# davidesantangelo/krep

Measured on AMD Instinct MI355X. Metric: GB/s scanned (literal scan, match offsets produced), haystack resident in HBM, higher is better.
Workload: dtype u8; 1 GPU; literal8: 8-byte case-sensitive literal 'Sherlock', ~1e-4 matches/byte, offsets tracked; 32 GiB per GPU (BASELINE.json configs[1]); pattern=Sherlock, bytes_per_gpu=34359738368, matches=3436005, parallelism=contiguous shards x1, start-offset ownership, 1 RCCL all-reduce of counts

## Files before the change

include/krep_gpu_debug.h:

```cpp
#ifndef KREP_GPU_DEBUG_H
#define KREP_GPU_DEBUG_H
#include "krep_gpu.h"
#ifdef __cplusplus
extern "C" {
#endif

uint64_t krep_gpu_debug_replay_host(int krep_ref_algo, const void *text, size_t n, const void *pattern, uint32_t m,
                                    int whole_word, size_t cur, int open_line);
void krep_gpu_debug_force_rounds(int rounds);
void krep_gpu_debug_force_stage_cap(int records);
void krep_gpu_debug_force_single_grid(int blocks);
uint64_t krep_gpu_debug_single_failovers(void);
uint64_t krep_gpu_debug_single_launches(void);
uint64_t krep_gpu_debug_tiny_launches(void);
uint64_t krep_gpu_debug_tiny_dense_launches(void);
void krep_gpu_debug_inject_failure(int kind);
void krep_gpu_debug_chain_fixups(uint64_t *rescans, uint64_t *replays);
void krep_gpu_debug_fold_carry(const krep_gpu_seq_carry_t *in, const krep_gpu_seq_carry_t *piece, krep_gpu_seq_carry_t *out);
uint64_t krep_gpu_debug_anchored_launches(void);
uint64_t krep_gpu_debug_literal_dma_launches(void);
uint64_t krep_gpu_debug_literal_dma_one_pass_launches(void);
uint64_t krep_gpu_debug_literal_dma_one_pass_failovers(void);
void krep_gpu_debug_force_literal_dma_grid(int blocks);
int krep_gpu_debug_literal_dma_state(const krep_gpu_plan_t *plan, int *looked, int *barred, double *pass_rate);
uint64_t krep_gpu_debug_runs_launches(void);
int krep_gpu_debug_split_state(const krep_gpu_plan_t *plan);
int krep_gpu_debug_anchor_info(const krep_gpu_plan_t *plan, int *state, uint32_t *moved, double *rate_end_grams, double *rate_anchors);
int krep_gpu_debug_anchor_measured(const krep_gpu_plan_t *plan, double *measured, int *resamples);

#ifdef __cplusplus
}
#endif
#endif
```

krep_amd/csrc/kg_ac.hip:

```cpp
#include <hip/hip_runtime.h>

#include <algorithm>
#include <atomic>
#include <cstdlib>
#include <cstring>
#include <unordered_map>
#include <vector>

#include "../../include/krep_gpu.h"
#include "kg_ac_common.h"
#include "kg_ac_tables.h"
#include "kg_internal.h"

namespace kg {

#ifndef KG_AC_LINES_ROLL_CELLS
#define KG_AC_LINES_ROLL_CELLS 4
#endif
template <bool CI, bool LINES, bool SHORT, int STRIDE, int ANCH = 0, bool WW = false>
__global__ __launch_bounds__(kAcBlock) void ac_scan_kernel(const AcArgs a)
{
    static_assert(!WW || (STRIDE == 2 && !SHORT), "the -w filter of the depth masks: pair filter, no short patterns");
    static_assert(!ANCH || (STRIDE == 2 && !LINES && !SHORT), "anchored scan: pair filter, records / counts only");
    extern __shared__ __attribute__((aligned(16))) u32 s_mem[];
// ... 959 lines not shown
    AcArgs &a = r.a;
    const size_t own_lo = c.own_lo, own_hi = r.own_hi, text_len = c.text_len;
    const bool own_by_end = c.own != AcOwn::Start;
    r.lines_on_list = c.own == AcOwn::LinesOnList;
    r.fsc = g_force_stage_cap.load(std::memory_order_relaxed);
    a.text = c.d_text; a.text_len = text_len; a.global_base = c.global_base;
    a.own_lo = own_lo; a.own_hi = own_hi;
    a.end_lo = own_lo;
    a.end_hi = (c.lines || own_by_end) ? own_hi : std::min<u64>(text_len, (u64)own_hi + t->lmax - 1);
    if (own_by_end)
    {
        a.own_lo = 0, a.own_hi = text_len;
    }
    a.anchor = ((own_by_end && !c.lines && own_lo && !getenv("KREP_GPU_AC_R05_ANCHOR")) ? own_lo - 1 : own_lo) & ~(u64)15;
    a.num_tiles = (a.end_hi - a.anchor + kAcUnitBytes - 1) / kAcUnitBytes;
    a.flags = (t->ci ? F_CI : 0) | (c.ww ? F_WW : 0) | (c.lines ? F_LINES : 0);
    a.flags |= getenv("KREP_GPU_AC_NOVERIFY") ? 1u << 31 : 0u;
    a.flags |= getenv("KREP_GPU_AC_NOSTAGE3") ? 1u << 28 : 0u;
    a.flags |= getenv("KREP_GPU_AC_NODEFER") ? 1u << 27 : 0u;
    a.flags |= getenv("KREP_GPU_AC_NOPROBE") ? 1u << 30 : 0u;
    a.lmax = t->lmax; a.has1 = t->has1; a.has2 = t->has2; a.has3 = t->has3; a.has4 = t->has4;
    a.stride = 1;
    a.filter = c.lines ? t->d_filterx19 : t->d_filterx20;
    a.filter_words = (1u << (c.lines ? kXBitsLines : kXBitsBig)) / 32;
    if (t->d_filters20)
    {
        a.filter = c.lines ? t->d_filters19 : t->d_filters20;
        a.stride = 2;
    }
    if (t->anch_state == 0 && text_len >= (1u << 20) && own_hi - own_lo >= (1u << 19))
    {
        HIPCHK(hipSetDevice(t->device));
        if (ac_anchor_prepare(t, c.d_text, text_len, own_lo, own_hi, c.st) == 2)
            (void)hipGetLastError();
    }
    if (t->anch_state == 2 && !c.lines && a.stride == 2 && !getenv("KREP_GPU_AC_NO_ANCHOR"))
    {
        a.filter = t->d_filtera20;
        a.anch = t->d_anch; a.anch_mask = t->anch_mask; a.anch_mul = t->anch_mul; a.anch_five = t->anch_five;
    }
    if (t->d_xtab && !getenv("KREP_GPU_AC_NO_EXACT"))
    {
        a.xlen = t->d_xlen; a.xtab = t->d_xtab; a.xmask = t->xmask; a.xmul = t->xmul;
    }
    a.s1 = t->d_s1; a.s2 = t->d_s2; a.s3 = t->d_s3;
    if (t->short_dup)
        a.flags |= F_AC_SHORT_DUP;
    a.edges = t->d_edges; a.emask = t->emask; a.copies = t->d_copies;
    a.gram4 = t->d_gram4; a.g4x = t->d_g4x; a.g4mask = t->g4mask;
    a.g4x_mode = t->g4x_mode; a.g4x_mask = t->g4x_mask; a.g4x_mul = t->g4x_mul;
    a.ctr = c.d_ctr;
    r.want = (c.d_pos && c.cap && !c.lines) ? std::min<u64>(c.cap, (u64)c.max_count) : 0;
    if (r.want)
        a.flags |= F_POS;
    a.positions = (u64 *)c.d_pos; a.pos_cap = r.want;
    return 0;
}
static int ac_result(const AcScan &c, const AcRun &r, bool staged, krep_gpu_scan_out_t *out)
{
    const Counters &h = *c.h_ctr;
    if (c.time_it)
    {
        float ms = 0;
        HIPCHK(hipEventElapsedTime(&ms, c.ev0, c.ev1));
        out->kernel_ms = ms;
    }
    const u64 total = h.total;
    out->total_matches = total;
    out->line_count = staged ? h.lines : 0;
    if (r.lines_on_list)
        out->line_count = (r.want && !h.overflow_units && total <= r.want) ? h.lines : ~0ull;
    const u64 summary = (staged && (r.want || c.lines)) ? h.summary : (total ? (kLnHead | kLnTail) : 0);
    out->has_newline = (summary & kLnNl) != 0;
    out->head_line_hit = (summary & kLnHead) != 0;
    out->tail_line_hit = (summary & kLnTail) != 0;
    out->count = std::min<u64>(c.lines ? h.lines : total, (u64)c.max_count);
    if (r.want && c.track)
    {
        out->stored = std::min<u64>(out->count, r.want);
        out->overflow = out->count > c.cap;
    }
    return 0;
}
static int ac_byte_set(const AcScan &c, AcRun &r, krep_gpu_scan_out_t *out)
{
    AcTables *t = c.t;
    if (!(t->set_n && r.want && !c.ww && c.own == AcOwn::Start && t->set_ok && c.text_len >= (size_t)16 * kSegBytes && !r.fsc &&
          !getenv("KREP_GPU_NO_FUSED1") && !getenv("KREP_GPU_AC_NO_TINY")))
        return kAcNext;
    LitArgs la{};
    la.text = c.d_text; la.text_len = c.text_len; la.global_base = c.global_base;
    la.own_lo = c.own_lo; la.own_hi = r.own_hi;
    la.anchor = c.own_lo & ~(u64)15;
    la.rounds = kRoundsBig;
    const u64 tile_bytes = (u64)kRoundsBig * kSegBytes * kWavesPerBlk;
    la.num_tiles = (r.own_hi - la.anchor + tile_bytes - 1) / tile_bytes;
    la.ww_exempt_left = ~0ull;
    la.m = 1;
    la.flags = (t->ci ? F_CI : 0) | F_POS;
    la.ctr = c.d_ctr; la.positions = (uint64_t *)c.d_pos; la.pos_cap = r.want;
    la.set_n = t->set_n;
    for (u32 k = 0; k < t->set_n; ++k)
    {
        la.set_p[k] = 0x01010101u * t->set_b[k];
        la.set_l[k] = (t->ci && t->set_b[k] >= 'a' && t->set_b[k] <= 'z') ? 0x20202020u : 0u;
    }
    la.p0 = la.set_p[0]; la.l0 = la.set_l[0]; la.k0 = 0xffu;
    HIPCHK(hipSetDevice(t->device));
    if (c.time_it) HIPCHK(hipEventRecord(c.ev0, c.st));
    const int rc = single_fused_run(la, la.num_tiles * kWavesPerBlk, r.own_hi - la.anchor, *c.post, c.d_ctr, c.h_ctr, (u32)c.num_cu, &t->set_shape,
                                    c.time_it ? c.ev1 : nullptr, c.st, false);
    if (rc == 2)
        return 2;
    if (rc != kFusedGaveUp)
        return ac_result(c, r, false, out);
    t->set_ok = false;
    return kAcNext;
}
static u32 tiny_dense_upt(double e)
{
    if (e <= 0.0)
        return 4u;
    const double u = (double)ac_tiny_dense_ring() / (2.5 * e);
    return u >= 4.0 ? 4u : (u32)u;
}
static void tiny_reopen(AcTables *t, u64 total, u64 n_units)
{
    if (!t->tiny_fused_ok && total < n_units * 20)
        t->tiny_fused_ok = true;
    if (!t->tiny_dense_ok && total < n_units * 20)
        t->tiny_dense_ok = true;
    if (!t->tiny.five && t->tiny_dense_ok && !t->tiny_dense_upt && total >= n_units * 48)
        t->tiny_dense_upt = tiny_dense_upt((double)total / (double)n_units);
}
static int ac_tiny_one_pass(const AcScan &c, const AcRun &r, krep_gpu_scan_out_t *out)
{
    AcTables *t = c.t;
    Counters *h_ctr = c.h_ctr;
    const bool one_pass_ok = t->tiny.ok && !t->tiny.five && r.want && !c.ww && c.own != AcOwn::End && c.track && !r.fsc &&
                             c.text_len >= (size_t)64 * kAcUnitBytes && !getenv("KREP_GPU_AC_NO_TINY_FUSED") && !getenv("KREP_GPU_AC_NO_TINY");
    const bool dense_first = getenv("KREP_GPU_AC_TINY_DENSE_FIRST") != nullptr;
    if (dense_first && one_pass_ok && !t->tiny_dense_upt && t->tiny_dense_ok)
        t->tiny_dense_upt = 4;
    for (int attempt = 0; one_pass_ok && attempt < 3; ++attempt)
    {
        const bool dense = t->tiny_dense_upt != 0 && !getenv("KREP_GPU_AC_NO_TINY_DENSE");
        if (!dense && (!t->tiny_fused_ok || t->tiny.llong))
            break;
        AcArgs f = r.a;
        f.upt = dense ? t->tiny_dense_upt : (u32)std::min<u64>(kAcUnitsPerTicketMax, std::max<u64>(1, f.num_tiles / ((u64)c.num_cu * kTinyWaves * 4)));
        const u64 n_tk = (f.num_tiles + f.upt - 1) / f.upt;
        const size_t tk_bytes = 2 * n_tk * sizeof(unsigned long long);
        HIPCHK(grow_scratch(c.post->tk_cap, n_tk, n_tk, {dev_buf(c.post->d_tk, tk_bytes)}));
        f.tk_agg = c.post->d_tk; f.tk_pref = c.post->d_tk + n_tk; f.n_tk = n_tk; f.stage_cap = 0;
        HIPCHK(hipSetDevice(t->device));
        if (c.time_it) HIPCHK(hipEventRecord(c.ev0, c.st));
        HIPCHK(hipMemsetAsync(c.d_ctr, 0, sizeof(Counters), c.st));
        HIPCHK(hipMemsetAsync(c.post->d_tk, 0, tk_bytes, c.st));
        HIPCHK(ac_tiny_launch_fused(f, t->tiny, n_tk, (u32)c.num_cu, c.st, dense));
        if (r.lines_on_list && tail_launch_line_gaps(c.d_text, c.text_len, c.global_base, (const uint64_t *)c.d_pos, &c.d_ctr->total,
                                                     &c.d_ctr->overflow_units, r.want, &c.d_ctr->lines, c.st))
            return 2;
        if (c.time_it) HIPCHK(hipEventRecord(c.ev1, c.st));
        HIPCHK(hipMemcpyAsync(h_ctr, c.d_ctr, sizeof(Counters), hipMemcpyDeviceToHost, c.st));
        HIPCHK(hipStreamSynchronize(c.st));
        const double per_unit = (double)h_ctr->total / (double)f.num_tiles;
        if (getenv("KREP_GPU_DEBUG"))
            fprintf(stderr, "krep-gpu: tiny one-pass (%s, %u units per ticket): %llu matches, %.1f per unit, %llu waves overflowed\n",
                    dense ? "dense" : "items", f.upt, (unsigned long long)h_ctr->total, per_unit, (unsigned long long)h_ctr->overflow_units);
        if (!h_ctr->overflow_units)
        {
            if (ac_result(c, r, false, out))
                return 2;
            if (dense)
            {
                if (per_unit < 24.0 && !dense_first)
                    t->tiny_dense_upt = 0, t->tiny_fused_ok = true;
                else
                    t->tiny_dense_upt = std::max(1u, tiny_dense_upt(per_unit));
            }
            return 0;
        }
        u32 nu = (t->tiny_dense_ok && h_ctr->total) ? tiny_dense_upt(per_unit) : 0u;
        if (dense && nu >= t->tiny_dense_upt)
            nu = t->tiny_dense_upt - 1u;
        if (!dense)
            t->tiny_fused_ok = false;
        t->tiny_dense_upt = nu;
        if (!nu)
        {
            t->tiny_dense_ok = false;
            break;
        }
    }
    return kAcNext;
}
static hipError_t ac_staged_launch(const AcScan &c, const AcRun &r, const AcArgs &a)
{
    const u64 n_tickets = (a.num_tiles + a.upt - 1) / a.upt;
    if (r.tiny)
        return ac_tiny_launch(a, c.t->tiny, n_tickets, (u32)c.num_cu, c.st);
    const u32 lds = ac_lds_bytes(a.filter_words, c.lines), per_cu = lds <= 80 * 1024 ? 2u : 1u;
    return ac_launch(a, (u32)std::min<u64>((n_tickets + kAcWaves - 1) / kAcWaves, (u64)c.num_cu * per_cu), lds, c.st);
}
static int ac_staged(const AcScan &c, AcRun &r)
{
    AcArgs &a = r.a;
    const bool chain = r.want || c.lines;
    const u64 n_units = a.num_tiles;
    a.stage_cap = r.want ? (r.fsc ? (u32)r.fsc : c.t->stage_cap) : 0u;
    if (chain)
    {
        if (post_reserve(*c.post, n_units, (n_units * a.stage_cap + 1) / 2))
            return 2;
        a.unitinfo = c.post->d_unitinfo; a.stage = (u64 *)c.post->d_stage; a.offsets = (const u64 *)c.post->d_offsets;
    }
    HIPCHK(hipSetDevice(c.t->device));
    r.tiny = c.t->tiny.ok && !c.ww && (!c.t->tiny.five || (!r.want && !c.lines && !c.t->ci));
    const u32 waves = r.tiny ? (u32)kTinyWaves : (u32)kAcWaves;
    a.upt = (u32)std::min<u64>(kAcUnitsPerTicketMax, std::max<u64>(1, a.num_tiles / ((u64)c.num_cu * waves * 4)));
    if (const char *e = getenv("KREP_GPU_AC_UPT"))
    {
        const int v = atoi(e);
        if (v >= 1 && v <= (int)kAcUnitsPerTicketMax)
            a.upt = (u32)v;
    }
    if (c.time_it) HIPCHK(hipEventRecord(c.ev0, c.st));
    const bool dbg_sync = getenv("KREP_GPU_SYNC_DEBUG") != nullptr;
    auto dbg = [&](const char *what) -> int {
        if (!dbg_sync)
            return 0;
        const hipError_t e = hipStreamSynchronize(c.st);
        return e == hipSuccess ? 0 : fail("ac_scan: %s faulted: %s (tiny=%d stride=%u units=%llu stage_cap=%u lines=%d list=%d own=[%llu,%llu) end=[%llu,%llu) n=%llu)", what,
                                          hipGetErrorString(e), (int)r.tiny, a.stride, (unsigned long long)n_units, a.stage_cap, (int)c.lines, (int)r.lines_on_list,
                                          (unsigned long long)a.own_lo, (unsigned long long)a.own_hi, (unsigned long long)a.end_lo,
                                          (unsigned long long)a.end_hi, (unsigned long long)c.text_len);
    };
    HIPCHK(hipMemsetAsync(c.d_ctr, 0, sizeof(Counters), c.st));
    HIPCHK(ac_staged_launch(c, r, a));
    if (dbg("scan kernel")) return 2;
    if (chain && post_order(*c.post, n_units, a.stage_cap, 0, a.anchor + c.global_base, kAcUnitBytes, c.lines, (uint64_t *)c.d_pos, r.want, c.d_ctr,
                            c.num_cu, c.st))
        return 2;
    if (dbg("post-pass")) return 2;
    if (r.lines_on_list && r.want && tail_launch_line_gaps(c.d_text, c.text_len, c.global_base, (const uint64_t *)c.d_pos, &c.d_ctr->total,
                                                           &c.d_ctr->overflow_units, r.want, &c.d_ctr->lines, c.st))
        return 2;
    if (dbg("line-gap kernel")) return 2;
    if (c.time_it) HIPCHK(hipEventRecord(c.ev1, c.st));
    HIPCHK(hipMemcpyAsync(c.h_ctr, c.d_ctr, sizeof(Counters), hipMemcpyDeviceToHost, c.st));
    HIPCHK(hipStreamSynchronize(c.st));
    return 0;
}
static void ac_learn(const AcScan &c, const AcRun &r)
{
    AcTables *t = c.t;
    const AcArgs &a = r.a;
    const Counters &h = *c.h_ctr;
    const size_t own_lo = c.own_lo, own_hi = r.own_hi;
    const u64 n_units = a.num_tiles;
    if (!r.tiny && !c.lines && a.stride == 2 && own_hi > own_lo)
    {
        const double tested = 0.5 * (double)(own_hi - own_lo);
        t->anch_measured = (double)h.candidates / tested;
        const double est = t->anch_state == 2 ? t->anch_rate : t->anch_rate0;
        if (t->anch_state != 0 && t->anch_resamples < kAnchResamples && c.text_len >= (1u << 20) && own_hi - own_lo >= (1u << 19) &&
            t->anch_measured > 0.008 && t->anch_measured > 2.0 * est + 0.002 && !getenv("KREP_GPU_AC_ANCHOR") && !getenv("KREP_GPU_AC_NO_RESAMPLE"))
        {
            if (getenv("KREP_GPU_DEBUG"))
                fprintf(stderr, "krep-gpu: anchors: measured %.3f %% candidates per tested position against %.3f %% estimated (%s): the next scan decides again\n",
                        100.0 * t->anch_measured, 100.0 * est, t->anch_state == 2 ? "anchored" : "end grams");
            t->anch_state = 0;
            ++t->anch_resamples;
        }
    }
    if (!r.want || r.fsc)
        return;
    if (r.tiny && h.overflow_units * 2 > n_units && h.total > n_units * 256)
        t->stage_cap = 0;
    else if (t->stage_cap && h.overflow_units * 64 > n_units)
        t->stage_cap = 64;
    else if (!t->stage_cap && h.total < n_units * 32)
        t->stage_cap = 64;
    if (r.tiny)
        tiny_reopen(t, h.total, n_units);
    if (t->set_n && !t->set_ok && own_hi > a.anchor && single_fused_reopens(h.total, own_hi - a.anchor))
        t->set_ok = true;
}
static int ac_emit(const AcScan &c, const AcRun &r)
{
    AcTables *t = c.t;
    const u64 n_units = r.a.num_tiles;
    AcArgs e = r.a;
    e.emit_mode = 1;
    HIPCHK(hipMemsetAsync(&c.d_ctr->ticket, 0, sizeof(unsigned long long), c.st));
    if (!r.tiny && !getenv("KREP_GPU_AC_NO_REDO_LIST"))
    {
        const u64 n_over = c.h_ctr->overflow_units;
        const u64 redo_cap = n_over + n_over / 4 + 64;
        if (grow_scratch(t->redo_cap, n_over, redo_cap, {dev_buf(t->d_redo, redo_cap * sizeof(u32))}) != hipSuccess)
            (void)hipGetLastError();
        if (t->d_redo && n_over <= 0xffffffffull)
        {
            HIPCHK(hipMemsetAsync(&c.d_ctr->pad[3], 0, sizeof(unsigned long long), c.st));
            hipLaunchKernelGGL(ac_redo_list_kernel, dim3((u32)((n_units + 255) / 256)), dim3(256), 0, c.st, (const u64 *)e.unitinfo, n_units, e.stage_cap,
                               t->d_redo, (u32)t->redo_cap, &c.d_ctr->pad[3]);
// ... 25 lines not shown
```

krep_amd/csrc/kg_ac_tiny.hip:

```cpp
#include <algorithm>
#include <atomic>
#include <type_traits>
#include <utility>

#include "kg_ac_common.h"
#include "kg_internal.h"
#include "kg_tickets.h"

namespace kg {

bool ac_tiny_keeps(const AcArgs &a);
extern int g_s1_force_grid;
#ifndef KG_TINY_KEEP_WAVES
#define KG_TINY_KEEP_WAVES 2
#endif
#ifndef KG_TINY_FUSED_WAVES
#define KG_TINY_FUSED_WAVES 3
#endif
#ifndef KG_TINY_FIVE_WAVES
#define KG_TINY_FIVE_WAVES 2
#endif
#ifndef KG_TINY_ROLL_CELLS
#define KG_TINY_ROLL_CELLS 6
#endif
#ifndef KG_TINY_LINES_WAVES
#define KG_TINY_LINES_WAVES 3
#endif
#ifndef KG_TINY_COUNT_WAVES
#define KG_TINY_COUNT_WAVES 3
#endif
#define KG_TINY_KEEP_WAVES_ARG ((KEEP && !EMIT) ? KG_TINY_KEEP_WAVES : (FIVE ? KG_TINY_FIVE_WAVES : (FUSED ? KG_TINY_FUSED_WAVES : (LINES ? KG_TINY_LINES_WAVES : KG_TINY_COUNT_WAVES))))
constexpr int kTinyBlock = kTinyWaves * 64;
constexpr u32 kTinyEntries = kAcUnitBytes / 16;

template <int... J, typename F>
__device__ __forceinline__ void tiny_static_for(std::integer_sequence<int, J...>, F &&f)
{
    (f(std::integral_constant<int, J>{}), ...);
}
__device__ __forceinline__ u32 tiny_scramble16(u32 m)
{
    u32 f = 0;
#pragma unroll
    for (int w = 0; w < 4; ++w)
        f |= ((((m >> (4 * w)) & 0xfu) * 0x00204081u) & 0x01010101u) << w;
    return f;
}

template <bool CI, bool LINES, bool KEEP, bool EMIT, bool LONG, bool FUSED = false, bool FIVE = false, bool DENSE = false>
__global__ __launch_bounds__(kTinyBlock, KG_TINY_KEEP_WAVES_ARG) void ac_tiny_kernel(const AcArgs a, const AcTiny td)
{
    static_assert(!DENSE || (FUSED && !FIVE), "DENSE is a flavour of the one-pass writer");
    extern __shared__ __attribute__((aligned(16))) u32 s_tiny[];
    const u32 lane = lane_id(), wave = threadIdx.x >> 6;
    static_assert(!FUSED || (!LINES && !KEEP && !EMIT), "the one-pass record writer is its own mode");
    static_assert(!FIVE || (!LINES && !KEEP && !EMIT && !LONG), "a fifth class: counting and one-pass records only");
    if constexpr (FUSED)
    {
        bool resolver = false;
        if (__builtin_amdgcn_readfirstlane(wave) == 0u)
            resolver = wave_fetch_add(&a.ctr->pad[0], 1ull, lane) == 0ull;
        if (resolver)
        {
            tk_resolve(a.tk_agg, a.tk_pref, a.n_tk, a.ctr, lane);
            return;
        }
    }
    constexpr u32 kPark = kAcUnitsPerTicketMax * 64 + kAcUnitsPerTicketMax * 2;
    constexpr u32 kPerWave = FUSED ? kTinyRing * 3u : kTinyEntries * 2 + kPark;
    u32 *base = s_tiny + wave * kPerWave;
    u32 *park_slots = base + kTinyEntries * 2;
    u64 *park_info = reinterpret_cast<u64 *>(base + kTinyEntries * 2 + kAcUnitsPerTicketMax * 64);
    uint2 *cw = reinterpret_cast<uint2 *>(base);

    const bool want_pos = (a.flags & F_POS) != 0;
    const bool chain = !FUSED && (want_pos || LINES);
    constexpr bool emit_final = EMIT;
    uint2 *ring_m = reinterpret_cast<uint2 *>(base);
    u32 *ring_id = base + 2u * kTinyRing;
    bool pend = false, overflowed = false;
    u64 pend_t = 0;
    u32 pend_at = 0, pend_items = 0, wp = 0;
    u32 f_at = 0, f_room = 0, f_items = 0;
    u32 lane_cnt = 0;
    constexpr u32 kDenseRing = kTinyRing * 6u;
    unsigned short *ring16 = reinterpret_cast<unsigned short *>(base);
    u32 u_c0 = 0, u_c1 = 0, u_c2 = 0, u_before = 0, pend_c0 = 0, pend_c1 = 0, pend_c2 = 0;
    auto dwrap = [](const u32 x) -> u32 { return x >= kDenseRing ? x - kDenseRing : x; };
    auto flush_dense = [&](const u32 l4) __attribute__((always_inline)) {
        const u64 first = tk_wait_prefix(a.tk_pref, pend_t, a.ctr, lane);
        const u64 tbase = a.anchor + pend_t * (u64)a.upt * kAcUnitBytes + a.global_base + 1u;
        const u32 b1 = pend_c0, b2 = pend_c0 + pend_c1, b3 = pend_c0 + pend_c1 + pend_c2;
        const u32 pad = (u32)(first & 7ull);
        for (u32 g = lane; g < pend_items + pad; g += 64u)
        {
            if (g < pad)
                continue;
            const u32 i = g - pad;
            const u32 ent = ring16[dwrap(pend_at + i)];
            const u32 unit = (i >= b1 ? 1u : 0u) + (i >= b2 ? 1u : 0u) + (i >= b3 ? 1u : 0u);
            const u64 idx = first + i;
            if (idx < a.pos_cap)
            {
                const u32 code = ent & 3u, len = code == 3u ? l4 : code + 1u;
                const u64 en = tbase + (u64)unit * kAcUnitBytes + (ent >> 2), st = en - len;
                typedef u32 u32x4 __attribute__((ext_vector_type(4)));
                const u32x4 rec = {(u32)st, (u32)(st >> 32), (u32)en, (u32)(en >> 32)};
                __builtin_nontemporal_store(rec, reinterpret_cast<u32x4 *>(a.positions + 2 * idx));
            }
        }
        pend = false;
    };
    auto walk_lane_cell = [&](const u32 cx, const u32 cy, const u32 cz, const u32 l4, const u32 l5, auto put) __attribute__((always_inline)) {
        const u32 hs = (cx | (cx >> 4) | cy | (cy >> 4) | cz) & 0x0f0f0f0fu;
        u32 h = 0;
#pragma unroll
        for (int b = 0; b < 4; ++b)
        {
            const u32 x = (hs >> (8 * b)) & 0xfu;
            h |= ((x | (x << 3) | (x << 6) | (x << 9)) & 0x1111u) << b;
        }
        while (h)
        {
            const u32 e = (u32)__builtin_ctz(h);
            h &= h - 1u;
            const u32 bit = 8u * (e & 3u) + (e >> 2);
            if (FIVE && ((cz >> bit) & 1u)) put(e, l5);
            if ((cy >> (bit + 4u)) & 1u) put(e, l4);
            if ((cy >> bit) & 1u) put(e, 3u);
            if ((cx >> (bit + 4u)) & 1u) put(e, 2u);
            if ((cx >> bit) & 1u) put(e, 1u);
        }
    };
    auto flush = [&](const u32 l4, const u32 l5) __attribute__((always_inline)) {
        const u64 first = tk_wait_prefix(a.tk_pref, pend_t, a.ctr, lane);
        const u64 tbase = a.anchor + pend_t * (u64)a.upt * kAcUnitBytes + a.global_base;
        u64 run = first;
        for (u32 b0 = 0; b0 < pend_items; b0 += 64u)
        {
            const bool live = b0 + lane < pend_items;
            const u32 slot = (pend_at + b0 + lane) & (kTinyRing - 1u);
            const uint2 m = live ? ring_m[slot] : make_uint2(0u, 0u);
            const u32 w3 = live ? ring_id[slot] : 0u;
            const u32 cz = FIVE ? (w3 & 0x0f0f0f0fu) : 0u;
            const u32 id = FIVE ? (((w3 >> 4) & 0xfu) | ((w3 >> 8) & 0xf0u) | ((w3 >> 12) & 0xf00u) | ((w3 >> 16) & 0xf000u)) : w3;
            const u32 c = (u32)(__popc(m.x) + __popc(m.y) + __popc(cz));
            u32 excl = 0, tot = 0;
            auto plane = [&](const int b) __attribute__((always_inline)) {
                const u64 bm = __ballot((c >> b) & 1u);
                excl += mbcnt64(bm) << b;
                tot += (u32)__popcll(bm) << b;
            };
            plane(0);
            plane(1);
            if (__ballot(c > 3u))
            {
                plane(2);
                plane(3);
                if (__ballot(c > 15u))
                {
                    plane(4);
                    plane(5);
                    plane(6);
                }
            }
            u64 idx = run + excl;
            run += tot;
            if (c)
            {
                const u64 end0 = tbase + (u64)id * 16u + 1u;
                walk_lane_cell(m.x, m.y, cz, l4, l5, [&](const u32 e, const u32 len) {
                    if (idx < a.pos_cap)
                    {
                        const u64 en = end0 + e, st = en - len;
                        typedef u32 u32x4 __attribute__((ext_vector_type(4)));
                        const u32x4 rec = {(u32)st, (u32)(st >> 32), (u32)en, (u32)(en >> 32)};
                        __builtin_nontemporal_store(rec, reinterpret_cast<u32x4 *>(a.positions + 2 * idx));
                    }
                    ++idx;
                });
            }
        }
        pend = false;
    };
    u64 acc_total = 0;
    u64 ovf_units = 0;
    u32 ovf_max = 0;
    constexpr bool LINL = LINES && !KEEP;
    static_assert(!EMIT || (KEEP && !LINES), "emit mode writes records");
    static_assert(!(KEEP && LINES), "-c keeps nothing: its lines are counted in the cell");
    u32 k7f;
    asm volatile("v_mov_b32 %0, 0x7f7f7f7f" : "=v"(k7f));
    const u32 lmax = __builtin_amdgcn_readfirstlane(td.lmax), llong = (LONG || FIVE) ? __builtin_amdgcn_readfirstlane(td.llong) : 0u;
    const u32 len4 = (LONG && llong) ? llong : 4u;
    const u32 n5 = FIVE ? __builtin_amdgcn_readfirstlane(td.n5) : 0u;
    const u32 n1 = __builtin_amdgcn_readfirstlane(td.n[0]), n2 = __builtin_amdgcn_readfirstlane(td.n[1]),
              n3 = __builtin_amdgcn_readfirstlane(td.n[2]), n4 = __builtin_amdgcn_readfirstlane(td.n[3]);

    for (;;)
    {
        const u64 tk = wave_fetch_add(&a.ctr->ticket, 1ull, lane);
        const u64 upt = EMIT ? 64ull : (u64)a.upt;
        const u64 u_begin = tk * upt;
        if (u_begin >= a.num_tiles)
            break;
        const u64 u_end = (u_begin + upt < a.num_tiles) ? u_begin + upt : a.num_tiles;
        u64 em_mask = 0;
        if (EMIT)
            em_mask = __ballot(u_begin + lane < u_end && (u32)(a.unitinfo[u_begin + lane] & kUiCountMask) > a.stage_cap);
        uint4 d[kCells];
        constexpr int kRoll = ((FUSED && !DENSE && !FIVE) || (LINES && (CI || LONG)) || (CI && LONG && !KEEP && !FUSED && !LINES)) ? KG_TINY_ROLL_CELLS : kCells;
        bool have = false;
        u32 carry = 0, carry2 = 0;
        if (FUSED)
        {
            f_at = wp;
            f_room = (DENSE ? kDenseRing : kTinyRing) - pend_items;
            f_items = 0;
            lane_cnt = 0;
            u_c0 = u_c1 = u_c2 = u_before = 0;
        }
        for (u64 unit = u_begin; unit < u_end; ++unit)
        {
            const u64 useg = a.anchor + unit * (u64)kAcUnitBytes;
            if (emit_final && !((em_mask >> (u32)(unit - u_begin)) & 1ull))
                continue;
            const bool do_final = emit_final && want_pos, do_stage = !emit_final && want_pos;
            u32 *slot = reinterpret_cast<u32 *>(a.stage) + unit * (u64)a.stage_cap;
            const bool parked = KEEP && !LINES && do_stage && a.stage_cap <= 64u && a.upt <= kAcUnitsPerTicketMax;
            const u64 fbase = do_final ? a.offsets[unit] : 0ull;
            u32 mycnt = 0;
            u32 l_cnt = 0, s_new = 0;
            bool s_open = false, s_seen = false, s_head = false;
            auto line_cell = [&](const u32 H, const u32 N) __attribute__((always_inline)) {
                const u64 B_any = __ballot(H != 0u), B_nl = __ballot(N != 0u);
                if (!B_any)
                {
                    if (B_nl)
                    {
                        if (!s_seen)
                        {
                            s_head = s_open;
                            s_seen = true;
                        }
                        s_open = false;
                    }
                    return;
                }
                const u32 Hs = H | N;
                l_cnt += (u32)__popc(H & ~(Hs - ((N << 1) & 0xffffu)));
                const u64 B_head = __ballot((H & (Hs ^ (Hs - 1u))) != 0u);
                const u64 G = __ballot(H > N), P = ~(B_nl | B_any);
                const unsigned __int128 sum = (unsigned __int128)(G | P) + G + (s_open ? 1u : 0u);
                const u64 O = (u64)sum ^ P;
                s_new += (u32)__popcll(B_head & ~O);
                if (!s_seen && B_nl)
                {
                    s_head = (((O | B_head) >> __builtin_ctzll(B_nl)) & 1ull) != 0ull;
                    s_seen = true;
                }
                s_open = (u64)(sum >> 64) != 0ull;
            };

#pragma unroll 1
            for (int r = 0; r < kAcRounds; ++r)
            {
                const u64 seg = useg + (u64)r * kSegBytes;
                const bool fast_now = seg + kSegBytes <= a.text_len;
                const bool interior = seg >= a.own_lo + (lmax - 1u) && seg >= a.end_lo && seg + kSegBytes <= a.own_hi && seg + kSegBytes <= a.end_hi;
                const uint4 *src = reinterpret_cast<const uint4 *>(a.text + seg) + lane;
                auto cell = [&](auto interC, const int j, const u32 (&D)[4], const u32 P, const u32 P2) __attribute__((always_inline)) {
                    constexpr bool inter = decltype(interC)::value, kp = KEEP;
                    u32 c1 = n1, c2 = n2, c3 = n3, c4 = n4, lmx = lmax, ll = llong;
                    asm volatile("" : "+s"(c1), "+s"(c2), "+s"(c3), "+s"(c4), "+s"(lmx));
                    u32 c5 = n5;
                    if (LONG || FIVE)
                        asm volatile("" : "+s"(ll));
                    if (FIVE)
                        asm volatile("" : "+s"(c5));
                    u32 NL = 0;
                    if (LINES)
                    {
#pragma unroll
                        for (int w = 0; w < 4; ++w)
                            NL |= movemask4(eq_bytes(D[w], 0x0a0a0a0au)) << (4 * w);
                    }
                    u32 X[4][4];
#pragma unroll
// ... 722 lines not shown
```

krep_amd/csrc/kg_config.hip:

```cpp
#include <hip/hip_runtime.h>

#include <algorithm>
#include <atomic>
#include <chrono>
#include <cstdarg>
#include <cstdio>
#include <cstdlib>
#include <cstring>
#include <mutex>
#include <string>
#include <vector>

#include "../../include/krep_gpu.h"
#include "kg_common.h"
#include "kg_internal.h"
#include "kg_plan.h"
#include "kg_replay.h"

using namespace kg;

static thread_local std::string g_err;
namespace kg {
int fail(const char *fmt, ...)
{
// ... 77 lines not shown
}
extern "C" void krep_gpu_set_reference_simd(int l) { g_simd.store(l, std::memory_order_relaxed); }
extern "C" int krep_gpu_get_reference_simd(void) { return kg::current_config().reference_simd; }
extern "C" void krep_gpu_set_only_matching(int on) { g_only_matching.store(on != 0, std::memory_order_relaxed); }
extern "C" void krep_gpu_set_result_order(int by_start) { g_result_order.store(by_start != 0, std::memory_order_relaxed); }
extern "C" void krep_gpu_set_force_no_simd(int on) { g_no_simd.store(on != 0, std::memory_order_relaxed); }
extern "C" void krep_gpu_set_algo_override(int a) { g_algo_override.store(a, std::memory_order_relaxed); }
extern "C" void krep_gpu_set_device(int d) { g_device.store(d, std::memory_order_relaxed); }
extern "C" void krep_gpu_set_stream_chunk(size_t bytes) { g_stream_chunk.store(bytes, std::memory_order_relaxed); }
extern "C" void krep_gpu_set_num_gpus(int n) { g_num_gpus.store(n, std::memory_order_relaxed); }
extern "C" void krep_gpu_set_min_text_bytes(size_t b) { g_min_bytes.store(b, std::memory_order_relaxed); }

__global__ void kg_probe_kernel(unsigned *out) { *out = 0x950u; }
namespace {
struct Avail
{
    std::mutex mu;
    std::vector<int> state;
    std::vector<std::string> reason;
};
Avail &avail()
{
    static Avail *a = new Avail();
    return *a;
}
thread_local std::string tl_unavail;
bool probe_device(int device, std::string &why)
{
    int prev = -1;
    (void)hipGetDevice(&prev);
    auto done = [&](bool ok) {
        if (prev >= 0)
            (void)hipSetDevice(prev);
        (void)hipGetLastError();
        return ok;
    };
    hipDeviceProp_t prop;
    if (hipGetDeviceProperties(&prop, device) != hipSuccess)
    {
        why = "hipGetDeviceProperties failed";
        return done(false);
    }
    if (strncmp(prop.gcnArchName, "gfx950", 6) != 0)
    {
        why = std::string("device is ") + prop.gcnArchName + ", this library holds gfx950 code only";
        return done(false);
    }
    unsigned *d = nullptr, h = 0;
    if (hipSetDevice(device) != hipSuccess || hipMalloc(&d, sizeof(unsigned)) != hipSuccess)
    {
        why = "cannot allocate on the device";
        return done(false);
    }
    hipLaunchKernelGGL(kg_probe_kernel, dim3(1), dim3(1), 0, nullptr, d);
    const bool ok = hipGetLastError() == hipSuccess && hipMemcpy(&h, d, sizeof h, hipMemcpyDeviceToHost) == hipSuccess && h == 0x950u;
    (void)hipFree(d);
    if (!ok)
        why = "the gfx950 code object of this library does not run on the device";
    return done(ok);
}
}
namespace kg {
const char *device_unusable(int device)
{
    if (const char *e = getenv("KREP_GPU_DISABLE"))
        if (*e && *e != '0')
            return "disabled by KREP_GPU_DISABLE";
    if (const char *e = getenv("KREP_GPU_ASSUME_AVAILABLE"))
        if (*e && *e != '0')
            return nullptr;
    int ndev = 0;
    const auto t_first = std::chrono::steady_clock::now();
    if (hipGetDeviceCount(&ndev) != hipSuccess || ndev <= 0)
    {
        (void)hipGetLastError();
        return "no HIP device available";
    }
    if (device < 0 || device >= ndev)
    {
        tl_unavail = "device " + std::to_string(device) + " out of range (have " + std::to_string(ndev) + ")";
        return tl_unavail.c_str();
    }
    Avail &a = avail();
    std::lock_guard<std::mutex> lk(a.mu);
    if ((size_t)ndev > a.state.size())
    {
        a.state.resize((size_t)ndev, 0);
        a.reason.resize((size_t)ndev);
    }
    if (a.state[device] == 0)
    {
        a.state[device] = probe_device(device, a.reason[device]) ? 1 : 2;
        if (a.state[device] == 1)
            cost_note_device_init(std::chrono::duration<double, std::milli>(std::chrono::steady_clock::now() - t_first).count());
    }
    if (a.state[device] == 1)
        return nullptr;
    tl_unavail = a.reason[device];
    return tl_unavail.c_str();
}
static std::atomic<int> g_inject{-1};
bool inject(int kind)
{
    int v = g_inject.load(std::memory_order_relaxed);
    if (v < 0)
    {
        const char *e = getenv("KREP_GPU_INJECT_FAILURE");
        v = e && *e ? atoi(e) : 0;
        g_inject.store(v, std::memory_order_relaxed);
    }
    return v == kind;
}
}
extern "C" void krep_gpu_debug_inject_failure(int kind) { kg::g_inject.store(kind < 0 ? 0 : kind, std::memory_order_relaxed); }
extern "C" int krep_gpu_available(void) { return kg::device_unusable(kg::current_config().device) == nullptr ? 1 : 0; }
extern "C" const char *krep_gpu_unavailable_reason(void)
{
    const char *r = kg::device_unusable(kg::current_config().device);
    return r ? r : "";
}

namespace kg {
std::atomic<int> g_force_rounds{0};
std::atomic<int> g_force_stage_cap{0};
}
extern "C" void krep_gpu_debug_force_stage_cap(int c) { g_force_stage_cap.store(c); }
extern "C" void krep_gpu_debug_force_rounds(int r) { g_force_rounds.store(r); }
namespace kg {
extern int g_s1_force_grid;
std::atomic<uint64_t> g_fused1_failovers{0};
}
extern "C" void krep_gpu_debug_force_single_grid(int blocks) { kg::g_s1_force_grid = blocks < 0 ? 0 : blocks; }
extern "C" uint64_t krep_gpu_debug_single_failovers(void) { return g_fused1_failovers.load(); }
namespace kg {
std::atomic<uint64_t> g_fused1_launches{0};
}
extern "C" uint64_t krep_gpu_debug_single_launches(void) { return kg::g_fused1_launches.load(); }
namespace kg {
std::atomic<uint64_t> g_tiny_launches{0};
}
extern "C" uint64_t krep_gpu_debug_tiny_launches(void) { return kg::g_tiny_launches.load(); }
namespace kg {
std::atomic<uint64_t> g_tiny_dense_launches{0};
}
extern "C" uint64_t krep_gpu_debug_tiny_dense_launches(void) { return kg::g_tiny_dense_launches.load(); }
namespace kg {
std::atomic<uint64_t> g_ac_anchored_launches{0};
}
extern "C" uint64_t krep_gpu_debug_anchored_launches(void) { return kg::g_ac_anchored_launches.load(); }
extern "C" uint64_t krep_gpu_debug_literal_dma_launches(void) { return kg::g_lit_dma_launches.load(); }
extern "C" uint64_t krep_gpu_debug_literal_dma_one_pass_launches(void) { return kg::g_lit_dma1p_launches.load(); }
extern "C" uint64_t krep_gpu_debug_literal_dma_one_pass_failovers(void) { return kg::g_lit_dma1p_failovers.load(); }
extern "C" void krep_gpu_debug_force_literal_dma_grid(int blocks) { kg::g_lit_dma1p_force_grid = blocks < 0 ? 0 : blocks; }
extern "C" uint64_t krep_gpu_debug_runs_launches(void) { return kg::g_runs_launches.load(); }
```

krep_amd/csrc/kg_internal.h:

```cpp
#pragma once
#include <hip/hip_runtime.h>

#include <atomic>
#include <cstring>
#include <initializer_list>
#include <mutex>
#include <vector>

#include "../../include/krep_gpu.h"
#include "../../include/krep_gpu_debug.h"
#include "kg_common.h"

namespace kg {

int fail(const char *fmt, ...);
const char *device_unusable(int device);
bool inject(int kind);
#define HIPCHK(x)                                                                                 \
    do                                                                                            \
    {                                                                                             \
        hipError_t e_ = (x);                                                                      \
        if (e_ != hipSuccess)                                                                     \
            return kg::fail("%s failed: %s (%s:%d)", #x, hipGetErrorString(e_), __FILE__, __LINE__); \
    } while (0)

struct DevBuf
{
    void **p;
    size_t bytes;
};
template <class T> DevBuf dev_buf(T *&p, size_t bytes) { return {reinterpret_cast<void **>(&p), bytes}; }
inline hipError_t grow_scratch(uint64_t &cap, uint64_t need, uint64_t new_cap, std::initializer_list<DevBuf> bufs)
{
    if (need <= cap)
        return hipSuccess;
    for (const DevBuf &b : bufs)
    {
        if (*b.p) (void)hipFree(*b.p);
        *b.p = nullptr;
    }
    cap = 0;
    for (const DevBuf &b : bufs)
        if (b.bytes)
            if (const hipError_t e = hipMalloc(b.p, b.bytes); e != hipSuccess)
                return e;
    cap = new_cap;
    return hipSuccess;
}

template <auto Kernel> hipError_t grant_dynamic_lds(int bytes)
{
    static std::atomic<bool> granted[64];
    int dev = 0;
    (void)hipGetDevice(&dev);
    const bool known = dev >= 0 && dev < 64;
    if (known && granted[dev].load(std::memory_order_acquire))
        return hipSuccess;
    const hipError_t e = hipFuncSetAttribute(reinterpret_cast<const void *>(Kernel), hipFuncAttributeMaxDynamicSharedMemorySize, bytes);
    if (e == hipSuccess && known)
        granted[dev].store(true, std::memory_order_release);
    return e;
}

hipError_t launch_literal(const LitArgs &a, uint32_t num_cu, hipStream_t st);
int runs_count_greedy(const uint8_t *d_text, uint64_t text_len, uint64_t lo, uint64_t hi, uint32_t m, uint8_t byte, bool ci, int num_cu,
                      unsigned long long *d_slots, unsigned long long *h_slots, hipStream_t st, uint64_t *total, uint64_t *end_p1);
bool literal_dma_eligible(const LitArgs &a);
hipError_t launch_literal_dma(const LitArgs &a, uint32_t num_cu, hipStream_t st);
hipError_t launch_dma_byte_look(const uint8_t *text, uint64_t lo, uint32_t n_cells, uint32_t prefilter, bool ci, unsigned long long *out, hipStream_t st);
extern std::atomic<uint64_t> g_runs_launches;
extern std::atomic<uint64_t> g_lit_dma_launches;
hipError_t launch_literal_dma_one_pass(const LitArgs &a, unsigned long long *d_agg, unsigned long long *d_pref, uint64_t n_tickets,
                                       uint32_t num_cu, hipStream_t st);
uint32_t lit_dma_one_pass_list();
extern std::atomic<uint64_t> g_lit_dma1p_launches;
extern std::atomic<uint64_t> g_lit_dma1p_failovers;
extern int g_lit_dma1p_force_grid;

struct PostScratch;
constexpr int kFusedShapeMax = 5;
double single_fused_max_density(int shape);
int single_fused_shape_for(double density, double margin, int start);
bool single_fused_reopens(uint64_t total, uint64_t span);
constexpr int kFusedGaveUp = 1;
int single_fused_run(const LitArgs &a, uint64_t n_units, uint64_t span, PostScratch &post, Counters *d_ctr, Counters *h_ctr,
                     uint32_t num_cu, int *shape, hipEvent_t ev_end, hipStream_t st, bool count_launch);

struct PostScratch
{
    unsigned long long *d_unitinfo = nullptr;
    unsigned long long *d_offsets = nullptr;
    unsigned long long *d_blk = nullptr;
    uint64_t units_cap = 0;
    unsigned long long *d_stage = nullptr;
    uint64_t stage_cap_words = 0;
    uint64_t *d_occ = nullptr;
    uint64_t occ_cap = 0;
    uint8_t *d_keep = nullptr;
    unsigned long long *d_gblk = nullptr;
    unsigned long long *d_surv = nullptr;
    uint64_t keep_cap = 0;
    unsigned long long *d_tk = nullptr;
    uint64_t tk_cap = 0;
};
void post_free(PostScratch &s);
int post_reserve(PostScratch &s, uint64_t n_units, uint64_t stage_words);
int post_order(PostScratch &s, uint64_t n_units, uint32_t stage_cap, uint32_t fixed_len, uint64_t origin, uint64_t unit_bytes,
               bool want_lines, uint64_t *d_pos, uint64_t pos_cap, Counters *d_ctr, int num_cu, hipStream_t st);
int post_offsets_pass(PostScratch &s, uint64_t n_units, bool want_lines, Counters *d_ctr, hipStream_t st);
int post_gather_pass(PostScratch &s, uint64_t n_units, uint32_t stage_cap, uint32_t fixed_len, uint64_t origin,
                     uint64_t unit_bytes, uint64_t *d_pos, uint64_t pos_cap, int num_cu, hipStream_t st);
constexpr uint32_t kWalkGreedy = 0;
constexpr uint32_t kWalkShortO = 1;
constexpr uint32_t kWalkShortOLines = 2;
struct WalkSpec
{
    uint32_t mode, m;
    bool ww, lines, ci;
    uint8_t b1, b2;
};
int post_walk(PostScratch &s, const uint8_t *d_text, uint64_t text_len, uint64_t global_base, const WalkSpec &ws,
              uint64_t n_occ, uint64_t *d_pos, uint64_t want, Counters *d_ctr, Counters *h_ctr, hipStream_t st,
              uint64_t *total, uint64_t *nlines, uint64_t *resume);

constexpr uint32_t kNlWalkSse42 = 0, kNlWalkKmp = 1;
int post_nlwalk(PostScratch &s, const uint8_t *d_text, uint64_t text_len, uint32_t mode, uint32_t m, uint32_t k0, bool ww, bool om,
                uint64_t maxc, uint64_t n_occ, const uint64_t *d_lineno, Counters *d_ctr, Counters *h_ctr, hipStream_t st,
                uint64_t *count, uint64_t global_base, uint64_t global_len, uint64_t line_off, uint64_t cp_in, uint64_t seen_in,
                uint64_t *cp_out, uint64_t *seen_out);

struct ReplayIn;
int tail_last_hit(const unsigned long long *d_unitinfo, uint64_t limit_units, unsigned long long *d_slot,
                  unsigned long long *h_slot, hipStream_t st, uint64_t *unit_plus1);
int tail_find_next_newline(const uint8_t *d_text, uint64_t from, uint64_t n, unsigned long long *d_slot,
                           unsigned long long *h_slot, hipStream_t st, uint64_t *pos);
int tail_find_prev_newline(const uint8_t *d_text, uint64_t before, unsigned long long *d_slot, unsigned long long *h_slot,
                           hipStream_t st, uint64_t *pos_plus1);
int tail_count_changes(const uint64_t *d_v, uint64_t n, unsigned long long *d_slot, unsigned long long *h_slot, hipStream_t st,
                       uint64_t *changes);
int tail_count_line_gaps(const uint8_t *d_text, uint64_t text_len, uint64_t global_base, const uint64_t *d_rec, uint64_t n, unsigned long long *d_slot,
                         unsigned long long *h_slot, hipStream_t st, uint64_t *lines);
int tail_launch_line_gaps(const uint8_t *d_text, uint64_t text_len, uint64_t global_base, const uint64_t *d_rec, const unsigned long long *d_n,
                          const unsigned long long *d_skip_if, uint64_t cap, unsigned long long *d_out, hipStream_t st);
int tail_count_newlines(const uint8_t *d_text, uint64_t lo, uint64_t hi, unsigned long long *d_slot, unsigned long long *h_slot,
                        hipStream_t st, uint64_t *count);
int tail_run_replay(const ReplayIn &r, unsigned long long *d_slot, unsigned long long *h_slot, hipStream_t st, uint64_t *lines);

int order_records(match_position_t *d_positions, uint64_t n, size_t max_offset, hipStream_t st, bool by_end);
struct AcTables;
AcTables *ac_build(const search_params_t &sp, int device);
void ac_free(AcTables *t);
enum class AcOwn { Start, LinesOnList, End };
struct AcScan
{
    AcTables *t = nullptr;
    Counters *d_ctr = nullptr, *h_ctr = nullptr;
    PostScratch *post = nullptr;
    int num_cu = 0;
    hipEvent_t ev0 = nullptr, ev1 = nullptr;
    hipStream_t st = nullptr;
    const uint8_t *d_text = nullptr;
    size_t text_len = 0, own_lo = 0, own_hi = 0, global_base = 0;
    match_position_t *d_pos = nullptr;
    uint64_t cap = 0, max_count = SIZE_MAX;
    bool track = false, ww = false, lines = false;
    AcOwn own = AcOwn::Start;
    int time_it = 0;
};
int ac_scan(const AcScan &c, krep_gpu_scan_out_t *out);

extern std::atomic<int> g_force_rounds, g_force_stage_cap;
extern std::atomic<uint64_t> g_tiny_launches;
extern std::atomic<uint64_t> g_tiny_dense_launches;
extern std::atomic<uint64_t> g_ac_anchored_launches;
extern std::atomic<uint64_t> g_fused1_launches;
extern std::atomic<uint64_t> g_fused1_failovers;
inline uint8_t lo8(uint8_t c) { return (c >= 'A' && c <= 'Z') ? (uint8_t)(c + 32) : c; }
inline bool pattern_has_border(const uint8_t *p, size_t m)
{
    for (size_t k = 1; k < m; ++k)
        if (memcmp(p, p + k, m - k) == 0)
            return true;
    return false;
}

krep_gpu_config_t current_config();
int mirror_top(const search_params_t *p, const krep_gpu_config_t &c);
int mirror_effective(int top, const search_params_t *p, size_t text_len);
const char *unsupported_reason(const search_params_t *p, const krep_gpu_config_t &c);
constexpr int kSplitWhole = 0, kSplitPieces = 1, kSplitChain = 2;
int split_mode(const search_params_t *p, const krep_gpu_config_t &c, size_t text_len);
bool shardable(const search_params_t *p, const krep_gpu_config_t &c, size_t text_len);
krep_gpu_seq_carry_t fold_carry(const krep_gpu_seq_carry_t &in, const krep_gpu_seq_carry_t &piece);
bool result_reserve(match_result_t *r, uint64_t extra);
inline bool by_start_end(const match_position_t &a, const match_position_t &b)
{
    return a.start_offset != b.start_offset ? a.start_offset < b.start_offset : a.end_offset < b.end_offset;
}
bool have_error();

void format_release();
extern std::mutex g_fmt_mu;
int fmt_reserve(size_t bytes, void **out);
uint64_t scan_sums_words(uint64_t n);
void scan_exclusive(const unsigned long long *in, uint64_t n, unsigned long long *out, unsigned long long *sums, bool take_max,
                    hipStream_t st);
constexpr uint32_t kLineBlock = 4096;
inline uint64_t line_blocks(uint64_t text_len) { return (text_len + kLineBlock - 1) / kLineBlock + 1; }
int newlines_before_blocks(const uint8_t *d_text, uint64_t text_len, unsigned long long *counts, unsigned long long *before,
                           unsigned long long *sums, hipStream_t st);

int allreduce_across_devices(const std::vector<int> &devs, std::vector<std::vector<unsigned long long>> &vecs);
int comm_warmup(const std::vector<int> &devs);
int comm_clique_ranks(const std::vector<int> &devs);

void cost_note_device_init(double ms);
void cost_note_host_path(size_t bytes, double seconds);

int host_scan(const search_params_t *params, const krep_gpu_config_t &cfg, const char *text, size_t text_len, int num_gpus,
              match_result_t *result, uint64_t *ret);

}
```

krep_amd/csrc/kg_literal_dma.hip:

```cpp
#include <hip/hip_runtime.h>
#include <algorithm>
#include <atomic>
#include <cstdlib>
#include "kg_common.h"
#include "kg_device.h"
#include "kg_internal.h"
#include "kg_tickets.h"

namespace kg {

namespace {

constexpr u32 kDmaPark = 80;
constexpr u32 kDmaRing = 2u * kSegBytes;
constexpr u32 kDmaTail = 256u;
constexpr u32 kDmaWaveLds = kDmaRing + kDmaTail;
constexpr u32 kOpHits = 768;
constexpr u32 kOpTk = 32;
static_assert(kOpHits * 4u + kOpTk * 12u <= kDmaPark * 44u, "the one-pass mode's static LDS stays within the staging mode's (two workgroups per CU)");
static_assert(kOpTk <= 64u, "one lane per parked ticket picks its prefix up");
}
uint32_t lit_dma_one_pass_list() { return kOpHits; }

template <int KIND, bool MASKED, bool CI, bool ONEP>
__global__ __launch_bounds__(kBlock, 2) void lit_scan_dma(const LitArgs a, u64 *__restrict__ agg, const u64 *__restrict__ pref, const u64 n_tickets)
{
    extern __shared__ __attribute__((aligned(16))) uint8_t d_smem[];
    __shared__ u64 s_info_all[kWavesPerBlk][ONEP ? 1u : kDmaPark];
    __shared__ __attribute__((aligned(16))) unsigned short s_slots_all[kWavesPerBlk][ONEP ? 8u : kDmaPark * 16u];
    __shared__ u32 s_unit_all[kWavesPerBlk][ONEP ? 1u : kDmaPark];
    __shared__ u32 s_hits_all[kWavesPerBlk][ONEP ? kOpHits : 1u];
    __shared__ u32 s_tk_all[kWavesPerBlk][ONEP ? 3u * kOpTk : 1u];
    const u32 lane = lane_id();
    const u32 wave = __builtin_amdgcn_readfirstlane(threadIdx.x >> 6);
    if (ONEP && wave == 0)
    {
        u64 r = 1;
        if (lane == 0)
            r = __hip_atomic_fetch_add(&a.ctr->pad[0], 1ull, __ATOMIC_RELAXED, __HIP_MEMORY_SCOPE_AGENT);
        if (rfl64(r) == 0ull)
        {
            tk_resolve(agg, const_cast<u64 *>(pref), n_tickets, a.ctr, lane);
            return;
        }
    }
    u32 *s_hits = s_hits_all[wave];
    u32 *s_tk = s_tk_all[wave];
    uint8_t *ring = d_smem + wave * kDmaWaveLds;
    uint8_t *tailb = ring + kDmaRing;
    u64 *s_info = s_info_all[wave];
    unsigned short *s_slots = s_slots_all[wave];
    u32 *s_unit = s_unit_all[wave];
    const u32 ring_lds = (u32)(size_t)(__attribute__((address_space(3))) uint8_t *)ring;

    const bool want_pos = (a.flags & F_POS) != 0;
    const bool ww = (a.flags & F_WW) != 0;
    const u64 hi_match = (a.own_hi < a.text_len - a.m + 1) ? a.own_hi : (a.text_len - a.m + 1);
    constexpr u64 kUnitBytes = (u64)kRoundsBig * kSegBytes;
    const u64 n_units = a.num_tiles * kWavesPerBlk;

    const bool park = want_pos && a.stage_cap >= 16u && a.stage_cap <= 128u && (a.stage_cap & 7u) == 0u && n_units < (1ull << 32);
    const u32 park_max = park ? kDmaPark * 16u / a.stage_cap : 0u;
    u32 n_park = 0;
    auto flush_parked = [&]() __attribute__((always_inline)) {
        for (u32 i = lane; i < n_park; i += 64u)
        {
            const u64 u = s_unit[i];
            a.unitinfo[u] = s_info[i];
            if (s_info[i] & kUiCountMask)
            {
                uint4 *dst = reinterpret_cast<uint4 *>(reinterpret_cast<unsigned short *>(a.stage) + u * (u64)a.stage_cap);
                const uint4 *src = reinterpret_cast<const uint4 *>(&s_slots[i * a.stage_cap]);
                const u32 c = (u32)(s_info[i] & kUiCountMask), nv = ((c < a.stage_cap ? c : a.stage_cap) + 7u) >> 3;
                for (u32 q = 0; q < nv; ++q)
                    dst[q] = src[q];
            }
        }
        n_park = 0;
    };

    const u32 tk_units = a.upt ? a.upt : 1u;
    u64 static_next = (u64)blockIdx.x * kWavesPerBlk + wave;
    auto next_ticket = [&]() -> u64 {
        if (a.upt)
        {
            return wave_fetch_add(&a.ctr->ticket, 1ull, lane) * (u64)a.upt;
        }
        const u64 u = static_next;
        static_next += (u64)gridDim.x * kWavesPerBlk;
        return u;
    };
    auto issue_round = [&](u64 seg, u32 buf) -> bool {
        if (seg + kSegBytes > a.text_len)
            return false;
        const uint8_t *src = a.text + seg + lane * 16u;
        uint8_t *dst = ring + buf * kSegBytes;
#pragma unroll
        for (int j = 0; j < kCells; ++j)
            __builtin_amdgcn_global_load_lds((const __attribute__((address_space(1))) void *)(src + j * kCellBytes),
                                             (__attribute__((address_space(3))) void *)(dst + j * kCellBytes), 16, 0, 2 );
        return true;
    };
    auto issue_tail = [&](u64 at) -> bool {
        if (at + kDmaTail > a.text_len)
            return false;
        __builtin_amdgcn_global_load_lds((const __attribute__((address_space(1))) void *)(a.text + at + lane * 4u),
                                         (__attribute__((address_space(3))) void *)tailb, 4, 0, 0);
        return true;
    };

    u32 hp = 0;
    u32 used = 0;
    u32 n_tkp = 0;
    bool overflowed = false;
    auto hwrap = [](const u32 x) -> u32 { return x >= kOpHits ? x - kOpHits : x; };
    auto flush_records = [&](const u32 n_out) __attribute__((always_inline)) {
        u64 pfx = 0;
        if (lane < n_out)
            pfx = tk_wait_prefix_lane(pref, (u64)s_tk[3u * lane], a.ctr);
        for (u32 i = 0; i < n_out; ++i)
        {
            const u32 t = __builtin_amdgcn_readfirstlane(s_tk[3u * i]), cnt = __builtin_amdgcn_readfirstlane(s_tk[3u * i + 1u]),
                      at = __builtin_amdgcn_readfirstlane(s_tk[3u * i + 2u]);
            const u64 first = ((u64)(u32)__builtin_amdgcn_readlane((u32)(pfx >> 32), i) << 32) | (u32)__builtin_amdgcn_readlane((u32)pfx, i);
            const u64 tbase = a.global_base + a.anchor + (u64)t * ((u64)tk_units * kUnitBytes);
            const u32 pad = (u32)(first & 7ull);
            for (u32 q = lane; q < cnt + pad; q += 64u)
            {
                if (q < pad)
                    continue;
                const u32 e = q - pad;
                const u64 idx = first + e;
                if (idx < a.pos_cap)
                {
                    const u64 st = tbase + s_hits[hwrap(at + e)], en = st + a.m;
                    typedef u32 u32x4 __attribute__((ext_vector_type(4)));
                    const u32x4 rec = {(u32)st, (u32)(st >> 32), (u32)en, (u32)(en >> 32)};
                    __builtin_nontemporal_store(rec, reinterpret_cast<u32x4 *>(a.positions + 2 * idx));
                }
            }
            used -= cnt;
        }
        if (n_out < n_tkp)
        {
            const u32 t = s_tk[3u * n_out], cnt = s_tk[3u * n_out + 1u], at = s_tk[3u * n_out + 2u];
            if (lane == 0)
            {
                s_tk[0] = t;
                s_tk[1] = cnt;
                s_tk[2] = at;
            }
        }
        n_tkp -= n_out;
    };

    u64 acc_total = 0;
    u32 pf_cells = 0;
    u32 wcnt = 0;
    auto stage_hit = [&](u64 unit, u32 idx, u32 rel) __attribute__((always_inline)) {
        if (ONEP)
        {
            if (idx < kOpHits - used)
                s_hits[hwrap(hp + idx)] = rel;
        }
        else if (idx < a.stage_cap)
        {
            unsigned short *slot = park ? &s_slots[n_park * a.stage_cap] : reinterpret_cast<unsigned short *>(a.stage) + unit * (u64)a.stage_cap;
            slot[idx] = (unsigned short)rel;
        }
    };
    auto publish = [&](u64 unit) __attribute__((always_inline)) {
        if (ONEP)
            return;
        acc_total += wcnt;
        if (want_pos)
        {
            if (lane == 0)
            {
                const u64 info = (u64)wcnt | (wcnt ? (kLnHead | kLnTail) : 0ull);
                if (park)
                {
                    s_info[n_park] = info;
                    s_unit[n_park] = (u32)unit;
                }
                else
                    a.unitinfo[unit] = info;
                if (wcnt > a.stage_cap)
                {
                    atomicAdd(&a.ctr->overflow_units, 1ull);
                    atomicMax(&a.ctr->max_unit_count, (u64)wcnt);
                }
            }
            if (park && ++n_park == park_max)
                flush_parked();
        }
        wcnt = 0;
    };
    auto end_ticket = [&](u32 t) __attribute__((always_inline)) {
        if (lane == 0)
            __hip_atomic_store(&agg[t], (u64)wcnt | kTkReady, __ATOMIC_RELAXED, __HIP_MEMORY_SCOPE_AGENT);
        u32 fresh = 0;
        if (wcnt > kOpHits - used)
            overflowed = true;
        else if (wcnt)
        {
            if (lane == 0)
            {
                s_tk[3u * n_tkp] = t;
                s_tk[3u * n_tkp + 1u] = wcnt;
                s_tk[3u * n_tkp + 2u] = hp;
            }
            ++n_tkp;
            hp = hwrap(hp + wcnt);
            used += wcnt;
            fresh = 1;
        }
        wcnt = 0;
        if ((n_tkp == kOpTk || used > kOpHits / 2u) && n_tkp > fresh)
            flush_records(n_tkp - fresh);
    };
    auto exact = [&](u32 A0, u32 A4) -> bool {
        const u32 e0 = CI ? (A0 | a.l0) : A0;
        bool h = (KIND == 4 && MASKED) ? (((e0 ^ a.p0) & a.k0) == 0u) : (e0 == a.p0);
        if (KIND >= 8)
        {
            const u32 e4 = CI ? (A4 | a.l1) : A4;
            h = h && ((KIND == 8 && MASKED) ? (((e4 ^ a.p1) & a.k1) == 0u) : (e4 == a.p1));
        }
        return h;
    };
    auto owned = [&](u64 p) -> bool { return p >= a.own_lo && p < hi_match && !(p >= a.excl_lo && p < a.excl_hi); };
    auto word_ok = [&](u64 p) -> bool {
        if (p > 0 && p != a.ww_exempt_left && is_wordc(a.text[p - 1]))
            return false;
        if (p + a.m < a.text_len && is_wordc(a.text[p + a.m]))
            return false;
        return true;
    };
    auto boundary = [&](u64 seg_prev, u64 unit, u32 r_prev, u32 c0, u32 c1, u32 n0, u32 n1) __attribute__((always_inline)) {
        {
            const u32 f = 0x01010101u * ((CI ? (a.p0 | 0x20u) : a.p0) & 0xffu);
            const u32 y0 = (CI ? (c0 | 0x20202020u) : c0) ^ f, y1 = (CI ? (c1 | 0x20202020u) : c1) ^ f;
            if (((((y0 - 0x01010101u) & ~y0) | ((y1 - 0x01010101u) & ~y1)) & 0x80808080u) == 0u)
                return;
        }
        const u32 q = lane & 7u, sh = q & 3u;
        const bool up = (q >> 2) != 0u;
        const u32 lo = up ? c1 : c0, mid = up ? n0 : c1, hi = up ? n1 : n0;
        const u32 A0 = __builtin_amdgcn_alignbyte(mid, lo, sh), A4 = __builtin_amdgcn_alignbyte(hi, mid, sh);
        const u64 p = seg_prev + (kSegBytes - 8u) + q;
        bool h = lane < 8u && q + a.m > 8u && exact(A0, A4) && owned(p);
        if (ww && __ballot(h))
            h = h && word_ok(p);
        const u64 bm = __ballot(h);
        if (bm)
        {
            if (h && want_pos)
                stage_hit(unit, wcnt + mbcnt64(bm), r_prev * kSegBytes + (kSegBytes - 8u) + q);
            wcnt += (u32)__popcll(bm);
        }
    };

    u64 u0 = next_ticket();
    bool dma_cur = u0 < n_units && issue_round(a.anchor + u0 * kUnitBytes, 0u);
    while (u0 < n_units)
    {
        const u32 nun = (u32)((n_units - u0 < (u64)tk_units) ? (n_units - u0) : (u64)tk_units), nr = nun * (u32)kRoundsBig;
        const u64 tbase = a.anchor + u0 * kUnitBytes;
        u64 u_next = ~0ull;
        bool tail_ok = false;
        u32 c0 = 0, c1 = 0;
        bool deferred = false;
#pragma unroll 1
        for (u32 g = 0; g < nr; ++g)
        {
            const u64 seg = tbase + (u64)g * kSegBytes, unit = u0 + (g >> 2);
            const u32 r = g & 3u;
            bool dma_nx = false, tail_now = false;
            asm volatile("s_waitcnt lgkmcnt(0)" ::: "memory");
            if (g + 1u < nr)
                dma_nx = issue_round(seg + kSegBytes, (g + 1u) & 1u);
            else
            {
                u_next = next_ticket();
                if (u_next < n_units)
                    dma_nx = issue_round(a.anchor + u_next * kUnitBytes, (g + 1u) & 1u);
            }
            if (g + 2u == nr)
                tail_ok = tail_now = issue_tail(tbase + (u64)nr * kSegBytes);
            if (dma_cur)
            {
                if (dma_nx && tail_now)
                    asm volatile("s_waitcnt vmcnt(9)" ::: "memory");
                else if (dma_nx)
                    asm volatile("s_waitcnt vmcnt(8)" ::: "memory");
                else if (tail_now)
                    asm volatile("s_waitcnt vmcnt(1)" ::: "memory");
                else
                    asm volatile("s_waitcnt vmcnt(0)" ::: "memory");
            }
            const bool interior = seg >= a.own_lo && seg + kSegBytes <= hi_match && (seg + kSegBytes <= a.excl_lo || seg >= a.excl_hi);
            uint4 vv[kCells];
            uint2 nn[kCells];
            if (dma_cur)
            {
                typedef u32 v4 __attribute__((ext_vector_type(4)));
                typedef u32 v2 __attribute__((ext_vector_type(2)));
                const u32 addr = ring_lds + (g & 1u) * kSegBytes + lane * 16u;
                v4 x[kCells];
                v2 y[kCells];
#pragma unroll
                for (int j = 0; j < kCells; ++j)
                {
                    asm volatile("ds_read_b128 %0, %1 offset:%2" : "=v"(x[j]) : "v"(addr), "n"(j * (int)kCellBytes));
                    asm volatile("ds_read_b64 %0, %1 offset:%2" : "=v"(y[j]) : "v"(addr), "n"(j * (int)kCellBytes + 16));
                }
                asm volatile("s_waitcnt lgkmcnt(0)"
                             : "+v"(x[0]), "+v"(x[1]), "+v"(x[2]), "+v"(x[3]), "+v"(x[4]), "+v"(x[5]), "+v"(x[6]), "+v"(x[7]), "+v"(y[0]), "+v"(y[1]),
                               "+v"(y[2]), "+v"(y[3]), "+v"(y[4]), "+v"(y[5]), "+v"(y[6]), "+v"(y[7])
                             :
                             : "memory");
#pragma unroll
                for (int j = 0; j < kCells; ++j)
                {
                    vv[j] = make_uint4(x[j].x, x[j].y, x[j].z, x[j].w);
                    nn[j] = make_uint2(y[j].x, y[j].y);
                }
            }
            else
            {
#pragma unroll
                for (int j = 0; j < kCells; ++j)
                {
                    const W6 w = load_window_guarded(a.text, a.text_len, seg + (u64)j * kCellBytes + (u64)lane * 16u);
                    vv[j] = make_uint4(w.v[0], w.v[1], w.v[2], w.v[3]);
                    nn[j] = make_uint2(w.v[4], w.v[5]);
                }
            }
            if (deferred)
            {
                boundary(seg - kSegBytes, u0 + ((g - 1u) >> 2), ONEP ? g - 1u : (g - 1u) & 3u, c0, c1, __builtin_amdgcn_readfirstlane(vv[0].x),
                         __builtin_amdgcn_readfirstlane(vv[0].y));
                deferred = false;
                if (r == 0u)
                    publish(unit - 1u);
            }
            __builtin_amdgcn_sched_barrier(0);
#pragma unroll
            for (int j = 0; j < kCells; ++j)
            {
                const u64 lbase = seg + (u64)j * kCellBytes + (u64)lane * 16u;
                const u32 D[6] = {vv[j].x, vv[j].y, vv[j].z, vv[j].w, nn[j].x, nn[j].y};
                auto A = [&](int k) -> u32 {
// ... 1 lines not shown
                };
                u32 Dq[6];
#pragma unroll
                for (int w = 0; w < 6; ++w)
                    Dq[w] = CI ? (D[w] | 0x20202020u) : D[w];
                auto Aq = [&](int k) -> u32 {
                    return ((k & 3) == 0) ? Dq[k >> 2] : __builtin_amdgcn_alignbyte(Dq[(k >> 2) + 1], Dq[k >> 2], (u32)(k & 3));
                };
                const u32 p0q = CI ? (a.p0 | 0x20202020u) : a.p0;
                if (a.prefilter)
                {
                    u32 z = 0;
#pragma unroll
                    for (int w = 0; w < 4; ++w)
                    {
                        const u32 y = Dq[w] ^ a.prefilter;
                        z |= (y - 0x01010101u) & ~y;
                    }
                    if (!__ballot((z & 0x80808080u) != 0u))
                        continue;
                    ++pf_cells;
                }
                bool c[16];
                u64 any = 0;
#pragma unroll
                for (int k = 0; k < 16; ++k)
                {
                    const u32 x = Aq(k);
                    c[k] = (KIND == 4 && MASKED) ? (((x ^ p0q) & a.k0) == 0u) : (x == p0q);
                    any |= __ballot(c[k]);
                }
                if (!any)
                    continue;
                u32 m16 = 0;
#pragma unroll
                for (int k = 0; k < 16; ++k)
                    if (__ballot(c[k]))
                        m16 |= (c[k] && exact(A(k), A(k + 4))) ? (1u << k) : 0u;
                if (dma_cur && j == kCells - 1 && lane == 63u)
                    m16 &= (1u << (17u - a.m)) - 1u;
                if (!interior)
                {
                    auto clip = [&](u64 lo, u64 hi) -> u32 {
                        const u32 klo = lo > lbase ? (u32)((lo - lbase) < 16 ? (lo - lbase) : 16) : 0u;
                        const u32 khi = hi > lbase ? (u32)((hi - lbase) < 16 ? (hi - lbase) : 16) : 0u;
                        return khi > klo ? (((1u << khi) - 1u) & ~((1u << klo) - 1u)) : 0u;
                    };
                    m16 &= clip(a.own_lo, hi_match) & ~clip(a.excl_lo, a.excl_hi);
                }
                if (ww && __ballot(m16 != 0u))
                {
                    const u32 below = __shfl_up(D[3], 1);
                    auto pick = [&](u32 i) -> u32 {
                        const u32 q = i >> 2;
                        const u32 w = q == 0u ? below : q == 1u ? D[0] : q == 2u ? D[1] : q == 3u ? D[2] : q == 4u ? D[3] : q == 5u ? D[4] : D[5];
                        return (w >> (8u * (i & 3u))) & 0xffu;
                    };
                    const bool edge = dma_cur && j == kCells - 1 && lane == 63u;
                    u32 rest = m16;
                    while (rest)
                    {
                        const u32 k = __builtin_ctz(rest);
                        rest &= rest - 1u;
                        const u64 p = lbase + k;
                        bool bad;
                        if (edge || (lane == 0u && k == 0u))
                            bad = !word_ok(p);
                        else
                            bad = (p != a.ww_exempt_left && is_wordc(pick(k + 3u))) || is_wordc(pick(k + a.m + 4u));
                        if (bad)
                            m16 &= ~(1u << k);
                    }
                }
                if (!__ballot(m16 != 0u))
                    continue;
                const u32 cnt = __popc(m16);
                u32 idx = wcnt, tot = 0;
                auto plane = [&](int b) {
                    const u64 bm = __ballot((cnt >> b) & 1u);
                    idx += mbcnt64(bm) << b;
                    tot += (u32)__popcll(bm) << b;
                };
                plane(0);
                plane(1);
                if (__ballot(cnt > 3u))
                {
                    plane(2);
                    plane(3);
                    plane(4);
                }
                wcnt += tot;
                if (want_pos)
                {
                    const u32 rel0 = ((ONEP ? g : r) * (u32)kCells + (u32)j) * kCellBytes + lane * 16u;
                    u32 rest = m16;
                    while (rest)
                    {
                        const u32 k = __builtin_ctz(rest);
                        rest &= rest - 1u;
                        stage_hit(unit, idx++, rel0 + k);
                    }
                }
            }
            if (dma_cur)
            {
                c0 = __builtin_amdgcn_readlane(vv[kCells - 1].z, 63);
                c1 = __builtin_amdgcn_readlane(vv[kCells - 1].w, 63);
                deferred = true;
            }
            if (g + 1u == nr)
            {
                if (deferred)
                {
                    u32 n0 = 0, n1 = 0;
                    if (tail_ok)
                    {
                        typedef u32 v2 __attribute__((ext_vector_type(2)));
                        v2 t;
                        const u32 taddr = ring_lds + kDmaRing;
                        asm volatile("ds_read_b64 %0, %1\n\ts_waitcnt lgkmcnt(0)" : "=v"(t) : "v"(taddr) : "memory");
                        n0 = __builtin_amdgcn_readfirstlane(t.x);
                        n1 = __builtin_amdgcn_readfirstlane(t.y);
                    }
                    else
                    {
                        const W6 w = load_window_guarded(a.text, a.text_len, seg + kSegBytes);
                        n0 = __builtin_amdgcn_readfirstlane(w.v[0]);
                        n1 = __builtin_amdgcn_readfirstlane(w.v[1]);
                    }
                    boundary(seg, unit, ONEP ? g : r, c0, c1, n0, n1);
                    deferred = false;
                }
                if (ONEP)
                    end_ticket((u32)u0 / tk_units);
                else
                    publish(unit);
            }
            else if (!deferred && r == 3u)
                publish(unit);
            dma_cur = dma_nx;
        }
        u0 = u_next;
    }
    if (!ONEP && park && n_park)
        flush_parked();
    if (ONEP && n_tkp)
        flush_records(n_tkp);
    if (ONEP && overflowed && lane == 0)
        atomicAdd(&a.ctr->overflow_units, 1ull);
    if (lane == 0 && acc_total)
        atomicAdd(&a.ctr->total, acc_total);
    if (lane == 0 && pf_cells)
        atomicAdd(&a.ctr->candidates, (u64)pf_cells);
}

__global__ __launch_bounds__(256) void dma_byte_look(const uint8_t *text, u64 lo, u32 n_cells, u32 b4, u32 fold, unsigned long long *out)
{
    const u32 lane = lane_id();
    const u32 wave = blockIdx.x * 4u + (threadIdx.x >> 6), n_waves = gridDim.x * 4u;
    u32 cnt = 0;
    for (u32 c = wave; c < n_cells; c += n_waves)
    {
        const uint4 v = *reinterpret_cast<const uint4 *>(text + lo + (u64)c * kCellBytes + lane * 16u);
        const u32 d[4] = {v.x, v.y, v.z, v.w};
        u32 z = 0;
#pragma unroll
        for (int w = 0; w < 4; ++w)
        {
            const u32 y = (d[w] | fold) ^ b4;
            z |= (y - 0x01010101u) & ~y;
        }
        if (__ballot((z & 0x80808080u) != 0u))
            ++cnt;
    }
    if (lane == 0 && cnt)
        atomicAdd(out, (u64)cnt);
}
hipError_t launch_dma_byte_look(const uint8_t *text, uint64_t lo, uint32_t n_cells, uint32_t prefilter, bool ci, unsigned long long *out, hipStream_t st)
{
    hipLaunchKernelGGL(dma_byte_look, dim3(256), dim3(256), 0, st, text, (u64)lo, n_cells, prefilter, ci ? 0x20202020u : 0u, out);
    return hipGetLastError();
}

std::atomic<uint64_t> g_lit_dma_launches{0};
std::atomic<uint64_t> g_lit_dma1p_launches{0};
std::atomic<uint64_t> g_lit_dma1p_failovers{0};
int g_lit_dma1p_force_grid = 0;

template <int KIND, bool MASKED, bool CI, bool ONEP>
static hipError_t dma_launch4(const LitArgs &a, u64 *agg, const u64 *pref, u64 n_tickets, u32 num_cu, hipStream_t st)
{
    constexpr u32 lds = kWavesPerBlk * kDmaWaveLds;
    if (const hipError_t e = grant_dynamic_lds<&lit_scan_dma<KIND, MASKED, CI, ONEP>>((int)lds); e != hipSuccess)
        return e;
    static const u32 bpc = [] { const char *e = getenv("KREP_GPU_LIT_DMA_BLOCKS_PER_CU"); return e && atoi(e) > 0 ? (u32)atoi(e) : 2u; }();
    u32 grid = (u32)std::min<u64>(a.num_tiles, (u64)num_cu * bpc);
    if (ONEP && g_lit_dma1p_force_grid > 0)
        grid = std::min<u32>(grid, (u32)g_lit_dma1p_force_grid);
    hipLaunchKernelGGL((lit_scan_dma<KIND, MASKED, CI, ONEP>), dim3(grid ? grid : 1), dim3(kBlock), lds, st, a, agg, pref, n_tickets);
    g_lit_dma_launches.fetch_add(1, std::memory_order_relaxed);
    if (ONEP)
        g_lit_dma1p_launches.fetch_add(1, std::memory_order_relaxed);
    return hipGetLastError();
}
template <int KIND, bool MASKED, bool ONEP>
static hipError_t dma_launch2(const LitArgs &a, u64 *agg, const u64 *pref, u64 n_tickets, u32 num_cu, hipStream_t st)
{
    return (a.flags & F_CI) ? dma_launch4<KIND, MASKED, true, ONEP>(a, agg, pref, n_tickets, num_cu, st)
                            : dma_launch4<KIND, MASKED, false, ONEP>(a, agg, pref, n_tickets, num_cu, st);
}
template <bool ONEP>
static hipError_t dma_launch1(const LitArgs &a, u64 *agg, const u64 *pref, u64 n_tickets, u32 num_cu, hipStream_t st)
{
    if (a.m < 4)
        return dma_launch2<4, true, ONEP>(a, agg, pref, n_tickets, num_cu, st);
    if (a.m == 4)
        return dma_launch2<4, false, ONEP>(a, agg, pref, n_tickets, num_cu, st);
    if (a.m < 8)
        return dma_launch2<8, true, ONEP>(a, agg, pref, n_tickets, num_cu, st);
    return dma_launch2<8, false, ONEP>(a, agg, pref, n_tickets, num_cu, st);
}

bool literal_dma_eligible(const LitArgs &a)
{
    return !getenv("KREP_GPU_LIT_NO_DMA") && a.prefilter != 0u && a.m >= 2 && a.m <= 8 && a.rounds == (u32)kRoundsBig && !(a.flags & F_LINES) && !a.emit_mode &&
           (a.upt >= 4 || getenv("KREP_GPU_LIT_DMA_ALL")) && a.text_len >= 4u * kSegBytes;
}
hipError_t launch_literal_dma(const LitArgs &a, u32 num_cu, hipStream_t st)
{
    return dma_launch1<false>(a, nullptr, nullptr, 0, num_cu, st);
}
hipError_t launch_literal_dma_one_pass(const LitArgs &a, unsigned long long *d_agg, unsigned long long *d_pref, uint64_t n_tickets, u32 num_cu,
                                       hipStream_t st)
{
    const u64 n_units = a.num_tiles * kWavesPerBlk;
    if (!(a.flags & F_POS) || !a.upt || n_units >= (1ull << 32) || n_tickets != (n_units + a.upt - 1) / a.upt || (u64)a.upt * kRoundsBig * kSegBytes > (1ull << 31))
        return hipErrorInvalidValue;
    return dma_launch1<true>(a, d_agg, d_pref, n_tickets, num_cu, st);
}

}
```

krep_amd/csrc/kg_plan.hip:

```cpp
#include <hip/hip_runtime.h>

#include <algorithm>
#include <atomic>
#include <chrono>
#include <cstdarg>
#include <cstdio>
#include <cstdlib>
#include <cstring>
#include <mutex>
#include <string>
#include <vector>

#include "../../include/krep_gpu.h"
#include "kg_common.h"
#include "kg_internal.h"
#include "kg_plan.h"
#include "kg_replay.h"
#include "kg_ac_tables.h"

using namespace kg;

extern "C" krep_gpu_plan_t *krep_gpu_plan_create_ex(const search_params_t *p, const krep_gpu_config_t *cfg_in)
{
    if (!p)
// ... 33 lines not shown
    else if (p->pattern)
        pl->pats.emplace_back((const uint8_t *)p->pattern, (const uint8_t *)p->pattern + p->pattern_len);
    for (auto &v : pl->pats)
    {
        pl->pat_ptrs.push_back(v.empty() ? "" : (const char *)v.data());
        pl->pat_lens.push_back(v.size());
    }
    pl->sp = *p;
    pl->sp.patterns = pl->pat_ptrs.data();
    pl->sp.pattern_lens = pl->pat_lens.data();
    pl->sp.num_patterns = pl->pats.size();
    if (!pl->pats.empty())
    {
        pl->sp.pattern = pl->pat_ptrs[0];
        pl->sp.pattern_len = pl->pat_lens[0];
    }
    pl->ref_algo = mirror_top(&pl->sp, cfg);
    if (const char *why = kg::unsupported_reason(&pl->sp, cfg))
        pl->unsupported = why;

    hipDeviceProp_t prop;
    if (hipGetDeviceProperties(&prop, device) == hipSuccess)
        pl->num_cu = prop.multiProcessorCount;
    bool ok = hipMalloc(&pl->d_ctr, sizeof(Counters)) == hipSuccess &&
              hipHostMalloc(&pl->h_ctr, sizeof(Counters)) == hipSuccess &&
              hipEventCreate(&pl->ev0) == hipSuccess && hipEventCreate(&pl->ev1) == hipSuccess;
    if (ok && pl->sp.num_patterns == 1 && pl->pats[0].size() >= 1)
    {
        const auto &raw = pl->pats[0];
        pl->m = (uint32_t)raw.size();
        pl->pat_folded = raw;
        if (!pl->cs)
            for (auto &c : pl->pat_folded)
                c = lo8(c);
        pl->has_border = pattern_has_border(pl->pat_folded.data(), pl->pat_folded.size());
        pl->has_newline = memchr(raw.data(), '\n', raw.size()) != nullptr;
        uint8_t w[8] = {0}, k[8] = {0};
        for (uint32_t i = 0; i < 8 && i < pl->m; ++i)
        {
            w[i] = pl->pat_folded[i];
            k[i] = 0xff;
        }
        memcpy(&pl->p0, w, 4);
        memcpy(&pl->p1, w + 4, 4);
        memcpy(&pl->k0, k, 4);
        memcpy(&pl->k1, k + 4, 4);
        if (pl->m == 1)
            pl->p0 = 0x01010101u * w[0];
        {
            uint8_t w2[8] = {0}, kk[8] = {0}, ll[8] = {0};
            for (uint32_t i = 8; i < 16 && i < pl->m; ++i)
            {
                w2[i - 8] = pl->pat_folded[i];
                kk[i - 8] = 0xff;
                ll[i - 8] = (!pl->cs && w2[i - 8] >= 'a' && w2[i - 8] <= 'z') ? 0x20 : 0;
            }
            memcpy(&pl->p2, w2, 4); memcpy(&pl->p3, w2 + 4, 4);
            memcpy(&pl->k2, kk, 4); memcpy(&pl->k3, kk + 4, 4);
            memcpy(&pl->l2, ll, 4); memcpy(&pl->l3, ll + 4, 4);
        }
        if (!pl->cs)
        {
            uint8_t l[8] = {0};
            for (uint32_t i = 0; i < 8 && i < pl->m; ++i)
                l[i] = (w[i] >= 'a' && w[i] <= 'z') ? 0x20 : 0;
            memcpy(&pl->l0, l, 4);
            memcpy(&pl->l1, l + 4, 4);
            if (pl->m == 1)
                pl->l0 = 0x01010101u * l[0];
        }
        ok = hipMalloc(&pl->d_pat, pl->m) == hipSuccess &&
             hipMemcpy(pl->d_pat, pl->pat_folded.data(), pl->m, hipMemcpyHostToDevice) == hipSuccess;
        if (ok && pl->m > 8)
        {
            pl->n_chunks = (pl->m - 8 + 7) / 8;
            std::vector<unsigned long long> ch(2 * pl->n_chunks, 0ull);
            for (uint32_t k = 0; k < pl->n_chunks; ++k)
            {
                const uint8_t *src = pl->pat_folded.data() + std::min<uint32_t>(8 + 8 * k, pl->m - 8);
                memcpy(&ch[k], src, 8);
                uint8_t l[8];
                for (int b = 0; b < 8; ++b)
                    l[b] = (!pl->cs && src[b] >= 'a' && src[b] <= 'z') ? 0x20 : 0;
                memcpy(&ch[pl->n_chunks + k], l, 8);
            }
            ok = hipMalloc(&pl->d_pat_chunks, ch.size() * 8) == hipSuccess &&
                 hipMemcpy(pl->d_pat_chunks, ch.data(), ch.size() * 8, hipMemcpyHostToDevice) == hipSuccess;
        }
    }
    if (ok && pl->ref_algo == KREP_RA_AHO_CORASICK)
    {
        for (auto &v : pl->pats)
            if (!v.empty() && memchr(v.data(), '\n', v.size()))
                pl->ac_has_newline = true;
        pl->ac = ac_build(pl->sp, device);
        ok = pl->ac != nullptr;
    }
    if (!ok)
    {
        if (!kg::have_error())
            kg::fail("plan_create: device allocation failed");
        krep_gpu_plan_destroy(pl);
        return nullptr;
    }
    return pl;
}
extern "C" krep_gpu_plan_t *krep_gpu_plan_create(const search_params_t *p, int only_matching, int device)
{
    krep_gpu_config_t c = kg::current_config();
    c.only_matching = only_matching != 0;
    c.device = device;
    return krep_gpu_plan_create_ex(p, &c);
}

#define DBGFREE(x)                                                                      \
    do                                                                                  \
    {                                                                                   \
        hipError_t e_ = (x);                                                            \
        if (e_ != hipSuccess && getenv("KREP_GPU_DEBUG"))                               \
            fprintf(stderr, "krep-gpu: (debug) %s -> %s\n", #x, hipGetErrorString(e_)); \
    } while (0)
extern "C" void krep_gpu_plan_destroy(krep_gpu_plan_t *pl)
{
    if (!pl)
        return;
    (void)hipSetDevice(pl->device);
    if (pl->d_pat) DBGFREE(hipFree(pl->d_pat));
    if (pl->d_pat_chunks) DBGFREE(hipFree(pl->d_pat_chunks));
    if (pl->d_ctr) DBGFREE(hipFree(pl->d_ctr));
    if (pl->h_ctr) DBGFREE(hipHostFree(pl->h_ctr));
    if (pl->ev0) DBGFREE(hipEventDestroy(pl->ev0));
    if (pl->ev1) DBGFREE(hipEventDestroy(pl->ev1));
    if (pl->ac) ac_free(pl->ac);
    if (pl->ac_long) ac_free(pl->ac_long);
    if (pl->ac_short) ac_free(pl->ac_short);
    if (pl->d_split_rec) DBGFREE(hipFree(pl->d_split_rec));
    if (pl->d_nl_rec) DBGFREE(hipFree(pl->d_nl_rec));
    if (pl->d_nl_ln) DBGFREE(hipFree(pl->d_nl_ln));
    post_free(pl->post);
    post_free(pl->aux);
    delete pl;
}
extern "C" int krep_gpu_plan_ref_algo(const krep_gpu_plan_t *pl) { return pl ? pl->ref_algo : KREP_RA_NONE; }
extern "C" int krep_gpu_debug_split_state(const krep_gpu_plan_t *pl) { return pl ? pl->ac_split : -1; }
extern "C" int krep_gpu_debug_literal_dma_state(const krep_gpu_plan_t *pl, int *looked, int *barred, double *pass_rate)
{
    if (!pl)
        return 2;
    if (looked) *looked = pl->dma_look_done;
    if (barred) *barred = pl->dma_off;
    if (pass_rate) *pass_rate = pl->dma_pass_rate;
    return 0;
}
extern "C" int krep_gpu_debug_anchor_measured(const krep_gpu_plan_t *pl, double *measured, int *resamples)
{
    if (!pl || !pl->ac)
        return 2;
    if (measured) *measured = pl->ac->anch_measured;
    if (resamples) *resamples = pl->ac->anch_resamples;
    return 0;
}
extern "C" int krep_gpu_debug_anchor_info(const krep_gpu_plan_t *pl, int *state, uint32_t *moved, double *rate_end_grams, double *rate_anchors)
{
    if (!pl || !pl->ac)
        return 2;
    if (state) *state = pl->ac->anch_state;
    if (moved) *moved = pl->ac->anch_moved;
    if (rate_end_grams) *rate_end_grams = pl->ac->anch_rate0;
    if (rate_anchors) *rate_anchors = pl->ac->anch_rate;
    return 0;
}
```

krep_amd/csrc/kg_scan.hip:

```cpp
#include <hip/hip_runtime.h>

#include <algorithm>
#include <cstdio>
#include <cstdlib>
#include <cstring>
#include <vector>

#include "../../include/krep_gpu.h"
#include "kg_common.h"
#include "kg_internal.h"
#include "kg_plan.h"
#include "kg_replay.h"

using namespace kg;

struct Verdict { uint64_t ret, store; };
static Verdict verdict_for(int algo, const krep_gpu_plan *pl, uint64_t total, uint64_t lines, bool have_result)
{
    const size_t maxc = pl->max_count;
    const bool store = pl->track && have_result;
    Verdict v{0, 0};
    switch (algo)
    {
    case KREP_RA_MEMCHR:
    case KREP_RA_KMP:
    case KREP_RA_AHO_CORASICK:
    case KREP_RA_SSE42:
        if (maxc == 0)
            return v;
        break;
    case KREP_RA_NEON:
        if (maxc == 0)
            return v;
        break;
    default:
        if (maxc == 0)
        {
            if (pl->lines || pl->track)
                return v;
            v.ret = total > 0 ? 1 : 0;
            return v;
        }
    }
    if (pl->lines)
    {
        v.ret = std::min<uint64_t>(lines, maxc);
        return v;
    }
    v.ret = std::min<uint64_t>(total, maxc);
    if (store)
    {
        v.store = v.ret;
        if (algo == KREP_RA_KMP && maxc != SIZE_MAX && total > maxc)
            v.store = v.ret + 1;
    }
    return v;
}

int kg::stop_clock(krep_gpu_plan *pl, bool record_ev1, hipStream_t st, krep_gpu_scan_out_t *out)
{
    if (record_ev1) HIPCHK(hipEventRecord(pl->ev1, st));
    HIPCHK(hipStreamSynchronize(st));
    float ms = 0;
    HIPCHK(hipEventElapsedTime(&ms, pl->ev0, pl->ev1));
    out->kernel_ms = ms;
    return 0;
}

namespace {
struct LitPass
{
    bool ww = false, lines = false;
    bool first_byte = false;
    size_t own_lo = 0, own_hi = 0;
    uint64_t excl_lo = 0, excl_hi = 0;
    uint64_t ww_exempt = ~0ull;
    enum Sink { COUNT, RECORDS, OCC } sink = COUNT;
    uint64_t *d_out = nullptr;
    uint64_t out_cap = 0;
    PostScratch *post = nullptr;
    hipEvent_t ev_end = nullptr;
};
struct LitResult
{
    uint64_t total = 0, lines = 0;
    unsigned long long summary = 0;
    uint64_t n_units = 0, unit_bytes = 0, anchor = 0;
};
struct LitScan
{
    LitArgs a{};
    uint64_t hi_match = 0;
    uint64_t n_units = 0;
    int fsc = 0;
    bool dma_keep = false;
    uint64_t span() const { return hi_match - a.anchor; }
    uint64_t unit_bytes() const { return (uint64_t)a.rounds * kSegBytes; }
    double density(uint64_t hits) const { return (double)hits / (double)span(); }
};
}

static double fusedk_min_hits_per_unit()
{
    static const double v = [] {
        const char *e = getenv("KREP_GPU_FUSEDK_MIN");
        return e ? atof(e) : 24.0;
    }();
    return v;
}
static double lit_dma_max_pass()
{
    static const double v = [] { const char *e = getenv("KREP_GPU_LIT_DMA_MAX_PASS"); return e ? atof(e) : 0.35; }();
    return v;
}

static LitScan lit_args(const krep_gpu_plan *pl, const Window &w, const LitPass &ps, size_t own_hi, uint64_t hi_match)
{
    LitScan L;
    LitArgs &a = L.a;
    const uint32_t m_scan = ps.first_byte ? 1u : pl->m;
    L.hi_match = hi_match;
    a.text = w.d_text;
    a.text_len = w.text_len;
    a.own_lo = ps.own_lo;
    a.own_hi = own_hi;
    a.anchor = ps.own_lo & ~(uint64_t)15;
    {
        const uint64_t span = hi_match - a.anchor;
        a.rounds = span >= ((uint64_t)pl->num_cu * 16 * kRoundsBig * kSegBytes * kWavesPerBlk) ? kRoundsBig : 1;
        const int fr = g_force_rounds.load(std::memory_order_relaxed);
        if (fr == 1 || fr == kRoundsBig)
            a.rounds = (uint32_t)fr;
        const uint64_t tile_bytes = (uint64_t)a.rounds * kSegBytes * kWavesPerBlk;
        a.num_tiles = (span + tile_bytes - 1) / tile_bytes;
    }
    a.global_base = w.global_base;
    a.ww_exempt_left = ps.ww_exempt;
    a.excl_lo = ps.excl_lo;
    a.excl_hi = ps.excl_hi;
    a.m = m_scan;
    if (ps.first_byte)
    {
        const uint8_t b = pl->pat_folded[0];
        a.p0 = 0x01010101u * b;
        a.k0 = 0xffu;
        a.l0 = (!pl->cs && b >= 'a' && b <= 'z') ? 0x20202020u : 0u;
    }
    else
    {
        a.p0 = pl->p0; a.p1 = pl->p1; a.k0 = pl->k0; a.k1 = pl->k1;
        a.l0 = pl->l0; a.l1 = pl->l1;
        a.p2 = pl->p2; a.p3 = pl->p3; a.k2 = pl->k2; a.k3 = pl->k3; a.l2 = pl->l2; a.l3 = pl->l3;
    }
    a.pat = pl->d_pat;
    a.pat_chunks = pl->d_pat_chunks;
    a.n_chunks = ps.first_byte ? 0 : pl->n_chunks;
    a.ctr = pl->d_ctr;
    a.flags = (pl->cs ? 0 : F_CI) | (ps.ww ? F_WW : 0) | (ps.lines ? F_LINES : 0) | (ps.sink != LitPass::COUNT ? F_POS : 0);
    {
        const uint32_t b0 = (a.p0 & 0xffu) | (pl->cs ? 0u : 0x20u);
        static const char common[] = "etaoinshrdlu";
        bool rare = b0 != ' ' && b0 != '\n';
        for (const char *q = common; *q; ++q)
            rare = rare && b0 != (uint32_t)*q;
        a.prefilter = (rare && !ps.first_byte && !getenv("KREP_GPU_LIT_NO_PREFILTER")) ? 0x01010101u * b0 : 0u;
// ... 57 lines not shown
    if (pl->dma_pass_rate > lit_dma_max_pass() && !L.dma_keep)
    {
        pl->dma_off = true;
        pl->dma_off_text = w.d_text;
        pl->dma_off_len = w.text_len;
        if (getenv("KREP_GPU_DEBUG"))
            fprintf(stderr, "krep-gpu: literal scan: the prefilter passed %.1f %% of the 1-KiB cells -> the register kernel from the next scan on\n", 100.0 * pl->dma_pass_rate);
    }
}

static int lit_first_look(krep_gpu_plan *pl, const LitPass &ps, LitScan &L, hipStream_t st)
{
    LitArgs &a = L.a;
    const uint32_t m_scan = a.m;
    if (!(ps.sink == LitPass::RECORDS && !pl->first_look_done && a.rounds == kRoundsBig && L.fsc == 0 && !ps.first_byte && !ps.lines &&
          ps.excl_lo == ps.excl_hi && L.span() >= (1ull << 30) && !getenv("KREP_GPU_NO_FIRST_LOOK")))
        return 0;
    pl->first_look_done = true;
    const uint64_t span = L.span(), win = 2ull << 20, tile_bytes = (uint64_t)kRoundsBig * kSegBytes * kWavesPerBlk;
    HIPCHK(hipMemsetAsync(pl->d_ctr, 0, sizeof(Counters), st));
    uint64_t looked = 0;
    for (int q = 0; q < 2; ++q)
    {
        LitArgs sm = a;
        sm.flags &= ~(uint32_t)(F_POS | F_LINES);
        sm.stage_cap = 0;
        sm.upt = 0;
        sm.emit_mode = 0;
        sm.own_lo = (a.anchor + span / 4 * (2 * q + 1)) & ~(uint64_t)15;
        sm.own_hi = std::min<uint64_t>(L.hi_match, sm.own_lo + win);
        sm.anchor = sm.own_lo;
        sm.num_tiles = (sm.own_hi - sm.anchor + tile_bytes - 1) / tile_bytes;
        looked += sm.own_hi - sm.own_lo;
        HIPCHK(launch_literal(sm, (uint32_t)pl->num_cu, st));
    }
    HIPCHK(hipMemcpyAsync(pl->h_ctr, pl->d_ctr, sizeof(Counters), hipMemcpyDeviceToHost, st));
    HIPCHK(hipStreamSynchronize(st));
    const double density = looked ? (double)pl->h_ctr->total / (double)looked : 0.0, per_unit = density * 32768.0;
    pl->lit_density = density;
    if (m_scan == 1)
    {
        if (density > single_fused_max_density(kFusedShapeMax))
            pl->fused1_ok = false;
        else
            pl->fused1_shape = single_fused_shape_for(density, 1.05, 0);
    }
    else if (m_scan <= 8 && !pl->fusedk_never && per_unit >= fusedk_min_hits_per_unit() &&
             density <= single_fused_max_density(kFusedShapeMax))
    {
        pl->fusedk_on = true;
        pl->fusedk_shape = single_fused_shape_for(density, 1.05, 0);
    }
    else if (per_unit > 6.0)
        pl->sparse_cap = std::max<uint32_t>(pl->sparse_cap, per_unit > 100.0 ? 256u : per_unit > 40.0 ? 128u : 64u);
    if (getenv("KREP_GPU_DEBUG"))
        fprintf(stderr, "krep-gpu: first look: %.2f hits per 32-KiB unit in %llu sampled bytes -> one-pass %d (shape %d / %d), staging slot %u\n", per_unit,
                (unsigned long long)looked, (int)(m_scan == 1 ? pl->fused1_ok : pl->fusedk_on), pl->fused1_shape, pl->fusedk_shape, pl->sparse_cap);
    if ((a.flags & F_POS) && !L.fsc)
        a.stage_cap = a.rounds == kRoundsBig ? (m_scan == 1 ? 512u : pl->sparse_cap) : a.stage_cap;
    return 0;
}

static int lit_one_pass(krep_gpu_plan *pl, const Window &w, const LitPass &ps, LitScan &L, hipStream_t st, LitResult *res, bool *done)
{
    LitArgs &a = L.a;
    const uint32_t m_scan = a.m;
    *done = false;
    const bool fusedk = m_scan >= 2 && m_scan <= 8 && pl->fusedk_on;
    if (!((m_scan == 1 ? pl->fused1_ok : fusedk) && ps.sink == LitPass::RECORDS && !(ps.ww && m_scan == 1) && !ps.lines && !ps.first_byte &&
          a.rounds == kRoundsBig && L.fsc == 0 && ps.excl_lo == ps.excl_hi && w.text_len >= 2 * (size_t)kSegBytes &&
          !getenv("KREP_GPU_NO_FUSED1")))
        return 0;
    a.positions = ps.d_out;
    a.pos_cap = ps.out_cap;
    int &plan_shape = m_scan == 1 ? pl->fused1_shape : pl->fusedk_shape;
    const int rc = single_fused_run(a, L.n_units, L.span(), *ps.post, pl->d_ctr, pl->h_ctr, (uint32_t)pl->num_cu, &plan_shape, ps.ev_end, st,
                                    true);
    if (rc == 2)
        return 2;
    if (rc != kFusedGaveUp)
    {
        res->total = pl->h_ctr->total;
        res->summary = res->total ? (kLnHead | kLnTail) : 0;
        if (m_scan != 1 && L.density(res->total) * 32768.0 < 0.5 * fusedk_min_hits_per_unit())
            pl->fusedk_on = false;
        *done = true;
        return 0;
    }
    if (m_scan == 1)
        pl->fused1_ok = false;
    else
        pl->fusedk_on = false, pl->fusedk_never = true;
    g_fused1_failovers.fetch_add(1);
    return 0;
}

static void lit_learn_density(krep_gpu_plan *pl, const LitPass &ps, const LitScan &L)
{
    const LitArgs &a = L.a;
    const uint32_t m_scan = a.m;
    if (L.span() >= 8 * L.unit_bytes() && !ps.first_byte)
        pl->lit_density = L.density(pl->h_ctr->total);
    if ((a.flags & F_POS) && m_scan != 1 && a.rounds == kRoundsBig && pl->h_ctr->overflow_units * 64 > L.n_units && !L.fsc)
    {
        uint32_t want = 64;
        if (pl->sparse_cap >= 64)
            for (want = 128; want < 256 && want < pl->h_ctr->max_unit_count; want *= 2) {}
        pl->sparse_cap = std::max(pl->sparse_cap, want);
    }
    if ((a.flags & F_POS) && m_scan >= 2 && m_scan <= 8 && a.rounds == kRoundsBig && !L.fsc && !pl->fusedk_never &&
        ps.sink == LitPass::RECORDS && !ps.lines && L.hi_match > a.anchor)
    {
        const double density = L.density(pl->h_ctr->total);
        if (density * 32768.0 >= fusedk_min_hits_per_unit() && density <= single_fused_max_density(kFusedShapeMax))
        {
            pl->fusedk_on = true;
            pl->fusedk_shape = single_fused_shape_for(density, 1.0, 0);
        }
    }
    if (getenv("KREP_GPU_DEBUG") && (a.flags & F_POS))
        fprintf(stderr, "krep-gpu: literal scan: %llu of %llu units overflowed a %u-entry slot (fullest: %llu); one-pass next: %d (shape %d)\n",
                pl->h_ctr->overflow_units, (unsigned long long)L.n_units, a.stage_cap, pl->h_ctr->max_unit_count, (int)pl->fusedk_on,
                pl->fusedk_shape);
}
static void lit_reopen(krep_gpu_plan *pl, const LitScan &L)
{
    const uint32_t m_scan = L.a.m;
    if (!pl->fused1_ok && m_scan == 1 && single_fused_reopens(pl->h_ctr->total, L.span()))
        pl->fused1_ok = true;
    if (pl->fusedk_never && m_scan >= 2 && m_scan <= 8 && single_fused_reopens(pl->h_ctr->total, L.span()))
        pl->fusedk_never = false;
}

static int lit_dma_one_pass(krep_gpu_plan *pl, const Window &w, const LitPass &ps, LitScan &L, hipStream_t st, LitResult *res, bool *done)
{
    *done = false;
    if (!(ps.sink == LitPass::RECORDS && !ps.lines && !ps.first_byte && ps.excl_lo == ps.excl_hi && L.fsc == 0 && !getenv("KREP_GPU_LIT_DMA_TWO_PASS")))
        return 0;
    LitArgs a = L.a;
    if (!a.upt && getenv("KREP_GPU_LIT_DMA_ALL") && !getenv("KREP_GPU_LIT_UPT"))
        a.upt = 8;
    if (!a.upt || !literal_dma_eligible(a) || L.n_units >= (1ull << 32))
        return 0;
    if (pl->dma1p_off && pl->dma1p_off_text == (const void *)w.d_text && pl->dma1p_off_len == w.text_len)
        return 0;
    const uint64_t ticket_bytes = (uint64_t)a.upt * L.unit_bytes();
    const double gate = std::min(0.25 * (double)lit_dma_one_pass_list(), fusedk_min_hits_per_unit() * (double)a.upt);
    if (pl->lit_density >= 0.0 && pl->lit_density * (double)ticket_bytes >= gate)
        return 0;
    constexpr uint64_t kCtrWords = 16;
    static_assert(sizeof(Counters) <= kCtrWords * sizeof(unsigned long long), "the counters in front of the ticket arrays");
    const uint64_t n_tk = (L.n_units + a.upt - 1) / a.upt, cap_tk = n_tk + kCtrWords / 2;
    PostScratch &post = *ps.post;
    HIPCHK(grow_scratch(post.tk_cap, cap_tk, cap_tk, {dev_buf(post.d_tk, 2 * cap_tk * sizeof(unsigned long long))}));
    Counters *d_ctr = reinterpret_cast<Counters *>(post.d_tk);
    unsigned long long *d_agg = post.d_tk + kCtrWords, *d_pref = d_agg + n_tk;
    a.ctr = d_ctr;
    a.positions = ps.d_out;
    a.pos_cap = ps.out_cap;
    a.stage_cap = 0;
    HIPCHK(hipMemsetAsync(post.d_tk, 0, (kCtrWords + 2 * n_tk) * sizeof(unsigned long long), st));
    HIPCHK(launch_literal_dma_one_pass(a, d_agg, d_pref, n_tk, (uint32_t)pl->num_cu, st));
    if (ps.ev_end) HIPCHK(hipEventRecord(ps.ev_end, st));
    HIPCHK(hipMemcpyAsync(pl->h_ctr, d_ctr, sizeof(Counters), hipMemcpyDeviceToHost, st));
    HIPCHK(hipStreamSynchronize(st));
    LitScan La = L;
    La.a = a;
    lit_dma_rate(pl, w, La);
    if (pl->h_ctr->overflow_units)
    {
        pl->dma1p_off = true;
        pl->dma1p_off_text = w.d_text;
        pl->dma1p_off_len = w.text_len;
        g_lit_dma1p_failovers.fetch_add(1);
        if (getenv("KREP_GPU_DEBUG"))
            fprintf(stderr, "krep-gpu: literal scan: a ticket overflowed the one-pass hit list -> the two-pass road for this text\n");
        return 0;
    }
    if (L.span() >= ticket_bytes)
        pl->lit_density = L.density(pl->h_ctr->total);
    res->total = pl->h_ctr->total;
    res->summary = res->total ? (kLnHead | kLnTail) : 0;
    *done = true;
    return 0;
}

static int lit_two_pass(krep_gpu_plan *pl, const Window &w, const LitPass &ps, LitScan &L, bool chain, hipStream_t st)
{
    LitArgs &a = L.a;
    a.positions = ps.d_out;
    a.pos_cap = ps.sink == LitPass::RECORDS ? ps.out_cap : 0;
    HIPCHK(launch_literal(a, (uint32_t)pl->num_cu, st));
    if (chain && post_order(*ps.post, L.n_units, a.stage_cap, a.m, a.anchor + w.global_base, L.unit_bytes(), ps.lines, ps.d_out, a.pos_cap,
                            pl->d_ctr, pl->num_cu, st))
        return 2;
    if (ps.ev_end) HIPCHK(hipEventRecord(ps.ev_end, st));
    HIPCHK(hipMemcpyAsync(pl->h_ctr, pl->d_ctr, sizeof(Counters), hipMemcpyDeviceToHost, st));
    HIPCHK(hipStreamSynchronize(st));
    lit_dma_rate(pl, w, L);
    lit_learn_density(pl, ps, L);
    if ((a.flags & F_POS) && pl->h_ctr->overflow_units)
    {
        LitArgs e = a;
        e.emit_mode = 1;
        HIPCHK(hipMemsetAsync(&pl->d_ctr->ticket, 0, sizeof(unsigned long long), st));
        HIPCHK(launch_literal(e, (uint32_t)pl->num_cu, st));
        if (ps.ev_end) HIPCHK(hipEventRecord(ps.ev_end, st));
    }
    return 0;
}
static int lit_two_pass_occ(krep_gpu_plan *pl, const Window &w, const LitPass &ps, const LitScan &L, hipStream_t st)
{
    const LitArgs &a = L.a;
    PostScratch &post = *ps.post;
    HIPCHK(launch_literal(a, (uint32_t)pl->num_cu, st));
    if (post_offsets_pass(post, L.n_units, false, pl->d_ctr, st))
        return 2;
    HIPCHK(hipMemcpyAsync(pl->h_ctr, pl->d_ctr, sizeof(Counters), hipMemcpyDeviceToHost, st));
    HIPCHK(hipStreamSynchronize(st));
    const uint64_t n_occ = pl->h_ctr->total;
    HIPCHK(grow_scratch(post.occ_cap, n_occ, n_occ, {dev_buf(post.d_occ, n_occ * 2 * sizeof(uint64_t))}));
    if (n_occ)
    {
        if (post_gather_pass(post, L.n_units, a.stage_cap, a.m, a.anchor + w.global_base, L.unit_bytes(), post.d_occ, n_occ, pl->num_cu, st))
            return 2;
        if (pl->h_ctr->overflow_units)
        {
            LitArgs e = a;
            e.emit_mode = 1;
            e.positions = post.d_occ;
            e.pos_cap = n_occ;
            HIPCHK(hipMemsetAsync(&pl->d_ctr->ticket, 0, sizeof(unsigned long long), st));
            HIPCHK(launch_literal(e, (uint32_t)pl->num_cu, st));
        }
    }
    return 0;
}

static int lit_pass(krep_gpu_plan *pl, const Window &w, const LitPass &ps, hipStream_t st, LitResult *res)
{
    *res = LitResult{};
    const uint32_t m_scan = ps.first_byte ? 1u : pl->m;
    size_t own_hi = std::min(ps.own_hi, w.text_len);
    if (ps.first_byte)
        own_hi = std::min<size_t>(own_hi, w.text_len - pl->m + 1);
    const uint64_t hi_match = std::min<uint64_t>(own_hi, w.text_len - m_scan + 1);
    if (hi_match <= ps.own_lo)
        return 0;
    LitScan L = lit_args(pl, w, ps, own_hi, hi_match);
    if (lit_dma_look(pl, w, ps, L, st))
        return 2;
    res->n_units = L.n_units;
    res->unit_bytes = L.unit_bytes();
    res->anchor = L.a.anchor;
    bool done = false;
    if (lit_first_look(pl, ps, L, st) || lit_one_pass(pl, w, ps, L, st, res, &done))
        return 2;
    if (done)
        return 0;
    if (lit_dma_one_pass(pl, w, ps, L, st, res, &done))
        return 2;
    if (done)
        return 0;
    const bool chain = (L.a.flags & (F_POS | F_LINES)) != 0;
    if (chain)
    {
        PostScratch &post = *ps.post;
        if (post_reserve(post, L.n_units, (L.n_units * L.a.stage_cap + 3) / 4))
            return 2;
        L.a.unitinfo = post.d_unitinfo;
        L.a.stage = (uint64_t *)post.d_stage;
        L.a.offsets = (const uint64_t *)post.d_offsets;
    }
    HIPCHK(hipMemsetAsync(pl->d_ctr, 0, sizeof(Counters), st));
    if (ps.sink != LitPass::OCC ? lit_two_pass(pl, w, ps, L, chain, st) : lit_two_pass_occ(pl, w, ps, L, st))
        return 2;
    res->total = pl->h_ctr->total;
    res->lines = pl->h_ctr->lines;
    lit_reopen(pl, L);
    res->summary = chain ? pl->h_ctr->summary : (res->total ? (kLnHead | kLnTail) : 0);
    return 0;
}

namespace {
struct Family
{
    bool greedy = false;
    bool mshort_o = false;
    bool need_walk = false;
    bool replay = false;
    bool neon_zero = false;
    bool nlwalk = false;
    bool whole_text() const { return need_walk || replay || neon_zero || nlwalk; }
};
Family family_of(int algo, bool only_matching, bool lines, bool ww, bool track, size_t maxc, bool has_border, uint32_t m,
                 bool pat_has_newline = false)
{
    Family f;
    if (lines && pat_has_newline && (algo == KREP_RA_SSE42 || algo == KREP_RA_KMP))
    {
        f.nlwalk = true;
        return f;
    }
    f.greedy = (algo == KREP_RA_SSE42 || algo == KREP_RA_KMP);
    if (only_matching)
    {
        if (algo == KREP_RA_SSE42)
            f.greedy = false;
        else if (algo == KREP_RA_BMH && !lines)
            f.greedy = true;
        else if (algo == KREP_RA_MEMCHR_SHORT)
            f.mshort_o = true;
    }
    f.need_walk = (f.greedy && has_border && m > 1) || f.mshort_o;
    if (f.need_walk && !f.mshort_o && lines && !ww)
        f.need_walk = false;
    f.replay = lines && (algo == KREP_RA_AVX512 || algo == KREP_RA_NEON || (algo == KREP_RA_AVX2 && ww));
    f.neon_zero = algo == KREP_RA_NEON && maxc == 0 && !lines && !track;
// ... 506 lines not shown
    }
    if (j.carry_out)
        j.carry_out->resume = std::max(resume_in, resume_out);
    t->summary = t->total ? (kLnHead | kLnTail) : 0;
    if (pl->lines && !j.whole)
    {
        unsigned long long *d_slot = &pl->d_ctr->pad[0], *h_slot = &pl->h_ctr->pad[0];
        uint64_t first_nl = own_hi, last_p1 = 0;
        if (tail_find_next_newline(w.d_text, w.own_lo, own_hi, d_slot, h_slot, st, &first_nl))
            return 2;
        t->summary = 0;
        if (first_nl < own_hi)
        {
            if (tail_find_prev_newline(w.d_text, own_hi, d_slot, h_slot, st, &last_p1))
                return 2;
            t->summary |= kLnNl;
        }
        if (t->total)
        {
            uint64_t s_first[2], s_last[2];
            HIPCHK(hipMemcpy(s_first, pl->post.d_surv, sizeof s_first, hipMemcpyDeviceToHost));
            HIPCHK(hipMemcpy(s_last, pl->post.d_surv + 2 * (t->total - 1), sizeof s_last, hipMemcpyDeviceToHost));
            const uint64_t f = s_first[0] - w.global_base, l = s_last[0] - w.global_base;
            if (!(t->summary & kLnNl))
                t->summary |= kLnHead | kLnTail;
            else
                t->summary |= (f <= first_nl ? kLnHead : 0) | (l >= last_p1 ? kLnTail : 0);
        }
    }
    return 0;
}

static int lit_finish(const LitJob &j, int time_it, const LitTotals &t, krep_gpu_scan_out_t *out)
{
    krep_gpu_plan *pl = j.pl;
    if (time_it)
    {
        if (stop_clock(pl, !t.ev1_recorded, j.st, out))
            return 2;
    }
    else
        HIPCHK(hipStreamSynchronize(j.st));
    out->total_matches = t.total;
    out->line_count = t.lines;
    out->has_newline = (t.summary & kLnNl) != 0;
    out->head_line_hit = (t.summary & kLnHead) != 0;
    out->tail_line_hit = (t.summary & kLnTail) != 0;
    Verdict v = verdict_for(j.algo, pl, t.total, t.lines, j.d_pos != nullptr);
    out->count = v.ret;
    if (j.d_pos && j.cap && pl->track && !pl->lines)
    {
        const uint64_t maxc = pl->max_count;
        const uint64_t needed = (j.algo == KREP_RA_MEMCHR && maxc != SIZE_MAX && maxc != 0) ? std::min<uint64_t>(t.total, maxc + 1)
                                                                                             : v.store;
        out->overflow = needed > j.cap;
        out->stored = std::min<uint64_t>(needed, std::min<uint64_t>(t.total, j.want));
    }
    return 0;
}

static int scan_literal(krep_gpu_plan *pl, int algo, const Window &w, match_position_t *d_pos, uint64_t cap, hipStream_t st,
                        int time_it, const krep_gpu_seq_carry_t *carry_in, krep_gpu_seq_carry_t *carry_out, krep_gpu_scan_out_t *out)
{
    const uint32_t m = pl->m;
    memset(out, 0, sizeof *out);
    if (carry_out)
        *carry_out = carry_in ? *carry_in : krep_gpu_seq_carry_t{};
    if (m == 0 || w.global_len < m || w.text_len < m || w.own_lo >= w.own_hi)
        return 0;
    const size_t own_hi = std::min(w.own_hi, w.text_len);
    const bool whole = w.global_base == 0 && w.own_lo == 0 && own_hi + m > w.text_len && w.global_len == w.text_len;

    const Family fam = family_of(algo, pl->only_matching, pl->lines, pl->ww, pl->track, pl->max_count, pl->has_border, m,
                                 pl->has_newline);
    LitJob j{pl, algo, w, own_hi, whole, st, carry_in, carry_out, d_pos, cap, 0};
    if (fam.nlwalk)
        return lit_nlwalk(j, time_it, out);
    if (fam.need_walk && !whole && !carry_in && w.global_base + w.own_lo != 0)
        return kg::fail("the greedy / only-matching families couple neighbouring matches: scan the whole text in one window, or "
                        "its pieces in text order through krep_gpu_scan_device_seq() (%s, pattern length %u)",
                        krep_gpu_algorithm_name(algo), m);

    {
        const uint64_t G = w.global_len, base = w.global_base;
        auto to_local = [&](uint64_t g) -> uint64_t { return g >= base && g - base < w.text_len ? g - base : ~0ull; };
        if (algo == KREP_RA_AVX512 && !pl->lines && G >= 64 && (G % 64) < (uint64_t)m - 1)
        {
            const uint64_t ghi = G - G % 64, glo = ghi - 64;
            if (ghi > base && glo < base + w.text_len)
            {
                j.excl_lo = glo > base ? glo - base : 0;
                j.excl_hi = std::min<uint64_t>(ghi - base, w.text_len);
            }
        }
        if (pl->ww && !pl->lines)
        {
            const uint64_t B = algo == KREP_RA_AVX2 ? 32 : algo == KREP_RA_AVX512 ? 64 : algo == KREP_RA_NEON ? 16 : 0;
            if (B && (G % B) >= m)
                j.ww_exempt = to_local(G - G % B);
        }
    }
    if (d_pos && cap && !pl->lines)
    {
        const uint64_t maxc = pl->max_count;
        j.want = maxc;
        if ((algo == KREP_RA_KMP || algo == KREP_RA_MEMCHR) && maxc != SIZE_MAX)
            j.want = maxc + 1;
        j.want = std::min<uint64_t>(j.want, cap);
    }

    HIPCHK(hipSetDevice(pl->device));
    if (time_it) HIPCHK(hipEventRecord(pl->ev0, st));
    LitTotals t;
    int rc;
    if (fam.replay)
        rc = whole ? lit_replay_whole(j, &t) : lit_replay_piece(j, &t);
    else if (fam.need_walk)
        rc = lit_walk(j, fam, &t);
    else if (fam.neon_zero)
        return lit_neon_zero(j, time_it, out);
    else
        rc = lit_plain(j, time_it, &t);
    if (rc)
        return rc;
    return lit_finish(j, time_it, t, out);
}

static int scan_device_impl(krep_gpu_plan_t *pl, const void *d_text, size_t text_len, size_t own_lo, size_t own_hi,
                            size_t global_base, size_t global_len, match_position_t *d_positions, uint64_t position_capacity,
                            void *stream, int time_it, const krep_gpu_seq_carry_t *carry_in, krep_gpu_seq_carry_t *carry_out,
                            krep_gpu_scan_out_t *out)
{
    krep_gpu_scan_out_t tmp;
    if (!out)
        out = &tmp;
    memset(out, 0, sizeof *out);
    if (carry_out)
        *carry_out = carry_in ? *carry_in : krep_gpu_seq_carry_t{};
    if (!pl || (!d_text && text_len))
        return kg::fail("scan_device: bad arguments");
    if (global_len == 0)
        global_len = global_base + text_len;
    if (global_len < global_base + text_len)
        return kg::fail("scan_device: global_len %zu is shorter than global_base + text_len", global_len);
    {
        const hipError_t stale = hipGetLastError();
        if (stale != hipSuccess && getenv("KREP_GPU_DEBUG"))
            fprintf(stderr, "krep-gpu: (debug) cleared stale HIP error: %s\n", hipGetErrorString(stale));
    }
    hipStream_t st = (hipStream_t)stream;
    if (pl->unsupported)
        return kg::fail("%s", pl->unsupported);
    if (kg::inject(3))
        return kg::fail("injected failure: kernel launch");
    Window w{(const uint8_t *)d_text, text_len, own_lo, own_hi, global_base, global_len};
    if (pl->ref_algo == KREP_RA_AHO_CORASICK)
        return scan_ac(pl, w, d_positions, position_capacity, st, time_it, carry_in, carry_out, out);
    if (pl->sp.num_patterns != 1)
        return kg::fail("scan_device: no pattern");
    const int algo = mirror_effective(pl->ref_algo, &pl->sp, global_len);
    return scan_literal(pl, algo, w, d_positions, position_capacity, st, time_it, carry_in, carry_out, out);
}
extern "C" int krep_gpu_scan_device_ex(krep_gpu_plan_t *pl, const void *d_text, size_t text_len, size_t own_lo, size_t own_hi,
                                       size_t global_base, size_t global_len, match_position_t *d_positions,
                                       uint64_t position_capacity, void *stream, int time_it, krep_gpu_scan_out_t *out)
{
    return scan_device_impl(pl, d_text, text_len, own_lo, own_hi, global_base, global_len, d_positions, position_capacity, stream,
                            time_it, nullptr, nullptr, out);
}
extern "C" int krep_gpu_scan_device_seq(krep_gpu_plan_t *pl, const void *d_text, size_t text_len, size_t own_lo, size_t own_hi,
                                        size_t global_base, size_t global_len, match_position_t *d_positions,
                                        uint64_t position_capacity, void *stream, int time_it,
                                        const krep_gpu_seq_carry_t *carry_in, krep_gpu_seq_carry_t *carry_out,
                                        krep_gpu_scan_out_t *out)
{
    krep_gpu_seq_carry_t zero{};
    return scan_device_impl(pl, d_text, text_len, own_lo, own_hi, global_base, global_len, d_positions, position_capacity, stream,
                            time_it, carry_in ? carry_in : &zero, carry_out, out);
}
extern "C" int krep_gpu_replay_tail(krep_gpu_plan_t *pl, const void *d_tail, size_t tail_len, size_t global_len, void *stream,
                                    const krep_gpu_seq_carry_t *carry_true, const krep_gpu_seq_carry_t *piece,
                                    krep_gpu_seq_carry_t *carry_out, uint64_t *lines)
{
    if (!pl || !d_tail || !piece || !lines)
        return kg::fail("krep_gpu_replay_tail: NULL argument");
    if (pl->unsupported)
        return kg::fail("%s", pl->unsupported);
    if (pl->ref_algo == KREP_RA_AHO_CORASICK || pl->sp.num_patterns != 1)
        return kg::fail("krep_gpu_replay_tail: not a single-literal plan");
    const int algo = mirror_effective(pl->ref_algo, &pl->sp, global_len);
    const Family fam = family_of(algo, pl->only_matching, pl->lines, pl->ww, pl->track, pl->max_count, pl->has_border, pl->m, pl->has_newline);
    if (!fam.replay)
        return kg::fail("krep_gpu_replay_tail: %s under these parameters has no end-of-text replay", krep_gpu_algorithm_name(algo));
    if (!piece->local_lines)
        return kg::fail("krep_gpu_replay_tail: the record is not that of the piece that ends the text");
    const uint64_t G = global_len, need = std::min<uint64_t>(G, 512);
    if (tail_len > G || tail_len < need)
        return kg::fail("krep_gpu_replay_tail: the tail must hold the last %llu bytes of the text", (unsigned long long)need);
    const krep_gpu_seq_carry_t zero{};
    const krep_gpu_seq_carry_t co = kg::fold_carry(carry_true ? *carry_true : zero, *piece);
    uint64_t extra = 0;
    hipStream_t st = (hipStream_t)stream;
    if (replay_from_record(pl, algo, co, rebased(d_tail, G - tail_len), G - tail_len ? G - tail_len + 1 : 0, G, st, &extra))
        return 2;
    HIPCHK(hipStreamSynchronize(st));
    if (carry_out)
        *carry_out = co;
    *lines = (piece->local_lines - 1) + extra;
    return 0;
}
extern "C" int krep_gpu_scan_device(krep_gpu_plan_t *pl, const void *d_text, size_t text_len, size_t own_lo, size_t own_hi,
                                    size_t global_base, match_position_t *d_positions, uint64_t position_capacity,
                                    void *stream, int time_it, krep_gpu_scan_out_t *out)
{
    return krep_gpu_scan_device_ex(pl, d_text, text_len, own_lo, own_hi, global_base, 0, d_positions, position_capacity, stream,
                                   time_it, out);
}

extern "C" uint64_t krep_gpu_combine_line_counts(const krep_gpu_scan_out_t *s, int n)
{
    uint64_t total = 0;
    bool open = false;
    for (int i = 0; i < n; ++i)
    {
        total += s[i].line_count;
        if (open && s[i].head_line_hit)
            total -= 1;
        open = s[i].has_newline ? (s[i].tail_line_hit != 0) : (open || s[i].head_line_hit != 0);
    }
    return total;
}
```

krep_amd/csrc/kg_single.hip:

```cpp
#include <hip/hip_runtime.h>
#include <algorithm>
#include <atomic>
#include <cstdlib>
#include "kg_common.h"
#include "kg_device.h"
#include "kg_internal.h"
#include "kg_tickets.h"

namespace kg {

#ifndef KG_S1_UPT
#define KG_S1_UPT 4
#endif
constexpr u32 kUptStd = KG_S1_UPT;
static_assert(kUptStd >= 1 && kUptStd <= 4, "flush() derives a record's unit from three boundaries");
constexpr u32 kRingStd = 1024u * kUptStd;
constexpr u32 kRingDense = 8192u;
constexpr u32 kRingDensest = 16384u;
constexpr u64 kReady = kTkReady;
constexpr u64 kUnitBytes1 = (u64)kRoundsBig * kSegBytes;

__device__ __noinline__ uint4 s_load16_guarded(const uint8_t *text, u64 text_len, u64 off)
{
    u32 w[4] = {0, 0, 0, 0};
    for (u32 b = 0; b < 16; ++b)
        if (off + b < text_len)
            w[b >> 2] |= (u32)text[off + b] << (8 * (b & 3u));
    return make_uint4(w[0], w[1], w[2], w[3]);
}


template <bool CI, u32 kUpt, u32 kRing, int WPE, bool SET, bool MULTI = false, bool BDRAW = false, bool WW = false>
__global__ __launch_bounds__(kBlock, WPE) void single_fused(const LitArgs a, u64 *__restrict__ agg, u64 *__restrict__ pref,
                                                            const u64 n_tickets)
{
    static_assert(!MULTI || !SET, "a byte set is a single-byte scan");
    static_assert(kUpt >= 1 && kUpt <= 4, "ticket shape");
    auto rwrap = [](const u32 x) -> u32 {
        if constexpr ((kRing & (kRing - 1u)) == 0u)
            return x & (kRing - 1u);
        else
            return x >= kRing ? x - kRing : x;
    };
    const u32 lane = lane_id();
    const u32 wave = __builtin_amdgcn_readfirstlane(threadIdx.x >> 6);
    const u64 n_units = a.num_tiles * kWavesPerBlk;

    bool resolver = false;
    if (wave == 0)
    {
        u64 r = 1;
        if (lane == 0)
            r = __hip_atomic_fetch_add(&a.ctr->pad[0], 1ull, __ATOMIC_RELAXED, __HIP_MEMORY_SCOPE_AGENT);
        resolver = rfl64(r) == 0ull;
    }
    extern __shared__ __attribute__((aligned(16))) unsigned short s_ring[];
    u64 *s_draw = reinterpret_cast<u64 *>(s_ring + (size_t)kWavesPerBlk * kRing);
    bool bmode = false;
    if constexpr (BDRAW)
    {
        if (threadIdx.x == 0)
            s_draw[1] = resolver ? 1ull : 0ull;
        __syncthreads();
        bmode = s_draw[1] == 0ull;
    }
    if (resolver)
    {
        tk_resolve(agg, pref, n_tickets, a.ctr, lane);
        return;
    }
    unsigned short *ring = s_ring + (size_t)wave * kRing;
    const u64 hi_match = a.own_hi < a.text_len - a.m + 1 ? a.own_hi : a.text_len - a.m + 1;

    bool pend = false;
    u64 pend_t = 0;
    u32 pend_at = 0, pend_cnt = 0, pend_c0 = 0, pend_c1 = 0, pend_c2 = 0;
    u32 wp = 0;
    bool overflowed = false;

    auto flush = [&]() __attribute__((always_inline)) {
#ifdef KG_S1_NOWAIT
        const u64 first = pend_t * 1400ull;
#else
        const u64 first = tk_wait_prefix(pref, pend_t, a.ctr, lane);
#endif
        const u64 tbase = a.anchor + pend_t * (u64)kUpt * kUnitBytes1 + a.global_base;
        const u32 b1 = pend_c0, b2 = pend_c0 + pend_c1, b3 = pend_c0 + pend_c1 + pend_c2;
        const u32 pad = (u32)(first & 7ull);
        for (u32 g = lane; g < pend_cnt + pad; g += 64u)
        {
            if (g < pad)
                continue;
            const u32 i = g - pad;
            const u32 off = ring[rwrap(pend_at + i)];
            const u32 unit = (i >= b1 ? 1u : 0u) + (i >= b2 ? 1u : 0u) + (i >= b3 ? 1u : 0u);
            const u64 idx = first + i;
#ifdef KG_S1_NOSTORE
            if (idx == ~0ull)
#else
            if (idx < a.pos_cap)
#endif
            {
                const u64 st = tbase + (u64)unit * kUnitBytes1 + off, en = st + (MULTI ? (u64)a.m : 1ull);
                typedef u32 u32x4 __attribute__((ext_vector_type(4)));
                const u32x4 rec = {(u32)st, (u32)(st >> 32), (u32)en, (u32)(en >> 32)};
#ifdef KG_S1_PLAIN_STORES
                *reinterpret_cast<u32x4 *>(a.positions + 2 * idx) = rec;
#else
                __builtin_nontemporal_store(rec, reinterpret_cast<u32x4 *>(a.positions + 2 * idx));
#endif
            }
        }
        pend = false;
    };

    constexpr u32 kRoundsPerTicket = kUpt * kRoundsBig;
    constexpr u64 kTicketBytes = (u64)kUpt * kUnitBytes1;
    const u64 scan_end = a.anchor + n_units * kUnitBytes1 < a.text_len ? a.anchor + n_units * kUnitBytes1 : a.text_len;
    const u64 fb = (a.text_len - kSegBytes) & ~15ull;
    auto issue = [&](uint4 (&X)[kCells], u64 seg) __attribute__((always_inline)) {
        const uint4 *src = reinterpret_cast<const uint4 *>(a.text + seg) + lane;
#pragma unroll
        for (int j = 0; j < kCells; ++j)
        {
            typedef u32 u32x4 __attribute__((ext_vector_type(4)));
            const u32x4 v = __builtin_nontemporal_load(reinterpret_cast<const u32x4 *>(src + j * kWave));
            X[j] = make_uint4(v.x, v.y, v.z, v.w);
        }
    };
    u32 cnt = 0;
    u32 at = 0, room = 0;
    auto process = [&](uint4 (&X)[kCells], u64 seg, bool have, u32 rr) __attribute__((always_inline)) {
        if (!have)
        {
            if (seg + kSegBytes <= a.text_len)
                issue(X, seg);
            else
            {
#pragma unroll
                for (int j = 0; j < kCells; ++j)
                    X[j] = s_load16_guarded(a.text, a.text_len, seg + (u64)j * kCellBytes + (u64)lane * 16u);
            }
        }
        const bool interior = seg >= a.own_lo && seg + kSegBytes <= hi_match;
        u32 aft0 = 0, aft1 = 0;
        if (MULTI)
        {
            const u64 q = seg + kSegBytes;
            if (q + 8 <= a.text_len)
            {
                const uint2 t2 = *reinterpret_cast<const uint2 *>(a.text + q);
                aft0 = __builtin_amdgcn_readfirstlane(t2.x);
                aft1 = __builtin_amdgcn_readfirstlane(t2.y);
            }
            else
            {
                u32 w2[2] = {0, 0};
                for (u32 b = 0; b < 8; ++b)
                    if (q + b < a.text_len)
                        w2[b >> 2] |= (u32)a.text[q + b] << (8 * (b & 3u));
                aft0 = __builtin_amdgcn_readfirstlane(w2[0]);
                aft1 = __builtin_amdgcn_readfirstlane(w2[1]);
            }
        }
#pragma unroll
        for (int j = 0; j < kCells; ++j)
        {
            const u32 D[4] = {X[j].x, X[j].y, X[j].z, X[j].w};
            u32 m16 = 0;
            if (MULTI)
            {
                const u32 n0 = __shfl_down(D[0], 1), n1 = __shfl_down(D[1], 1);
                const u32 e0 = j + 1 < kCells ? __builtin_amdgcn_readfirstlane(X[j + 1 < kCells ? j + 1 : j].x) : aft0;
                const u32 e1 = j + 1 < kCells ? __builtin_amdgcn_readfirstlane(X[j + 1 < kCells ? j + 1 : j].y) : aft1;
                const u32 W[6] = {D[0], D[1], D[2], D[3], lane == 63u ? e0 : n0, lane == 63u ? e1 : n1};
                auto A = [&](int k) -> u32 {
                    return ((k & 3) == 0) ? W[k >> 2] : __builtin_amdgcn_alignbyte(W[(k >> 2) + 1], W[k >> 2], (u32)(k & 3));
                };
#pragma unroll
                for (int k = 0; k < 16; ++k)
                    m16 |= ((((CI ? (A(k) | a.l0) : A(k)) ^ a.p0) & a.k0) == 0u) ? (1u << k) : 0u;
                if (a.m > 4u && __ballot(m16 != 0u))
                {
#pragma unroll
                    for (int k = 0; k < 16; ++k)
                        if ((((CI ? (A(k + 4) | a.l1) : A(k + 4)) ^ a.p1) & a.k1) != 0u)
                            m16 &= ~(1u << k);
                }
                if (WW && __ballot(m16 != 0u))
                {
                    const u32 below = __shfl_up(D[3], 1);
                    const u64 lb = seg + (u64)j * kCellBytes + (u64)lane * 16u;
                    auto pick = [&](u32 i) -> u32 {
                        const u32 q = i >> 2;
                        const u32 w = q == 0u ? below : q == 1u ? W[0] : q == 2u ? W[1] : q == 3u ? W[2] : q == 4u ? W[3] : q == 5u ? W[4] : W[5];
                        return (w >> (8u * (i & 3u))) & 0xffu;
                    };
                    u32 rest = m16;
                    while (rest)
                    {
                        const u32 k = __builtin_ctz(rest);
                        rest &= rest - 1u;
                        const u64 p = lb + k;
                        bool left = is_wordc(pick(k + 3u));
                        if (lane == 0u && k == 0u)
                            left = p > 0 && is_wordc(a.text[p - 1]);
                        if (p == a.ww_exempt_left)
                            left = false;
                        if (left || is_wordc(pick(k + a.m + 4u)))
                            m16 &= ~(1u << k);
                    }
                }
            }
            else if (SET)
            {
#pragma unroll
                for (int w = 0; w < 4; ++w)
                {
                    u32 f = eq_bytes(CI ? (D[w] | a.set_l[0]) : D[w], a.set_p[0]);
                    if (a.set_n > 1u) f |= eq_bytes(CI ? (D[w] | a.set_l[1]) : D[w], a.set_p[1]);
                    if (a.set_n > 2u) f |= eq_bytes(CI ? (D[w] | a.set_l[2]) : D[w], a.set_p[2]);
                    if (a.set_n > 3u) f |= eq_bytes(CI ? (D[w] | a.set_l[3]) : D[w], a.set_p[3]);
                    m16 |= movemask4(f) << (4 * w);
                }
            }
            else
            {
#pragma unroll
                for (int w = 0; w < 4; ++w)
                    m16 |= movemask4(eq_bytes(CI ? (D[w] | a.l0) : D[w], a.p0)) << (4 * w);
            }
            if (!interior)
            {
                const u64 lbase = seg + (u64)j * kCellBytes + (u64)lane * 16u;
                const u32 klo = a.own_lo > lbase ? (u32)((a.own_lo - lbase) < 16 ? (a.own_lo - lbase) : 16) : 0u;
                const u32 khi = hi_match > lbase ? (u32)((hi_match - lbase) < 16 ? (hi_match - lbase) : 16) : 0u;
                m16 &= khi > klo ? (((1u << khi) - 1u) & ~((1u << klo) - 1u)) : 0u;
// ... 69 lines not shown
                break;
            process(A, seg, haveA, rr);
            haveA = false;
            if ((rr & (kRoundsBig - 1u)) == kRoundsBig - 1u)
            {
                const u32 cu = cnt - before, uu = rr / kRoundsBig;
                before = cnt;
                units_done = uu + 1u;
                c0 = uu == 0u ? cu : c0;
                c1 = uu == 1u ? cu : c1;
                c2 = uu == 2u ? cu : c2;
            }
        }
        {
            const u32 cu = cnt - before;
            c0 = units_done == 0u ? cu : c0;
            c1 = units_done == 1u ? cu : c1;
            c2 = units_done == 2u ? cu : c2;
        }
        if (cnt > room)
            overflowed = true;
        if (lane == 0 && mine)
            __hip_atomic_store(&agg[t], (u64)cnt | kReady, __ATOMIC_RELAXED, __HIP_MEMORY_SCOPE_AGENT);
        const u64 tn = draw();
        haveA = tn < n_tickets && a.anchor + tn * kTicketBytes + kSegBytes <= a.text_len;
        issue(A, haveA ? a.anchor + tn * kTicketBytes : fb);
        if (pend)
            flush();
        if (cnt && cnt <= room)
        {
            pend = true;
            pend_t = t;
            pend_at = at;
            pend_cnt = cnt;
            pend_c0 = c0;
            pend_c1 = c1;
            pend_c2 = c2;
            wp = rwrap(at + cnt);
        }
        else
            pend_cnt = 0;
        t = tn;
    }
    if (pend)
        flush();
    if (overflowed && lane == 0)
        atomicAdd(&a.ctr->overflow_units, 1ull);
}

int g_s1_force_grid = 0;
template <bool CI, u32 UPT, u32 RING, int WPE, bool SET, bool MULTI, bool BDRAW = false, bool WW = false>
static hipError_t launch_fused(const LitArgs &a, u64 *agg, u64 *pref, u64 n_tickets, u32 num_cu, hipStream_t st)
{
    constexpr size_t kLds = (size_t)kWavesPerBlk * RING * sizeof(unsigned short) + (BDRAW ? 16u : 0u);
    static std::atomic<u32> s_bpc[64];
    int dev = 0;
    (void)hipGetDevice(&dev);
    const u32 slot = (u32)dev < 64u ? (u32)dev : 63u;
    u32 bpc = s_bpc[slot].load(std::memory_order_acquire);
    if (!bpc)
    {
        if (kLds > 64 * 1024)
        {
            const hipError_t e = hipFuncSetAttribute(reinterpret_cast<const void *>(&single_fused<CI, UPT, RING, WPE, SET, MULTI, BDRAW, WW>),
                                                     hipFuncAttributeMaxDynamicSharedMemorySize, (int)kLds);
            if (e != hipSuccess)
                return e;
        }
        int n = 0;
        if (hipOccupancyMaxActiveBlocksPerMultiprocessor(&n, single_fused<CI, UPT, RING, WPE, SET, MULTI, BDRAW, WW>, kBlock, kLds) != hipSuccess || n < 1)
        {
            (void)hipGetLastError();
            n = 1;
        }
        bpc = (u32)std::min(n, 4);
        s_bpc[slot].store(bpc, std::memory_order_release);
    }
    const u64 want = (n_tickets + kWavesPerBlk - 1) / kWavesPerBlk + 1;
    u32 grid = (u32)std::max<u64>(1, std::min<u64>(want, (u64)num_cu * bpc));
    if (g_s1_force_grid > 0)
        grid = std::min<u32>(grid, (u32)g_s1_force_grid);
    hipLaunchKernelGGL((single_fused<CI, UPT, RING, WPE, SET, MULTI, BDRAW, WW>), dim3(grid), dim3(kBlock), kLds, st, a, agg, pref, n_tickets);
    return hipGetLastError();
}

constexpr u32 kRingMid = 6144u;
static u32 shape_upt(int shape) { return shape == 0 ? kUptStd : (shape <= 2 ? 2u : 1u); }
static u32 shape_ring(int shape) { return shape == 0 ? kRingStd : (shape == 5 ? kRingDensest : ((shape & 1) ? kRingMid : kRingDense)); }
static uint64_t single_fused_tickets(uint64_t n_units, int shape) { return (n_units + shape_upt(shape) - 1) / shape_upt(shape); }
static uint64_t single_fused_scratch_words(uint64_t n_tickets) { return 2 * n_tickets; }
double single_fused_max_density(int shape)
{
    return 0.4 * (double)shape_ring(shape) / ((double)shape_upt(shape) * (double)kUnitBytes1);
}

template <bool CI, bool SET, bool MULTI = false, bool WW = false>
static hipError_t launch_shape(const LitArgs &a, u64 *agg, u64 *pref, u64 n_tickets, u32 num_cu, int shape, hipStream_t st)
{
    static_assert(kFusedShapeMax == 5, "six shapes");
    if (shape == 0) return launch_fused<CI, kUptStd, kRingStd, 4, SET, MULTI, false, WW>(a, agg, pref, n_tickets, num_cu, st);
    if (shape == 1) return launch_fused<CI, 2u, kRingMid, 3, SET, MULTI, false, WW>(a, agg, pref, n_tickets, num_cu, st);
    if (shape == 2) return launch_fused<CI, 2u, kRingDense, 2, SET, MULTI, false, WW>(a, agg, pref, n_tickets, num_cu, st);
#ifndef KG_S1_NO_BDRAW
    constexpr bool kB = true;
#else
    constexpr bool kB = false;
#endif
    if (shape == 3) return launch_fused<CI, 1u, kRingMid, 3, SET, MULTI, kB, WW>(a, agg, pref, n_tickets, num_cu, st);
    if (shape == 4) return launch_fused<CI, 1u, kRingDense, 2, SET, MULTI, kB, WW>(a, agg, pref, n_tickets, num_cu, st);
    return launch_fused<CI, 1u, kRingDensest, 1, SET, MULTI, false, WW>(a, agg, pref, n_tickets, num_cu, st);
}

hipError_t launch_single_fused(const LitArgs &a, unsigned long long *d_agg, unsigned long long *d_pref, uint64_t n_tickets,
                               uint32_t num_cu, int shape, hipStream_t st)
{
    const bool ci = (a.flags & F_CI) != 0, set = a.set_n != 0u;
    if (!set && a.m > 1u)
    {
        if (a.m > 8u)
            return hipErrorInvalidValue;
        if (a.flags & F_WW)
            return ci ? launch_shape<true, false, true, true>(a, d_agg, d_pref, n_tickets, num_cu, shape, st)
                      : launch_shape<false, false, true, true>(a, d_agg, d_pref, n_tickets, num_cu, shape, st);
        return ci ? launch_shape<true, false, true>(a, d_agg, d_pref, n_tickets, num_cu, shape, st)
                  : launch_shape<false, false, true>(a, d_agg, d_pref, n_tickets, num_cu, shape, st);
    }
    if (set)
        return ci ? launch_shape<true, true>(a, d_agg, d_pref, n_tickets, num_cu, shape, st)
                  : launch_shape<false, true>(a, d_agg, d_pref, n_tickets, num_cu, shape, st);
    return ci ? launch_shape<true, false>(a, d_agg, d_pref, n_tickets, num_cu, shape, st)
              : launch_shape<false, false>(a, d_agg, d_pref, n_tickets, num_cu, shape, st);
}

int single_fused_shape_for(double density, double margin, int start)
{
    int shape = start;
    while (shape < kFusedShapeMax && margin * density > single_fused_max_density(shape))
        ++shape;
    return shape;
}
bool single_fused_reopens(uint64_t total, uint64_t span)
{
    return span && (double)total / (double)span < 0.5 * single_fused_max_density(kFusedShapeMax);
}
int single_fused_run(const LitArgs &a, uint64_t n_units, uint64_t span, PostScratch &post, Counters *d_ctr, Counters *h_ctr,
                     uint32_t num_cu, int *shape_io, hipEvent_t ev_end, hipStream_t st, bool count_launch)
{
    for (;;)
    {
        const int shape = *shape_io;
        const uint64_t n_tk = single_fused_tickets(n_units, shape);
        const size_t tk_bytes = single_fused_scratch_words(n_tk) * sizeof(unsigned long long);
        HIPCHK(grow_scratch(post.tk_cap, n_tk, n_tk, {dev_buf(post.d_tk, tk_bytes)}));
        HIPCHK(hipMemsetAsync(d_ctr, 0, sizeof(Counters), st));
        HIPCHK(hipMemsetAsync(post.d_tk, 0, tk_bytes, st));
        HIPCHK(launch_single_fused(a, post.d_tk, post.d_tk + n_tk, n_tk, num_cu, shape, st));
        if (count_launch)
            g_fused1_launches.fetch_add(1);
        if (ev_end) HIPCHK(hipEventRecord(ev_end, st));
        HIPCHK(hipMemcpyAsync(h_ctr, d_ctr, sizeof(Counters), hipMemcpyDeviceToHost, st));
        HIPCHK(hipStreamSynchronize(st));
        const double density = (double)h_ctr->total / (double)span;
        if (!h_ctr->overflow_units)
        {
            if (shape > 0 && density < 0.5 * single_fused_max_density(shape - 1))
                *shape_io = shape - 1;
            return 0;
        }
        const int next = shape < kFusedShapeMax ? single_fused_shape_for(density, 1.0, shape + 1) : shape;
        if (next == shape || density > single_fused_max_density(next) || h_ctr->total == 0)
            return kFusedGaveUp;
        *shape_io = next;
    }
}

}
```

krep_amd/csrc/kg_tickets.h:

```cpp
#pragma once
#include <hip/hip_runtime.h>
#include "kg_common.h"
#include "kg_device.h"

namespace kg {

constexpr unsigned long long kTkReady = 1ull << 63;
constexpr uint32_t kTkSpinLimit = 1u << 24;
constexpr uint32_t kTkResolveChunk = 8;

__device__ __forceinline__ void tk_resolve(unsigned long long *__restrict__ agg, unsigned long long *__restrict__ pref,
                                           const unsigned long long n_tickets, Counters *ctr, const uint32_t lane)
{
    u64 running = 0, base = 0;
    u32 spins = 0;
    while (base < n_tickets)
    {
        const u64 mine = base + (u64)lane * kTkResolveChunk;
        u64 v[kTkResolveChunk];
        u32 lead = 0, nvalid = 0;
        bool run = true;
#pragma unroll
        for (u32 k = 0; k < kTkResolveChunk; ++k)
        {
            const bool valid = mine + k < n_tickets;
            v[k] = valid ? __hip_atomic_load(&agg[mine + k], __ATOMIC_RELAXED, __HIP_MEMORY_SCOPE_AGENT) : 0ull;
            nvalid += valid ? 1u : 0u;
            run = run && valid && (v[k] & kTkReady);
            lead += run ? 1u : 0u;
        }
        const u64 open = __ballot(lead != nvalid);
        const u32 f = open ? (u32)__builtin_ctzll(open) : 64u;
        const u32 take = lane < f ? nvalid : (lane == f ? lead : 0u);
        u64 s = 0;
#pragma unroll
        for (u32 k = 0; k < kTkResolveChunk; ++k)
            s += k < take ? (v[k] & ~kTkReady) : 0ull;
        u64 incl = s;
        u32 tincl = take;
#pragma unroll
        for (int o = 1; o < 64; o <<= 1)
        {
            const u64 up = __shfl_up(incl, o);
            const u32 tup = __shfl_up(tincl, o);
            if (lane >= (u32)o)
            {
                incl += up;
                tincl += tup;
            }
        }
        u64 e = running + incl - s;
#pragma unroll
        for (u32 k = 0; k < kTkResolveChunk; ++k)
        {
            if (k < take)
                __hip_atomic_store(&pref[mine + k], e | kTkReady, __ATOMIC_RELAXED, __HIP_MEMORY_SCOPE_AGENT);
            e += k < take ? (v[k] & ~kTkReady) : 0ull;
        }
        const u32 published = __shfl(tincl, 63);
        running += __shfl(incl, 63);
        base += published;
        if (published)
            spins = 0;
        else
        {
            if (++spins > kTkSpinLimit)
            {
                if (lane == 0)
                    atomicAdd(&ctr->overflow_units, 1ull);
                for (u64 t = base + lane; t < n_tickets; t += 64)
                    __hip_atomic_store(&pref[t], kTkReady, __ATOMIC_RELAXED, __HIP_MEMORY_SCOPE_AGENT);
                return;
            }
            __builtin_amdgcn_s_sleep(8);
        }
    }
    if (lane == 0)
        ctr->total = running;
}

__device__ __forceinline__ unsigned long long tk_wait_prefix(const unsigned long long *__restrict__ pref, const unsigned long long t,
                                                              Counters *ctr, const uint32_t lane)
{
    u64 p = 0;
    if (lane == 0)
    {
        for (uint32_t spins = 0;; ++spins)
        {
            p = __hip_atomic_load(&pref[t], __ATOMIC_RELAXED, __HIP_MEMORY_SCOPE_AGENT);
            if (p & kTkReady)
                break;
            if (spins > 2u * kTkSpinLimit)
            {
                atomicAdd(&ctr->overflow_units, 1ull);
                p = kTkReady;
                break;
            }
            __builtin_amdgcn_s_sleep(4);
        }
    }
    return rfl64(p) & ~kTkReady;
}

__device__ __forceinline__ unsigned long long tk_wait_prefix_lane(const unsigned long long *__restrict__ pref, const unsigned long long t,
                                                                   Counters *ctr)
{
    u64 p = 0;
    for (uint32_t spins = 0;; ++spins)
    {
        p = __hip_atomic_load(&pref[t], __ATOMIC_RELAXED, __HIP_MEMORY_SCOPE_AGENT);
        if (p & kTkReady)
            break;
        if (spins > 2u * kTkSpinLimit)
        {
            atomicAdd(&ctr->overflow_units, 1ull);
            p = kTkReady;
            break;
        }
        __builtin_amdgcn_s_sleep(4);
    }
    return p & ~kTkReady;
}

}
```

krep_amd/engine.py:

```python
from __future__ import annotations

import ctypes as C
import os

import numpy as np

from . import abi

HERE = os.path.dirname(os.path.abspath(__file__))
LIB_PATH = os.path.join(HERE, "lib", "libkrep_gpu.so")


class KrepGpuError(RuntimeError):
    pass


class Engine:

    def __init__(self, path: str = LIB_PATH):
        path = os.environ.get("KREP_GPU_LIB", path)
        if not os.path.exists(path):
            raise KrepGpuError(f"{path} is missing: build it with `python -m krep_amd.build` "
                               "(hipcc --offload-arch=gfx950); there is no CPU fallback")
        if not os.environ.get("KREP_GPU_NO_TORCH"):
            try:
                import torch
            except Exception:
                pass
        L = self.lib = C.CDLL(path)
        sf = [C.POINTER(abi.SearchParams), C.c_void_p, C.c_size_t, C.POINTER(abi.MatchResult)]
        for n in ("krep_gpu_literal_search", "krep_gpu_aho_corasick_search"):
            getattr(L, n).restype = C.c_uint64
            getattr(L, n).argtypes = sf
        L.krep_gpu_select_search_algorithm.restype = C.c_void_p
        L.krep_gpu_select_search_algorithm.argtypes = [C.POINTER(abi.SearchParams)]
        L.search_buffer.restype = C.c_int
        L.search_buffer.argtypes = [C.POINTER(abi.SearchParams), C.c_void_p, C.c_size_t, C.c_int, C.c_int,
                                    C.POINTER(abi.MatchResult), C.POINTER(C.c_uint64)]
        L.search_buffer_ex.restype = C.c_int
        L.search_buffer_ex.argtypes = [C.POINTER(abi.SearchParams), C.c_void_p, C.c_size_t, C.POINTER(abi.Config), C.c_int,
                                       C.POINTER(abi.MatchResult), C.POINTER(C.c_uint64)]
        L.krep_gpu_can_accelerate.restype = C.c_int
        L.krep_gpu_can_accelerate.argtypes = [C.POINTER(abi.SearchParams)]
        L.krep_gpu_config_default.restype = None
        L.krep_gpu_config_default.argtypes = [C.POINTER(abi.Config)]
        L.krep_gpu_set_thread_config.restype = None
        L.krep_gpu_set_thread_config.argtypes = [C.POINTER(abi.Config)]
        L.krep_gpu_set_stream_chunk.restype = None
        L.krep_gpu_set_stream_chunk.argtypes = [C.c_size_t]
        L.krep_gpu_release_device_resources.restype = None
        L.krep_gpu_plan_create_ex.restype = C.c_void_p
        L.krep_gpu_plan_create_ex.argtypes = [C.POINTER(abi.SearchParams), C.POINTER(abi.Config)]
        L.krep_gpu_scan_device_ex.restype = C.c_int
        L.krep_gpu_scan_device_ex.argtypes = [C.c_void_p, C.c_void_p, C.c_size_t, C.c_size_t, C.c_size_t, C.c_size_t, C.c_size_t,
                                              C.c_void_p, C.c_uint64, C.c_void_p, C.c_int, C.POINTER(abi.ScanOut)]
        L.krep_gpu_scan_device_seq.restype = C.c_int
        L.krep_gpu_scan_device_seq.argtypes = [C.c_void_p, C.c_void_p, C.c_size_t, C.c_size_t, C.c_size_t, C.c_size_t, C.c_size_t,
                                               C.c_void_p, C.c_uint64, C.c_void_p, C.c_int, C.POINTER(abi.SeqCarry),
                                               C.POINTER(abi.SeqCarry), C.POINTER(abi.ScanOut)]
        L.krep_gpu_split_mode.restype = C.c_int
        L.krep_gpu_split_mode.argtypes = [C.POINTER(abi.SearchParams), C.c_size_t]
        L.krep_gpu_match_result_init.restype = C.POINTER(abi.MatchResult)
        L.krep_gpu_match_result_init.argtypes = [C.c_uint64]
        L.krep_gpu_match_result_free.restype = None
        L.krep_gpu_match_result_free.argtypes = [C.POINTER(abi.MatchResult)]
        L.krep_gpu_plan_create.restype = C.c_void_p
        L.krep_gpu_plan_create.argtypes = [C.POINTER(abi.SearchParams), C.c_int, C.c_int]
        L.krep_gpu_plan_destroy.restype = None
        L.krep_gpu_plan_destroy.argtypes = [C.c_void_p]
        L.krep_gpu_plan_ref_algo.restype = C.c_int
        L.krep_gpu_plan_ref_algo.argtypes = [C.c_void_p]
        L.krep_gpu_scan_device.restype = C.c_int
        L.krep_gpu_scan_device.argtypes = [C.c_void_p, C.c_void_p, C.c_size_t, C.c_size_t, C.c_size_t, C.c_size_t,
                                           C.c_void_p, C.c_uint64, C.c_void_p, C.c_int, C.POINTER(abi.ScanOut)]
        L.krep_gpu_generate.restype = C.c_int
        L.krep_gpu_generate.argtypes = [C.c_void_p, C.c_size_t, C.c_size_t, C.c_int, C.c_uint64, C.c_void_p,
                                        C.c_size_t, C.c_uint64, C.c_void_p]
        L.krep_gpu_generate_host.restype = None
        L.krep_gpu_generate_host.argtypes = [C.c_void_p, C.c_size_t, C.c_size_t, C.c_int, C.c_uint64, C.c_void_p,
                                             C.c_size_t, C.c_uint64]
        L.krep_gpu_combine_line_counts.restype = C.c_uint64
        L.krep_gpu_combine_line_counts.argtypes = [C.POINTER(abi.ScanOut), C.c_int]
        L.krep_gpu_mirror_select.restype = C.c_int
        L.krep_gpu_mirror_select.argtypes = [C.POINTER(abi.SearchParams), C.c_size_t]
        L.krep_gpu_algorithm_name.restype = C.c_char_p
        L.krep_gpu_algorithm_name.argtypes = [C.c_int]
        L.krep_gpu_order_by_start.restype = C.c_int
        L.krep_gpu_order_by_start.argtypes = [C.c_void_p, C.c_uint64, C.c_size_t, C.c_void_p]
        L.krep_gpu_line_numbers.restype = C.c_int
        L.krep_gpu_line_numbers.argtypes = [C.c_void_p, C.c_size_t, C.c_void_p, C.c_uint64, C.c_void_p, C.c_void_p]
        if hasattr(L, "krep_gpu_format_lines"):
            L.krep_gpu_matching_lines.restype = C.c_int
            L.krep_gpu_matching_lines.argtypes = [C.c_void_p, C.c_size_t, C.c_void_p, C.c_uint64, C.c_uint64, C.c_void_p, C.c_void_p,
                                                  C.c_uint64, C.POINTER(abi.LinesOut), C.c_void_p]
            L.krep_gpu_format_lines.restype = C.c_int
            L.krep_gpu_format_lines.argtypes = [C.c_void_p, C.c_size_t, C.c_void_p, C.c_uint64, C.c_uint64, C.c_char_p, C.c_size_t,
                                                C.c_void_p, C.c_size_t, C.POINTER(abi.LinesOut), C.c_void_p]
        if hasattr(L, "krep_gpu_format_lines_ex"):
            L.krep_gpu_format_lines_ex.restype = C.c_int
            L.krep_gpu_format_lines_ex.argtypes = [C.c_void_p, C.c_size_t, C.c_void_p, C.c_uint64, C.c_uint64, C.POINTER(abi.LineFormat),
                                                   C.c_void_p, C.c_size_t, C.POINTER(abi.LinesOut), C.c_void_p]
        if hasattr(L, "krep_gpu_format_lines_window"):
            L.krep_gpu_format_lines_window.restype = C.c_int
            L.krep_gpu_format_lines_window.argtypes = [C.c_void_p, C.c_size_t, C.POINTER(abi.LinesWindow), C.c_void_p, C.c_uint64,
                                                       C.c_uint64, C.POINTER(abi.LineFormat), C.c_void_p, C.c_size_t,
                                                       C.POINTER(abi.LinesWindowOut), C.c_void_p]
        if hasattr(L, "krep_gpu_format_matches"):
            L.krep_gpu_format_matches.restype = C.c_int
            L.krep_gpu_format_matches.argtypes = [C.c_void_p, C.c_size_t, C.c_void_p, C.c_uint64, C.c_uint64, C.POINTER(abi.MatchFormat),
                                                  C.c_void_p, C.c_size_t, C.POINTER(abi.MatchesOut), C.c_void_p]
        if hasattr(L, "krep_gpu_format_matches_window"):
            L.krep_gpu_format_matches_window.restype = C.c_int
            L.krep_gpu_format_matches_window.argtypes = [C.c_void_p, C.c_size_t, C.POINTER(abi.MatchesWindow), C.c_void_p, C.c_uint64,
                                                         C.c_uint64, C.POINTER(abi.MatchFormat), C.c_void_p, C.c_size_t,
                                                         C.POINTER(abi.MatchesWindowOut), C.c_void_p]
        for n in ("krep_gpu_set_reference_simd", "krep_gpu_set_only_matching", "krep_gpu_set_force_no_simd",
                  "krep_gpu_set_algo_override", "krep_gpu_debug_force_rounds", "krep_gpu_debug_force_stage_cap",
                  "krep_gpu_set_result_order", "krep_gpu_set_device", "krep_gpu_set_num_gpus", "krep_gpu_debug_inject_failure"):
            getattr(L, n).restype = None
            getattr(L, n).argtypes = [C.c_int]
        L.krep_gpu_get_reference_simd.restype = C.c_int
        L.krep_gpu_comm_unique_id.restype = C.c_int
        L.krep_gpu_comm_unique_id.argtypes = [C.c_void_p]
        L.krep_gpu_comm_init_rank.restype = C.c_int
        L.krep_gpu_comm_init_rank.argtypes = [C.c_void_p, C.c_int, C.c_int, C.c_int]
        L.krep_gpu_comm_allreduce_u64.restype = C.c_int
        L.krep_gpu_comm_allreduce_u64.argtypes = [C.POINTER(C.c_uint64), C.c_int]
        L.krep_gpu_comm_allreduce_device_u64.restype = C.c_int
        L.krep_gpu_comm_allreduce_device_u64.argtypes = [C.c_void_p, C.c_int, C.c_void_p]
        L.krep_gpu_comm_destroy.restype = None
        L.krep_gpu_rccl_calls.restype = C.c_uint64
        L.krep_gpu_rccl_version.restype = C.c_int
        L.krep_gpu_debug_force_single_grid.restype = None
        L.krep_gpu_debug_force_single_grid.argtypes = [C.c_int]
        L.krep_gpu_debug_single_failovers.restype = C.c_uint64
        L.krep_gpu_debug_single_launches.restype = C.c_uint64
        L.krep_gpu_debug_tiny_launches.restype = C.c_uint64
        L.krep_gpu_debug_chain_fixups.restype = None
        L.krep_gpu_debug_chain_fixups.argtypes = [C.POINTER(C.c_uint64), C.POINTER(C.c_uint64)]
        L.krep_gpu_debug_tiny_dense_launches.restype = C.c_uint64
        if hasattr(L, "krep_gpu_debug_anchor_info"):
            L.krep_gpu_debug_anchored_launches.restype = C.c_uint64
            L.krep_gpu_debug_literal_dma_launches.restype = C.c_uint64
            L.krep_gpu_debug_runs_launches.restype = C.c_uint64
            L.krep_gpu_debug_anchor_info.restype = C.c_int
            L.krep_gpu_debug_anchor_info.argtypes = [C.c_void_p, C.POINTER(C.c_int), C.POINTER(C.c_uint32), C.POINTER(C.c_double),
                                                     C.POINTER(C.c_double)]
        if hasattr(L, "krep_gpu_debug_literal_dma_one_pass_launches"):
            L.krep_gpu_debug_literal_dma_one_pass_launches.restype = C.c_uint64
            L.krep_gpu_debug_literal_dma_one_pass_failovers.restype = C.c_uint64
            L.krep_gpu_debug_force_literal_dma_grid.restype = None
            L.krep_gpu_debug_force_literal_dma_grid.argtypes = [C.c_int]
        if hasattr(L, "krep_gpu_alloc_placed"):
            L.krep_gpu_alloc_placed.restype = C.c_int
            L.krep_gpu_alloc_placed.argtypes = [C.c_int, C.c_size_t, C.c_size_t, C.c_int, C.POINTER(C.c_void_p), C.POINTER(C.c_void_p),
                                                C.POINTER(abi.Placement)]
            L.krep_gpu_free_placed.restype = C.c_int
            L.krep_gpu_free_placed.argtypes = [C.c_int, C.c_void_p]
        if hasattr(L, "krep_gpu_debug_literal_dma_state"):
            L.krep_gpu_debug_literal_dma_state.restype = C.c_int
            L.krep_gpu_debug_literal_dma_state.argtypes = [C.c_void_p, C.POINTER(C.c_int), C.POINTER(C.c_int), C.POINTER(C.c_double)]
        if hasattr(L, "krep_gpu_debug_anchor_measured"):
            L.krep_gpu_debug_anchor_measured.restype = C.c_int
            L.krep_gpu_debug_anchor_measured.argtypes = [C.c_void_p, C.POINTER(C.c_double), C.POINTER(C.c_int)]
        L.krep_gpu_last_shard_info.restype = None
        L.krep_gpu_last_shard_info.argtypes = [C.POINTER(abi.ShardInfo)]
        L.krep_gpu_available.restype = C.c_int
        L.krep_gpu_unavailable_reason.restype = C.c_char_p
        L.krep_gpu_last_status.restype = C.c_int
        L.krep_gpu_set_cpu_fallback.restype = None
        L.krep_gpu_set_cpu_fallback.argtypes = [C.c_void_p]
        L.krep_gpu_worthwhile.restype = C.c_int
        L.krep_gpu_worthwhile.argtypes = [C.POINTER(abi.SearchParams), C.c_size_t]
        L.krep_gpu_worthwhile_ex.restype = C.c_int
        L.krep_gpu_worthwhile_ex.argtypes = [C.POINTER(abi.SearchParams), C.c_size_t, C.c_int]
        L.krep_gpu_cost_estimate.restype = C.c_int
        L.krep_gpu_cost_estimate.argtypes = [C.POINTER(abi.SearchParams), C.c_size_t, C.c_int, C.POINTER(abi.Cost)]
        L.krep_gpu_get_cost_rates.restype = None
        L.krep_gpu_get_cost_rates.argtypes = [C.POINTER(abi.CostRates)]
        L.krep_gpu_set_cost_rates.restype = None
        L.krep_gpu_set_cost_rates.argtypes = [C.POINTER(abi.CostRates)]
        L.krep_gpu_set_min_text_bytes.restype = None
        L.krep_gpu_set_min_text_bytes.argtypes = [C.c_size_t]
        L.krep_gpu_device_count.restype = C.c_int
        L.krep_gpu_last_error.restype = C.c_char_p
        L.krep_gpu_clear_error.restype = None
        L.krep_gpu_version.restype = C.c_char_p

    def set_reference_simd(self, level: int):
        self.lib.krep_gpu_set_reference_simd(level)

    def set_only_matching(self, on: bool):
        self.lib.krep_gpu_set_only_matching(int(on))

    def set_force_no_simd(self, on: bool):
        self.lib.krep_gpu_set_force_no_simd(int(on))

    def set_algo_override(self, a: int):
        self.lib.krep_gpu_set_algo_override(a)

    def force_rounds(self, r: int):
        self.lib.krep_gpu_debug_force_rounds(r)

    def force_single_grid(self, blocks: int):
        self.lib.krep_gpu_debug_force_single_grid(blocks)

    def single_failovers(self) -> int:
        return int(self.lib.krep_gpu_debug_single_failovers())

    def single_launches(self) -> int:
        return int(self.lib.krep_gpu_debug_single_launches())

    def chain_fixups(self):
        a, b = C.c_uint64(0), C.c_uint64(0)
        self.lib.krep_gpu_debug_chain_fixups(C.byref(a), C.byref(b))
        return int(a.value), int(b.value)

    def tiny_dense_launches(self) -> int:
        return int(self.lib.krep_gpu_debug_tiny_dense_launches())

    def runs_launches(self) -> int:
        return int(self.lib.krep_gpu_debug_runs_launches())

    def literal_dma_launches(self) -> int:
        return int(self.lib.krep_gpu_debug_literal_dma_launches())

    def literal_dma_one_pass_launches(self) -> int:
        return int(self.lib.krep_gpu_debug_literal_dma_one_pass_launches())

    def literal_dma_one_pass_failovers(self) -> int:
        return int(self.lib.krep_gpu_debug_literal_dma_one_pass_failovers())

    def force_literal_dma_grid(self, blocks: int):
        self.lib.krep_gpu_debug_force_literal_dma_grid(blocks)

    def alloc_placed(self, text_bytes: int, record_bytes: int, tries: int = 3, device: int = 0):
        t, r, info = C.c_void_p(0), C.c_void_p(0), abi.Placement()
        if self.lib.krep_gpu_alloc_placed(device, text_bytes, record_bytes, tries, C.byref(t), C.byref(r), C.byref(info)):
            raise KrepGpuError("krep_gpu_alloc_placed failed: " + self.last_error())
        return int(t.value), int(r.value or 0), info

    def free_placed(self, d_text: int, device: int = 0):
        if self.lib.krep_gpu_free_placed(device, C.c_void_p(d_text)):
            raise KrepGpuError("krep_gpu_free_placed failed: " + self.last_error())

    def anchored_launches(self) -> int:
        return int(self.lib.krep_gpu_debug_anchored_launches())

    def tiny_launches(self) -> int:
        return int(self.lib.krep_gpu_debug_tiny_launches())

    def force_stage_cap(self, c: int):
        self.lib.krep_gpu_debug_force_stage_cap(c)

    def default_config(self) -> abi.Config:
        c = abi.Config()
        self.lib.krep_gpu_config_default(C.byref(c))
        return c

    def set_thread_config(self, cfg: "abi.Config | None"):
        self.lib.krep_gpu_set_thread_config(C.byref(cfg) if cfg is not None else None)

    def set_stream_chunk(self, nbytes: int):
        self.lib.krep_gpu_set_stream_chunk(nbytes)

    def can_accelerate(self, params: abi.Params) -> bool:
        return bool(self.lib.krep_gpu_can_accelerate(params.ref))

    def select(self, params: abi.Params):
        return self.lib.krep_gpu_select_search_algorithm(params.ref)

    def available(self) -> bool:
        return bool(self.lib.krep_gpu_available())

    def unavailable_reason(self) -> str:
        return (self.lib.krep_gpu_unavailable_reason() or b"").decode()

    def last_status(self) -> int:
        return int(self.lib.krep_gpu_last_status())

    def set_cpu_fallback(self, selector_address):
        self.lib.krep_gpu_set_cpu_fallback(C.c_void_p(selector_address) if selector_address else None)

    def worthwhile(self, params: abi.Params, text_len: int) -> bool:
        return bool(self.lib.krep_gpu_worthwhile(params.ref, text_len))

    def worthwhile_ex(self, params: abi.Params, text_len: int, cpu_threads: int) -> bool:
        return bool(self.lib.krep_gpu_worthwhile_ex(params.ref, text_len, cpu_threads))

    def cost_estimate(self, params: abi.Params, text_len: int, cpu_threads: int = 0) -> "abi.Cost":
        c = abi.Cost()
        if self.lib.krep_gpu_cost_estimate(params.ref, text_len, cpu_threads, C.byref(c)):
            raise KrepGpuError("krep_gpu_cost_estimate failed")
        return c

    def cost_rates(self) -> "abi.CostRates":
        r = abi.CostRates()
        self.lib.krep_gpu_get_cost_rates(C.byref(r))
        return r

    def set_cost_rates(self, rates: "abi.CostRates | None"):
        self.lib.krep_gpu_set_cost_rates(C.byref(rates) if rates is not None else None)

    def inject_failure(self, kind: int):
        self.lib.krep_gpu_debug_inject_failure(kind)

    def set_num_gpus(self, n: int):
        self.lib.krep_gpu_set_num_gpus(n)

    def comm_unique_id(self) -> bytes:
        buf = C.create_string_buffer(128)
        if self.lib.krep_gpu_comm_unique_id(buf):
            raise KrepGpuError("krep_gpu_comm_unique_id failed: " + self.last_error())
        return buf.raw

    def comm_init_rank(self, id128: bytes, nranks: int, rank: int, device: int):
        assert len(id128) == 128
        buf = C.create_string_buffer(id128, 128)
        if self.lib.krep_gpu_comm_init_rank(buf, nranks, rank, device):
            raise KrepGpuError("krep_gpu_comm_init_rank failed: " + self.last_error())

    def comm_allreduce(self, values):
        arr = (C.c_uint64 * len(values))(*[int(v) for v in values])
        if self.lib.krep_gpu_comm_allreduce_u64(arr, len(values)):
            raise KrepGpuError("krep_gpu_comm_allreduce_u64 failed: " + self.last_error())
        return [int(v) for v in arr]

    def comm_destroy(self):
        self.lib.krep_gpu_comm_destroy()

    def rccl_calls(self) -> int:
        return int(self.lib.krep_gpu_rccl_calls())

    def rccl_version(self) -> int:
        return int(self.lib.krep_gpu_rccl_version())

    def last_shard_info(self) -> "abi.ShardInfo":
        info = abi.ShardInfo()
        self.lib.krep_gpu_last_shard_info(C.byref(info))
        return info

    def split_mode(self, params: abi.Params, text_len: int) -> int:
        return int(self.lib.krep_gpu_split_mode(params.ref, text_len))

    def release_device_resources(self):
        self.lib.krep_gpu_release_device_resources()

    def mirror_select(self, params: abi.Params, text_len: int) -> int:
        return int(self.lib.krep_gpu_mirror_select(params.ref, text_len))

    def last_error(self) -> str:
        return (self.lib.krep_gpu_last_error() or b"").decode()

    def device_count(self) -> int:
        return int(self.lib.krep_gpu_device_count())

    def set_result_order(self, by_start: bool):
        self.lib.krep_gpu_set_result_order(int(by_start))

    def order_by_start(self, d_positions: int, n: int, text_len: int, stream: int = 0):
        if self.lib.krep_gpu_order_by_start(C.c_void_p(d_positions), n, text_len, C.c_void_p(stream)):
            raise KrepGpuError("krep_gpu_order_by_start failed: " + self.last_error())

    def line_numbers(self, d_text: int, text_len: int, d_positions: int, n: int, d_lines: int, stream: int = 0):
        if self.lib.krep_gpu_line_numbers(C.c_void_p(d_text), text_len, C.c_void_p(d_positions), n, C.c_void_p(d_lines),
                                          C.c_void_p(stream)):
            raise KrepGpuError("krep_gpu_line_numbers failed: " + self.last_error())

    def matching_lines(self, d_text: int, text_len: int, d_positions: int, n: int, max_lines: int = abi.SIZE_MAX, d_lines: int = 0,
                       d_first_record: int = 0, line_capacity: int = 0, stream: int = 0) -> "abi.LinesOut":
        out = abi.LinesOut()
        if self.lib.krep_gpu_matching_lines(C.c_void_p(d_text), text_len, C.c_void_p(d_positions), n, max_lines,
                                            C.c_void_p(d_lines) if d_lines else None,
                                            C.c_void_p(d_first_record) if d_first_record else None, line_capacity, C.byref(out),
                                            C.c_void_p(stream) if stream else None):
            raise KrepGpuError("krep_gpu_matching_lines failed: " + self.last_error())
        return out

    def format_lines(self, d_text: int, text_len: int, d_positions: int, n: int, max_lines: int = abi.SIZE_MAX, prefix: bytes = b"",
                     d_out: int = 0, out_capacity: int = 0, stream: int = 0) -> "abi.LinesOut":
        out = abi.LinesOut()
        if self.lib.krep_gpu_format_lines(C.c_void_p(d_text), text_len, C.c_void_p(d_positions), n, max_lines, prefix, len(prefix),
                                          C.c_void_p(d_out) if d_out else None, out_capacity, C.byref(out),
                                          C.c_void_p(stream) if stream else None):
            raise KrepGpuError("krep_gpu_format_lines failed: " + self.last_error())
        return out

# ... 284 lines not shown
                    if whole is not None:
                        assert whole.lines.lines == 1 and not whole.incomplete_line_start1
                        if lines_left != abi.SIZE_MAX:
                            lines_left -= 1
        return b"".join(parts)

    def grep_only_matching(self, d_text: int, n: int, filename=None, max_count=None, color=False, stream: int = 0) -> bytes:
        import torch
        eng = self.eng
        if not self.only_matching:
            raise KrepGpuError("grep_only_matching: the plan was not created with only_matching=True (the match set of -o differs)")
        limit = int(self.params.s.max_count)
        if max_count is not None:
            limit = min(limit, int(max_count))
        if limit == 0 or n == 0:
            return b""
        found = self.scan(d_text, n, stream=stream)
        cap = int(max(found.count, found.total_matches))
        if cap == 0:
            return b""
        pos = torch.empty(2 * (cap + 1), dtype=torch.int64, device="cuda")
        out = self.scan(d_text, n, d_positions=pos.data_ptr(), capacity=cap + 1, stream=stream)
        if out.overflow:
            raise KrepGpuError("grep_only_matching: the record list outgrew the count of the scan before it")
        m = min(int(out.stored), limit)
        if m == 0:
            return b""
        if self.params.s.num_patterns > 1:
            eng.order_by_start(pos.data_ptr(), m, n, stream)
        name = b"" if filename is None else (filename if isinstance(filename, bytes) else str(filename).encode())
        fmt = match_format(name if filename is not None else None, color)
        longest = max(int(x) for x in self.params.s.pattern_lens[: self.params.s.num_patterns])
        per_item = fmt.prefix_len + fmt.before_number_len + fmt.after_number_len + fmt.after_match_len + 20 + 2 + longest
        guess = m * per_item + 4096
        buf = torch.empty(guess, dtype=torch.uint8, device="cuda")
        res = eng.format_matches(d_text, n, pos.data_ptr(), m, limit, fmt, buf.data_ptr(), guess, stream)
        if res.overflow:
            buf = torch.empty(int(res.out_bytes), dtype=torch.uint8, device="cuda")
            res = eng.format_matches(d_text, n, pos.data_ptr(), m, limit, fmt, buf.data_ptr(), int(res.out_bytes), stream)
            assert not res.overflow
        return buf[: int(res.out_bytes)].cpu().numpy().tobytes()

    def grep_only_matching_pieces(self, text, piece_bytes: int, filename=None, color=False) -> bytes:
        import torch
        eng, s = self.eng, self.params.s
        if not self.only_matching:
            raise KrepGpuError("grep_only_matching_pieces: the plan was not created with only_matching=True (the match set of -o "
                               "differs)")
        if isinstance(text, torch.Tensor):
            host = text.contiguous().view(torch.uint8).reshape(-1)
        else:
            a = np.ascontiguousarray(text, dtype=np.uint8).reshape(-1) if isinstance(text, np.ndarray) \
                else np.frombuffer(bytes(text), dtype=np.uint8)
            host = torch.from_numpy(a if a.flags.writeable else a.copy())
        total = int(host.numel())
        piece_bytes = int(piece_bytes)
        if piece_bytes <= 0:
            raise KrepGpuError("grep_only_matching_pieces: piece_bytes must be positive")
        limit = int(s.max_count)
        multi = s.num_patterns > 1
        if multi and limit != abi.SIZE_MAX:
            raise KrepGpuError("grep_only_matching_pieces: a multi-pattern plan with max_count: the cut to the first max_count "
                               "records in emission order needs the whole record list")
        cfg = eng.default_config()
        cfg.only_matching = 1
        eng.set_thread_config(cfg)
        try:
            mode = eng.split_mode(self.params, total)
        finally:
            eng.set_thread_config(None)
        if mode == abi.SPLIT_WHOLE:
            raise KrepGpuError("grep_only_matching_pieces: this search takes the whole text in one window (krep_gpu_split_mode)")
        if limit == 0 or total == 0:
            return b""
        longest = max(int(x) for x in s.pattern_lens[: s.num_patterns]) if s.num_patterns else int(s.pattern_len)
        name = None if filename is None else (filename if isinstance(filename, bytes) else str(filename).encode())
        fmt = match_format(name, bool(color))
        per_item = fmt.prefix_len + fmt.before_number_len + fmt.after_number_len + fmt.after_match_len + 20 + 2 + longest
        buf = torch.empty(1 + piece_bytes + longest + 64, dtype=torch.uint8, device="cuda")
        view, step = memoryview(host.numpy()), 1 << 20
        last_nl1, at = 0, total
        while at > 0 and not last_nl1:
            lo_ = max(at - step, 0)
            k = bytes(view[lo_:at]).rfind(b"\n")
            last_nl1 = lo_ + k + 1 if k >= 0 else 0
            at = lo_
        sched = StaleSchedule(limit, last_nl1)
        parts = []
        chain = {"nl": 0, "stale": 0}

        dev = {"out": torch.empty(4096, dtype=torch.uint8, device="cuda"), "one": torch.empty(longest + 64, dtype=torch.uint8, device="cuda"),
               "rec": torch.empty(2, dtype=torch.int64, device="cuda")}

        def grown(key, nbytes):
            if dev[key].numel() < nbytes:
                dev[key] = torch.empty(max(nbytes, 2 * dev[key].numel()), dtype=torch.uint8, device="cuda")
            return dev[key]

        def fmt_call(d_text, blen, base, count_to, d_pos, n, rule):
            win = abi.MatchesWindow(base, total, count_to, chain["nl"], last_nl1, chain["stale"], int(rule))
            out = grown("out", n * per_item + 4096)
            res = eng.format_matches_window(d_text, blen, win, d_pos, n, abi.SIZE_MAX, fmt, out.data_ptr(), out.numel())
            if res.matches.overflow:
                out = grown("out", int(res.matches.out_bytes))
                res = eng.format_matches_window(d_text, blen, win, d_pos, n, abi.SIZE_MAX, fmt, out.data_ptr(), out.numel())
                assert not res.matches.overflow
            if res.matches.out_bytes:
                parts.append(out[: int(res.matches.out_bytes)].cpu().numpy().tobytes())
            return res

        def held_calls(records, rule):
            for start, end in records:
                stop = max(min(end, total), start + 1)
                one = grown("one", stop - start + 64)
                one[: stop - start].copy_(host[start:stop])
                dev["rec"].copy_(torch.tensor([start, end], dtype=torch.int64))
                chain["stale"] = int(fmt_call(one.data_ptr(), stop - start, start, start, dev["rec"].data_ptr(), 1, rule).stale_line)

        carry = None
        for lo in range(0, total, piece_bytes):
            left = limit - sched.count
            if left <= 0:
                break
            hi = min(lo + piece_bytes, total)
            base, end = max(lo - 1, 0), min(hi + longest, total)
            buf[: end - base].copy_(host[base:end])
            d_text, blen = buf.data_ptr(), end - base
            found, carry_out = self.scan_seq(d_text, blen, lo - base, hi - base, base, global_len=total, carry_in=carry)
            cap, m, pos = int(max(found.count, found.total_matches)), 0, None
            if cap:
                pos = torch.empty(2 * (cap + 1), dtype=torch.int64, device="cuda")
                got, carry_out = self.scan_seq(d_text, blen, lo - base, hi - base, base, pos.data_ptr(), cap + 1, global_len=total,
                                               carry_in=carry)
                if got.overflow:
                    raise KrepGpuError("grep_only_matching_pieces: the record list outgrew the count of the scan before it")
                m = min(int(got.stored), left)
                if multi and m:
                    eng.order_by_start(pos.data_ptr(), m, total)
            carry = carry_out
            flush, now, rule = sched.add(m, lambda: pos[: 2 * m].view(-1, 2).cpu().tolist())
            held_calls(flush, rule)
            res = fmt_call(d_text, blen, base, hi - 1 if hi < total else total, pos.data_ptr() if now else 0, now, rule)
            chain["nl"], chain["stale"] = int(res.newlines_before_count_to), int(res.stale_line)
        flush, rule = sched.end()
        held_calls(flush, rule)
        return b"".join(parts)

    def anchor_info(self):
        st, mv, r0, r1 = C.c_int(0), C.c_uint32(0), C.c_double(0), C.c_double(0)
        if self.eng.lib.krep_gpu_debug_anchor_info(self.h, C.byref(st), C.byref(mv), C.byref(r0), C.byref(r1)):
            return None
        return int(st.value), int(mv.value), float(r0.value), float(r1.value)

    def literal_dma_state(self):
        a, b, r = C.c_int(0), C.c_int(0), C.c_double(0)
        if self.eng.lib.krep_gpu_debug_literal_dma_state(self.h, C.byref(a), C.byref(b), C.byref(r)):
            return None
        return bool(a.value), bool(b.value), float(r.value)

    def split_state(self) -> int:
        f = self.eng.lib.krep_gpu_debug_split_state
        f.restype = C.c_int
        f.argtypes = [C.c_void_p]
        return int(f(self.h))

    def anchor_measured(self):
        m, r = C.c_double(0), C.c_int(0)
        if self.eng.lib.krep_gpu_debug_anchor_measured(self.h, C.byref(m), C.byref(r)):
            return None
        return float(m.value), int(r.value)

    def scan_seq(self, d_text: int, text_len: int, own_lo, own_hi, global_base=0, d_positions: int = 0, capacity: int = 0,
                 global_len=0, carry_in: "abi.SeqCarry | None" = None):
        out, cout = abi.ScanOut(), abi.SeqCarry()
        rc = self.eng.lib.krep_gpu_scan_device_seq(self.h, C.c_void_p(d_text), text_len, own_lo, own_hi, global_base, global_len,
                                                   C.c_void_p(d_positions) if d_positions else None, capacity, None, 0,
                                                   C.byref(carry_in) if carry_in is not None else None, C.byref(cout),
                                                   C.byref(out))
        if rc:
            raise KrepGpuError("krep_gpu_scan_device_seq failed: " + self.eng.last_error())
        return out, cout

    def close(self):
        if self.h:
            self.eng.lib.krep_gpu_plan_destroy(self.h)
            self.h = None

    def __del__(self):
        try:
            self.close()
        except Exception:
            pass


COLOR_RESET, COLOR_FILENAME, COLOR_SEPARATOR = b"\033[0m", b"\033[1;38;5;81m", b"\033[38;5;244m"
COLOR_LINE_NUMBER, COLOR_MATCH = b"\033[1;38;5;111m", b"\033[1;38;5;222m"
COLOR_TEXT = b"\033[38;5;252m"
STALE_AFTER = 10


def match_format(filename: "bytes | None" = None, color: bool = False) -> "abi.MatchFormat":
    if not color:
        return abi.MatchFormat(b"" if filename is None else filename + b":")
    prefix = b"" if filename is None else COLOR_FILENAME + filename + COLOR_RESET + COLOR_SEPARATOR + b":"
    return abi.MatchFormat(prefix, COLOR_LINE_NUMBER, COLOR_RESET + COLOR_MATCH, COLOR_RESET)


def line_format(filename: "bytes | None" = None, color: bool = False) -> "abi.LineFormat":
    if not color:
        return abi.LineFormat(b"" if filename is None else filename + b":")
    prefix = COLOR_TEXT if filename is None else COLOR_FILENAME + filename + COLOR_RESET + COLOR_SEPARATOR + b":" + COLOR_TEXT
    return abi.LineFormat(prefix, COLOR_MATCH, COLOR_TEXT, COLOR_RESET)


class StaleSchedule:

    def __init__(self, max_count: int, last_newline1: int):
        self.count, self.held, self.last_newline1 = 0, [], int(last_newline1)
        self.rule = False if (max_count <= STALE_AFTER or not last_newline1) else None

    def add(self, m: int, fetch):
        self.count += int(m)
        if self.rule is None and self.count > STALE_AFTER:
            self.rule = True
        if self.rule is not None:
            flush, self.held = self.held, []
            return flush, int(m), self.rule
        recs = [(int(s), int(e)) for s, e in fetch()] if m else []
        now = 0 if self.held else sum(1 for s, _ in recs if s < self.last_newline1)
        self.held += recs[now:]
        return [], now, False

    def end(self):
        if self.rule is None:
            self.rule = False
        flush, self.held = self.held, []
        return flush, self.rule


_engine = None


def load() -> Engine:
    global _engine
    if _engine is None:
        _engine = Engine()
    return _engine
```

Measured before the change: 6634 GB/s.

## Tag ticket generations to skip per-call memset and write counters to host directly

Replaces the single ready bit in the decoupled-lookback ticket words with a 16-bit generation tag, so the aggregate and prefix arrays no longer need zeroing before every one-pass literal scan. Only the first call, or a wrap after 0x7FFF generations, pays for a memset. The last finishing wave also copies the counters straight into mapped host memory and resets them on the device, which removes the per-call device-to-host memcpy. In exchange it adds a grid-wide completion atomic, a stamp check on the host, and cap the values at 48 bits, falling back to the memset path for larger buffers.

After: 6554 GB/s. 1.2% lower.

```diff
diff --git a/include/krep_gpu_debug.h b/include/krep_gpu_debug.h
--- a/include/krep_gpu_debug.h
+++ b/include/krep_gpu_debug.h
@@ -22,6 +22,8 @@
 uint64_t krep_gpu_debug_literal_dma_one_pass_launches(void);
 uint64_t krep_gpu_debug_literal_dma_one_pass_failovers(void);
 void krep_gpu_debug_force_literal_dma_grid(int blocks);
+uint64_t krep_gpu_debug_literal_dma_one_pass_memsets(void);
+int krep_gpu_debug_literal_dma_set_next_tag(krep_gpu_plan_t *plan, uint32_t tag);
 int krep_gpu_debug_literal_dma_state(const krep_gpu_plan_t *plan, int *looked, int *barred, double *pass_rate);
 uint64_t krep_gpu_debug_runs_launches(void);
 int krep_gpu_debug_split_state(const krep_gpu_plan_t *plan);
diff --git a/krep_amd/csrc/kg_ac.hip b/krep_amd/csrc/kg_ac.hip
--- a/krep_amd/csrc/kg_ac.hip
+++ b/krep_amd/csrc/kg_ac.hip
@@ -1135,6 +1135,7 @@
         const u64 n_tk = (f.num_tiles + f.upt - 1) / f.upt;
         const size_t tk_bytes = 2 * n_tk * sizeof(unsigned long long);
         HIPCHK(grow_scratch(c.post->tk_cap, n_tk, n_tk, {dev_buf(c.post->d_tk, tk_bytes)}));
+        c.post->tk_tag = 0;
         f.tk_agg = c.post->d_tk; f.tk_pref = c.post->d_tk + n_tk; f.n_tk = n_tk; f.stage_cap = 0;
         HIPCHK(hipSetDevice(t->device));
         if (c.time_it) HIPCHK(hipEventRecord(c.ev0, c.st));
diff --git a/krep_amd/csrc/kg_ac_tiny.hip b/krep_amd/csrc/kg_ac_tiny.hip
--- a/krep_amd/csrc/kg_ac_tiny.hip
+++ b/krep_amd/csrc/kg_ac_tiny.hip
@@ -62,7 +62,7 @@
             resolver = wave_fetch_add(&a.ctr->pad[0], 1ull, lane) == 0ull;
         if (resolver)
         {
-            tk_resolve(a.tk_agg, a.tk_pref, a.n_tk, a.ctr, lane);
+            tk_resolve(a.tk_agg, a.tk_pref, a.n_tk, a.ctr, lane, kTkTagLegacy);
             return;
         }
     }
@@ -88,7 +88,7 @@
     u32 u_c0 = 0, u_c1 = 0, u_c2 = 0, u_before = 0, pend_c0 = 0, pend_c1 = 0, pend_c2 = 0;
     auto dwrap = [](const u32 x) -> u32 { return x >= kDenseRing ? x - kDenseRing : x; };
     auto flush_dense = [&](const u32 l4) __attribute__((always_inline)) {
-        const u64 first = tk_wait_prefix(a.tk_pref, pend_t, a.ctr, lane);
+        const u64 first = tk_wait_prefix(a.tk_pref, pend_t, a.ctr, lane, kTkTagLegacy);
         const u64 tbase = a.anchor + pend_t * (u64)a.upt * kAcUnitBytes + a.global_base + 1u;
         const u32 b1 = pend_c0, b2 = pend_c0 + pend_c1, b3 = pend_c0 + pend_c1 + pend_c2;
         const u32 pad = (u32)(first & 7ull);
@@ -133,7 +133,7 @@
         }
     };
     auto flush = [&](const u32 l4, const u32 l5) __attribute__((always_inline)) {
-        const u64 first = tk_wait_prefix(a.tk_pref, pend_t, a.ctr, lane);
+        const u64 first = tk_wait_prefix(a.tk_pref, pend_t, a.ctr, lane, kTkTagLegacy);
         const u64 tbase = a.anchor + pend_t * (u64)a.upt * kAcUnitBytes + a.global_base;
         u64 run = first;
         for (u32 b0 = 0; b0 < pend_items; b0 += 64u)
diff --git a/krep_amd/csrc/kg_config.hip b/krep_amd/csrc/kg_config.hip
--- a/krep_amd/csrc/kg_config.hip
+++ b/krep_amd/csrc/kg_config.hip
@@ -253,4 +253,5 @@
 extern "C" uint64_t krep_gpu_debug_literal_dma_one_pass_launches(void) { return kg::g_lit_dma1p_launches.load(); }
 extern "C" uint64_t krep_gpu_debug_literal_dma_one_pass_failovers(void) { return kg::g_lit_dma1p_failovers.load(); }
 extern "C" void krep_gpu_debug_force_literal_dma_grid(int blocks) { kg::g_lit_dma1p_force_grid = blocks < 0 ? 0 : blocks; }
+extern "C" uint64_t krep_gpu_debug_literal_dma_one_pass_memsets(void) { return kg::g_lit_dma1p_memsets.load(); }
 extern "C" uint64_t krep_gpu_debug_runs_launches(void) { return kg::g_runs_launches.load(); }
diff --git a/krep_amd/csrc/kg_internal.h b/krep_amd/csrc/kg_internal.h
--- a/krep_amd/csrc/kg_internal.h
+++ b/krep_amd/csrc/kg_internal.h
@@ -71,11 +71,12 @@
 extern std::atomic<uint64_t> g_runs_launches;
 extern std::atomic<uint64_t> g_lit_dma_launches;
 hipError_t launch_literal_dma_one_pass(const LitArgs &a, unsigned long long *d_agg, unsigned long long *d_pref, uint64_t n_tickets,
-                                       uint32_t num_cu, hipStream_t st);
+                                       uint32_t tag, Counters *d_slot, uint32_t num_cu, hipStream_t st);
 uint32_t lit_dma_one_pass_list();
 extern std::atomic<uint64_t> g_lit_dma1p_launches;
 extern std::atomic<uint64_t> g_lit_dma1p_failovers;
 extern int g_lit_dma1p_force_grid;
+extern std::atomic<uint64_t> g_lit_dma1p_memsets;
 
 struct PostScratch;
 constexpr int kFusedShapeMax = 5;
@@ -102,6 +103,8 @@
     uint64_t keep_cap = 0;
     unsigned long long *d_tk = nullptr;
     uint64_t tk_cap = 0;
+    uint32_t tk_tag = 0;
+    bool tk_dirty = false;
 };
 void post_free(PostScratch &s);
 int post_reserve(PostScratch &s, uint64_t n_units, uint64_t stage_words);
diff --git a/krep_amd/csrc/kg_literal_dma.hip b/krep_amd/csrc/kg_literal_dma.hip
--- a/krep_amd/csrc/kg_literal_dma.hip
+++ b/krep_amd/csrc/kg_literal_dma.hip
@@ -1,6 +1,7 @@
 #include <hip/hip_runtime.h>
 #include <algorithm>
 #include <atomic>
+#include <cstddef>
 #include <cstdlib>
 #include "kg_common.h"
 #include "kg_device.h"
@@ -23,7 +24,8 @@
 uint32_t lit_dma_one_pass_list() { return kOpHits; }
 
 template <int KIND, bool MASKED, bool CI, bool ONEP>
-__global__ __launch_bounds__(kBlock, 2) void lit_scan_dma(const LitArgs a, u64 *__restrict__ agg, const u64 *__restrict__ pref, const u64 n_tickets)
+__global__ __launch_bounds__(kBlock, 2) void lit_scan_dma(const LitArgs a, u64 *__restrict__ agg, const u64 *__restrict__ pref, const u64 n_tickets,
+                                                          const u32 tag, Counters *__restrict__ slot)
 {
     extern __shared__ __attribute__((aligned(16))) uint8_t d_smem[];
     __shared__ u64 s_info_all[kWavesPerBlk][ONEP ? 1u : kDmaPark];
@@ -33,6 +35,22 @@
     __shared__ u32 s_tk_all[kWavesPerBlk][ONEP ? 3u * kOpTk : 1u];
     const u32 lane = lane_id();
     const u32 wave = __builtin_amdgcn_readfirstlane(threadIdx.x >> 6);
+    auto count_out = [&]() __attribute__((always_inline)) {
+        constexpr u32 kWords = (u32)(sizeof(Counters) / sizeof(u64)), kStamp = (u32)(offsetof(Counters, pad) / sizeof(u64)) + 1u;
+        static_assert(kWords <= 64u, "one lane per counter word");
+        u64 *c = reinterpret_cast<u64 *>(a.ctr);
+        u64 out = 0;
+        if (lane == 0)
+            out = __hip_atomic_fetch_add(&c[kStamp], 1ull, __ATOMIC_ACQ_REL, __HIP_MEMORY_SCOPE_AGENT);
+        if (rfl64(out) != (u64)gridDim.x * kWavesPerBlk - 1ull)
+            return;
+        if (lane < kWords)
+        {
+            const u64 v = __hip_atomic_load(&c[lane], __ATOMIC_RELAXED, __HIP_MEMORY_SCOPE_AGENT);
+            __hip_atomic_store(reinterpret_cast<u64 *>(slot) + lane, lane == kStamp ? (u64)tag : v, __ATOMIC_RELAXED, __HIP_MEMORY_SCOPE_SYSTEM);
+            c[lane] = 0ull;
+        }
+    };
     if (ONEP && wave == 0)
     {
         u64 r = 1;
@@ -40,7 +58,8 @@
             r = __hip_atomic_fetch_add(&a.ctr->pad[0], 1ull, __ATOMIC_RELAXED, __HIP_MEMORY_SCOPE_AGENT);
         if (rfl64(r) == 0ull)
         {
-            tk_resolve(agg, const_cast<u64 *>(pref), n_tickets, a.ctr, lane);
+            tk_resolve(agg, const_cast<u64 *>(pref), n_tickets, a.ctr, lane, tag);
+            count_out();
             return;
         }
     }
@@ -117,7 +136,7 @@
     auto flush_records = [&](const u32 n_out) __attribute__((always_inline)) {
         u64 pfx = 0;
         if (lane < n_out)
-            pfx = tk_wait_prefix_lane(pref, (u64)s_tk[3u * lane], a.ctr);
+            pfx = tk_wait_prefix_lane(pref, (u64)s_tk[3u * lane], a.ctr, tag);
         for (u32 i = 0; i < n_out; ++i)
         {
             const u32 t = __builtin_amdgcn_readfirstlane(s_tk[3u * i]), cnt = __builtin_amdgcn_readfirstlane(s_tk[3u * i + 1u]),
@@ -198,7 +217,7 @@
     };
     auto end_ticket = [&](u32 t) __attribute__((always_inline)) {
         if (lane == 0)
-            __hip_atomic_store(&agg[t], (u64)wcnt | kTkReady, __ATOMIC_RELAXED, __HIP_MEMORY_SCOPE_AGENT);
+            __hip_atomic_store(&agg[t], tk_pack(wcnt, tag), __ATOMIC_RELAXED, __HIP_MEMORY_SCOPE_AGENT);
         u32 fresh = 0;
         if (wcnt > kOpHits - used)
             overflowed = true;
@@ -506,6 +525,8 @@
         atomicAdd(&a.ctr->total, acc_total);
     if (lane == 0 && pf_cells)
         atomicAdd(&a.ctr->candidates, (u64)pf_cells);
+    if (ONEP)
+        count_out();
 }
 
 __global__ __launch_bounds__(256) void dma_byte_look(const uint8_t *text, u64 lo, u32 n_cells, u32 b4, u32 fold, unsigned long long *out)
@@ -540,9 +561,10 @@
 std::atomic<uint64_t> g_lit_dma1p_launches{0};
 std::atomic<uint64_t> g_lit_dma1p_failovers{0};
 int g_lit_dma1p_force_grid = 0;
+std::atomic<uint64_t> g_lit_dma1p_memsets{0};
 
 template <int KIND, bool MASKED, bool CI, bool ONEP>
-static hipError_t dma_launch4(const LitArgs &a, u64 *agg, const u64 *pref, u64 n_tickets, u32 num_cu, hipStream_t st)
+static hipError_t dma_launch4(const LitArgs &a, u64 *agg, const u64 *pref, u64 n_tickets, u32 tag, Counters *slot, u32 num_cu, hipStream_t st)
 {
     constexpr u32 lds = kWavesPerBlk * kDmaWaveLds;
     if (const hipError_t e = grant_dynamic_lds<&lit_scan_dma<KIND, MASKED, CI, ONEP>>((int)lds); e != hipSuccess)
@@ -551,28 +573,28 @@
     u32 grid = (u32)std::min<u64>(a.num_tiles, (u64)num_cu * bpc);
     if (ONEP && g_lit_dma1p_force_grid > 0)
         grid = std::min<u32>(grid, (u32)g_lit_dma1p_force_grid);
-    hipLaunchKernelGGL((lit_scan_dma<KIND, MASKED, CI, ONEP>), dim3(grid ? grid : 1), dim3(kBlock), lds, st, a, agg, pref, n_tickets);
+    hipLaunchKernelGGL((lit_scan_dma<KIND, MASKED, CI, ONEP>), dim3(grid ? grid : 1), dim3(kBlock), lds, st, a, agg, pref, n_tickets, tag, slot);
     g_lit_dma_launches.fetch_add(1, std::memory_order_relaxed);
     if (ONEP)
         g_lit_dma1p_launches.fetch_add(1, std::memory_order_relaxed);
     return hipGetLastError();
 }
 template <int KIND, bool MASKED, bool ONEP>
-static hipError_t dma_launch2(const LitArgs &a, u64 *agg, const u64 *pref, u64 n_tickets, u32 num_cu, hipStream_t st)
-{
-    return (a.flags & F_CI) ? dma_launch4<KIND, MASKED, true, ONEP>(a, agg, pref, n_tickets, num_cu, st)
-                            : dma_launch4<KIND, MASKED, false, ONEP>(a, agg, pref, n_tickets, num_cu, st);
+static hipError_t dma_launch2(const LitArgs &a, u64 *agg, const u64 *pref, u64 n_tickets, u32 tag, Counters *slot, u32 num_cu, hipStream_t st)
+{
+    return (a.flags & F_CI) ? dma_launch4<KIND, MASKED, true, ONEP>(a, agg, pref, n_tickets, tag, slot, num_cu, st)
+                            : dma_launch4<KIND, MASKED, false, ONEP>(a, agg, pref, n_tickets, tag, slot, num_cu, st);
 }
 template <bool ONEP>
-static hipError_t dma_launch1(const LitArgs &a, u64 *agg, const u64 *pref, u64 n_tickets, u32 num_cu, hipStream_t st)
+static hipError_t dma_launch1(const LitArgs &a, u64 *agg, const u64 *pref, u64 n_tickets, u32 tag, Counters *slot, u32 num_cu, hipStream_t st)
 {
     if (a.m < 4)
-        return dma_launch2<4, true, ONEP>(a, agg, pref, n_tickets, num_cu, st);
+        return dma_launch2<4, true, ONEP>(a, agg, pref, n_tickets, tag, slot, num_cu, st);
     if (a.m == 4)
-        return dma_launch2<4, false, ONEP>(a, agg, pref, n_tickets, num_cu, st);
+        return dma_launch2<4, false, ONEP>(a, agg, pref, n_tickets, tag, slot, num_cu, st);
     if (a.m < 8)
-        return dma_launch2<8, true, ONEP>(a, agg, pref, n_tickets, num_cu, st);
-    return dma_launch2<8, false, ONEP>(a, agg, pref, n_tickets, num_cu, st);
+        return dma_launch2<8, true, ONEP>(a, agg, pref, n_tickets, tag, slot, num_cu, st);
+    return dma_launch2<8, false, ONEP>(a, agg, pref, n_tickets, tag, slot, num_cu, st);
 }
 
 bool literal_dma_eligible(const LitArgs &a)
@@ -582,15 +604,16 @@
 }
 hipError_t launch_literal_dma(const LitArgs &a, u32 num_cu, hipStream_t st)
 {
-    return dma_launch1<false>(a, nullptr, nullptr, 0, num_cu, st);
-}
-hipError_t launch_literal_dma_one_pass(const LitArgs &a, unsigned long long *d_agg, unsigned long long *d_pref, uint64_t n_tickets, u32 num_cu,
-                                       hipStream_t st)
+    return dma_launch1<false>(a, nullptr, nullptr, 0, kTkTagLegacy, nullptr, num_cu, st);
+}
+hipError_t launch_literal_dma_one_pass(const LitArgs &a, unsigned long long *d_agg, unsigned long long *d_pref, uint64_t n_tickets, uint32_t tag,
+                                       Counters *d_slot, u32 num_cu, hipStream_t st)
 {
     const u64 n_units = a.num_tiles * kWavesPerBlk;
-    if (!(a.flags & F_POS) || !a.upt || n_units >= (1ull << 32) || n_tickets != (n_units + a.upt - 1) / a.upt || (u64)a.upt * kRoundsBig * kSegBytes > (1ull << 31))
+    if (!(a.flags & F_POS) || !a.upt || n_units >= (1ull << 32) || n_tickets != (n_units + a.upt - 1) / a.upt || (u64)a.upt * kRoundsBig * kSegBytes > (1ull << 31) ||
+        tag < kTkTagLegacy || tag > kTkTagLast || !d_slot)
         return hipErrorInvalidValue;
-    return dma_launch1<true>(a, d_agg, d_pref, n_tickets, num_cu, st);
-}
-
-}
+    return dma_launch1<true>(a, d_agg, d_pref, n_tickets, tag, d_slot, num_cu, st);
+}
+
+}
diff --git a/krep_amd/csrc/kg_plan.hip b/krep_amd/csrc/kg_plan.hip
--- a/krep_amd/csrc/kg_plan.hip
+++ b/krep_amd/csrc/kg_plan.hip
@@ -209,6 +209,13 @@
     if (pass_rate) *pass_rate = pl->dma_pass_rate;
     return 0;
 }
+extern "C" int krep_gpu_debug_literal_dma_set_next_tag(krep_gpu_plan_t *pl, uint32_t tag)
+{
+    if (!pl || (tag != 0 && (tag < 0x8001u || tag > 0xFFFFu)))
+        return 2;
+    pl->post.tk_tag = tag;
+    return 0;
+}
 extern "C" int krep_gpu_debug_anchor_measured(const krep_gpu_plan_t *pl, double *measured, int *resamples)
 {
     if (!pl || !pl->ac)
diff --git a/krep_amd/csrc/kg_scan.hip b/krep_amd/csrc/kg_scan.hip
--- a/krep_amd/csrc/kg_scan.hip
+++ b/krep_amd/csrc/kg_scan.hip
@@ -11,6 +11,7 @@
 #include "kg_internal.h"
 #include "kg_plan.h"
 #include "kg_replay.h"
+#include "kg_tickets.h"
 
 using namespace kg;
 
@@ -374,18 +375,42 @@
     static_assert(sizeof(Counters) <= kCtrWords * sizeof(unsigned long long), "the counters in front of the ticket arrays");
     const uint64_t n_tk = (L.n_units + a.upt - 1) / a.upt, cap_tk = n_tk + kCtrWords / 2;
     PostScratch &post = *ps.post;
+    if (cap_tk > post.tk_cap)
+        post.tk_tag = 0;
     HIPCHK(grow_scratch(post.tk_cap, cap_tk, cap_tk, {dev_buf(post.d_tk, 2 * cap_tk * sizeof(unsigned long long))}));
-    Counters *d_ctr = reinterpret_cast<Counters *>(post.d_tk);
+    Counters *d_ctr = reinterpret_cast<Counters *>(post.d_tk), *d_slot = nullptr;
+    HIPCHK(hipHostGetDevicePointer(reinterpret_cast<void **>(&d_slot), pl->h_ctr, 0));
     unsigned long long *d_agg = post.d_tk + kCtrWords, *d_pref = d_agg + n_tk;
     a.ctr = d_ctr;
     a.positions = ps.d_out;
     a.pos_cap = ps.out_cap;
     a.stage_cap = 0;
-    HIPCHK(hipMemsetAsync(post.d_tk, 0, (kCtrWords + 2 * n_tk) * sizeof(unsigned long long), st));
-    HIPCHK(launch_literal_dma_one_pass(a, d_agg, d_pref, n_tk, (uint32_t)pl->num_cu, st));
+    uint32_t tag = post.tk_dirty ? 0u : post.tk_tag;
+    if (a.pos_cap >= (1ull << kTkTagShift) || a.text_len >= (1ull << kTkTagShift))
+    {
+        HIPCHK(hipMemsetAsync(post.d_tk, 0, (kCtrWords + 2 * n_tk) * sizeof(unsigned long long), st));
+        g_lit_dma1p_memsets.fetch_add(1, std::memory_order_relaxed);
+        tag = kTkTagLegacy;
+        post.tk_tag = 0;
+    }
+    else
+    {
+        if (tag == 0)
+        {
+            HIPCHK(hipMemsetAsync(post.d_tk, 0, 2 * post.tk_cap * sizeof(unsigned long long), st));
+            g_lit_dma1p_memsets.fetch_add(1, std::memory_order_relaxed);
+            tag = kTkTagFirst;
+        }
+        post.tk_tag = tk_next_tag(tag);
+    }
+    post.tk_dirty = true;
+    pl->h_ctr->pad[1] = 0;
+    HIPCHK(launch_literal_dma_one_pass(a, d_agg, d_pref, n_tk, tag, d_slot, (uint32_t)pl->num_cu, st));
     if (ps.ev_end) HIPCHK(hipEventRecord(ps.ev_end, st));
-    HIPCHK(hipMemcpyAsync(pl->h_ctr, d_ctr, sizeof(Counters), hipMemcpyDeviceToHost, st));
     HIPCHK(hipStreamSynchronize(st));
+    if (pl->h_ctr->pad[1] != tag)
+        return kg::fail("literal scan: the one-pass kernel left no result (stamp %llx, expected %x)", pl->h_ctr->pad[1], tag);
+    post.tk_dirty = false;
     LitScan La = L;
     La.a = a;
     lit_dma_rate(pl, w, La);
@@ -1198,7 +1223,10 @@
     if (pl->unsupported)
         return kg::fail("%s", pl->unsupported);
     if (kg::inject(3))
+    {
+        pl->post.tk_dirty = true;
         return kg::fail("injected failure: kernel launch");
+    }
     Window w{(const uint8_t *)d_text, text_len, own_lo, own_hi, global_base, global_len};
     if (pl->ref_algo == KREP_RA_AHO_CORASICK)
         return scan_ac(pl, w, d_positions, position_capacity, st, time_it, carry_in, carry_out, out);
diff --git a/krep_amd/csrc/kg_single.hip b/krep_amd/csrc/kg_single.hip
--- a/krep_amd/csrc/kg_single.hip
+++ b/krep_amd/csrc/kg_single.hip
@@ -66,7 +66,7 @@
     }
     if (resolver)
     {
-        tk_resolve(agg, pref, n_tickets, a.ctr, lane);
+        tk_resolve(agg, pref, n_tickets, a.ctr, lane, kTkTagLegacy);
         return;
     }
     unsigned short *ring = s_ring + (size_t)wave * kRing;
@@ -82,7 +82,7 @@
 #ifdef KG_S1_NOWAIT
         const u64 first = pend_t * 1400ull;
 #else
-        const u64 first = tk_wait_prefix(pref, pend_t, a.ctr, lane);
+        const u64 first = tk_wait_prefix(pref, pend_t, a.ctr, lane, kTkTagLegacy);
 #endif
         const u64 tbase = a.anchor + pend_t * (u64)kUpt * kUnitBytes1 + a.global_base;
         const u32 b1 = pend_c0, b2 = pend_c0 + pend_c1, b3 = pend_c0 + pend_c1 + pend_c2;
@@ -458,6 +458,7 @@
         const uint64_t n_tk = single_fused_tickets(n_units, shape);
         const size_t tk_bytes = single_fused_scratch_words(n_tk) * sizeof(unsigned long long);
         HIPCHK(grow_scratch(post.tk_cap, n_tk, n_tk, {dev_buf(post.d_tk, tk_bytes)}));
+        post.tk_tag = 0;
         HIPCHK(hipMemsetAsync(d_ctr, 0, sizeof(Counters), st));
         HIPCHK(hipMemsetAsync(post.d_tk, 0, tk_bytes, st));
         HIPCHK(launch_single_fused(a, post.d_tk, post.d_tk + n_tk, n_tk, num_cu, shape, st));
diff --git a/krep_amd/csrc/kg_tickets.h b/krep_amd/csrc/kg_tickets.h
--- a/krep_amd/csrc/kg_tickets.h
+++ b/krep_amd/csrc/kg_tickets.h
@@ -5,12 +5,35 @@
 
 namespace kg {
 
-constexpr unsigned long long kTkReady = 1ull << 63;
+constexpr uint32_t kTkTagShift = 48;
+constexpr unsigned long long kTkValueMask = (1ull << kTkTagShift) - 1ull;
+constexpr uint32_t kTkTagLegacy = 0x8000u;
+constexpr uint32_t kTkTagFirst = 0x8001u;
+constexpr uint32_t kTkTagLast = 0xFFFFu;
+__host__ __device__ constexpr unsigned long long tk_pack(unsigned long long value, uint32_t tag)
+{
+    return (value & kTkValueMask) | ((unsigned long long)tag << kTkTagShift);
+}
+__host__ __device__ constexpr unsigned long long tk_value(unsigned long long word) { return word & kTkValueMask; }
+__host__ __device__ constexpr uint32_t tk_tag(unsigned long long word) { return (uint32_t)(word >> kTkTagShift); }
+__host__ __device__ constexpr bool tk_ready(unsigned long long word, uint32_t tag) { return tk_tag(word) == tag; }
+__host__ __device__ constexpr uint32_t tk_next_tag(uint32_t tag) { return tag >= kTkTagFirst && tag < kTkTagLast ? tag + 1u : 0u; }
+constexpr unsigned long long kTkReady = tk_pack(0, kTkTagLegacy);
+static_assert(kTkReady == 1ull << 63 && tk_pack(27, kTkTagLegacy) == (27ull | 1ull << 63), "tag 0x8000 is the old ready flag");
+static_assert(tk_value(tk_pack(0, kTkTagFirst)) == 0 && tk_value(tk_pack(kTkValueMask, kTkTagLast)) == kTkValueMask, "values round-trip");
+static_assert(tk_tag(tk_pack(kTkValueMask, kTkTagFirst)) == kTkTagFirst && tk_tag(tk_pack(~0ull, 0x9000u)) == 0x9000u, "a value never reaches the tag");
+static_assert(tk_ready(tk_pack(5, 0x8001u), 0x8001u) && !tk_ready(tk_pack(5, 0x8001u), 0x8002u) && !tk_ready(tk_pack(5, kTkTagLegacy), 0x8001u) &&
+                  !tk_ready(tk_pack(5, 0xFFFFu), 0x8001u),
+              "a word of another generation is not ready");
+static_assert(!tk_ready(0ull, kTkTagLegacy) && !tk_ready(0ull, kTkTagFirst) && !tk_ready(0ull, kTkTagLast), "a zeroed word is ready for nobody");
+static_assert(tk_next_tag(kTkTagFirst) == kTkTagFirst + 1u && tk_next_tag(kTkTagLast - 1u) == kTkTagLast && tk_next_tag(kTkTagLast) == 0u &&
+                  tk_next_tag(0u) == 0u && tk_next_tag(kTkTagLegacy) == 0u,
+              "the step from 0xFFFF (and from no tag at all) asks for a zeroed block");
 constexpr uint32_t kTkSpinLimit = 1u << 24;
 constexpr uint32_t kTkResolveChunk = 8;
 
 __device__ __forceinline__ void tk_resolve(unsigned long long *__restrict__ agg, unsigned long long *__restrict__ pref,
-                                           const unsigned long long n_tickets, Counters *ctr, const uint32_t lane)
+                                           const unsigned long long n_tickets, Counters *ctr, const uint32_t lane, const uint32_t tag)
 {
     u64 running = 0, base = 0;
     u32 spins = 0;
@@ -26,7 +49,7 @@
             const bool valid = mine + k < n_tickets;
             v[k] = valid ? __hip_atomic_load(&agg[mine + k], __ATOMIC_RELAXED, __HIP_MEMORY_SCOPE_AGENT) : 0ull;
             nvalid += valid ? 1u : 0u;
-            run = run && valid && (v[k] & kTkReady);
+            run = run && valid && tk_ready(v[k], tag);
             lead += run ? 1u : 0u;
         }
         const u64 open = __ballot(lead != nvalid);
@@ -35,7 +58,7 @@
         u64 s = 0;
 #pragma unroll
         for (u32 k = 0; k < kTkResolveChunk; ++k)
-            s += k < take ? (v[k] & ~kTkReady) : 0ull;
+            s += k < take ? tk_value(v[k]) : 0ull;
         u64 incl = s;
         u32 tincl = take;
 #pragma unroll
@@ -54,8 +77,8 @@
         for (u32 k = 0; k < kTkResolveChunk; ++k)
         {
             if (k < take)
-                __hip_atomic_store(&pref[mine + k], e | kTkReady, __ATOMIC_RELAXED, __HIP_MEMORY_SCOPE_AGENT);
-            e += k < take ? (v[k] & ~kTkReady) : 0ull;
+                __hip_atomic_store(&pref[mine + k], tk_pack(e, tag), __ATOMIC_RELAXED, __HIP_MEMORY_SCOPE_AGENT);
+            e += k < take ? tk_value(v[k]) : 0ull;
         }
         const u32 published = __shfl(tincl, 63);
         running += __shfl(incl, 63);
@@ -69,7 +92,7 @@
                 if (lane == 0)
                     atomicAdd(&ctr->overflow_units, 1ull);
                 for (u64 t = base + lane; t < n_tickets; t += 64)
-                    __hip_atomic_store(&pref[t], kTkReady, __ATOMIC_RELAXED, __HIP_MEMORY_SCOPE_AGENT);
+                    __hip_atomic_store(&pref[t], tk_pack(0, tag), __ATOMIC_RELAXED, __HIP_MEMORY_SCOPE_AGENT);
                 return;
             }
             __builtin_amdgcn_s_sleep(8);
@@ -80,7 +103,7 @@
 }
 
 __device__ __forceinline__ unsigned long long tk_wait_prefix(const unsigned long long *__restrict__ pref, const unsigned long long t,
-                                                              Counters *ctr, const uint32_t lane)
+                                                              Counters *ctr, const uint32_t lane, const uint32_t tag)
 {
     u64 p = 0;
     if (lane == 0)
@@ -88,38 +111,38 @@
         for (uint32_t spins = 0;; ++spins)
         {
             p = __hip_atomic_load(&pref[t], __ATOMIC_RELAXED, __HIP_MEMORY_SCOPE_AGENT);
-            if (p & kTkReady)
+            if (tk_ready(p, tag))
                 break;
             if (spins > 2u * kTkSpinLimit)
             {
                 atomicAdd(&ctr->overflow_units, 1ull);
-                p = kTkReady;
+                p = tk_pack(0, tag);
                 break;
             }
             __builtin_amdgcn_s_sleep(4);
         }
     }
-    return rfl64(p) & ~kTkReady;
+    return tk_value(rfl64(p));
 }
 
 __device__ __forceinline__ unsigned long long tk_wait_prefix_lane(const unsigned long long *__restrict__ pref, const unsigned long long t,
-                                                                   Counters *ctr)
+                                                                   Counters *ctr, const uint32_t tag)
 {
     u64 p = 0;
     for (uint32_t spins = 0;; ++spins)
     {
         p = __hip_atomic_load(&pref[t], __ATOMIC_RELAXED, __HIP_MEMORY_SCOPE_AGENT);
-        if (p & kTkReady)
+        if (tk_ready(p, tag))
             break;
         if (spins > 2u * kTkSpinLimit)
         {
             atomicAdd(&ctr->overflow_units, 1ull);
-            p = kTkReady;
+            p = tk_pack(0, tag);
             break;
         }
         __builtin_amdgcn_s_sleep(4);
     }
-    return p & ~kTkReady;
+    return tk_value(p);
 }
 
 }
diff --git a/krep_amd/engine.py b/krep_amd/engine.py
--- a/krep_amd/engine.py
+++ b/krep_amd/engine.py
@@ -151,6 +151,10 @@
             L.krep_gpu_debug_literal_dma_one_pass_failovers.restype = C.c_uint64
             L.krep_gpu_debug_force_literal_dma_grid.restype = None
             L.krep_gpu_debug_force_literal_dma_grid.argtypes = [C.c_int]
+        if hasattr(L, "krep_gpu_debug_literal_dma_one_pass_memsets"):
+            L.krep_gpu_debug_literal_dma_one_pass_memsets.restype = C.c_uint64
+            L.krep_gpu_debug_literal_dma_set_next_tag.restype = C.c_int
+            L.krep_gpu_debug_literal_dma_set_next_tag.argtypes = [C.c_void_p, C.c_uint32]
         if hasattr(L, "krep_gpu_alloc_placed"):
             L.krep_gpu_alloc_placed.restype = C.c_int
             L.krep_gpu_alloc_placed.argtypes = [C.c_int, C.c_size_t, C.c_size_t, C.c_int, C.POINTER(C.c_void_p), C.POINTER(C.c_void_p),
@@ -233,6 +237,9 @@
 
     def force_literal_dma_grid(self, blocks: int):
         self.lib.krep_gpu_debug_force_literal_dma_grid(blocks)
+
+    def literal_dma_one_pass_memsets(self) -> int:
+        return int(self.lib.krep_gpu_debug_literal_dma_one_pass_memsets())
 
     def alloc_placed(self, text_bytes: int, record_bytes: int, tries: int = 3, device: int = 0):
         t, r, info = C.c_void_p(0), C.c_void_p(0), abi.Placement()
@@ -823,6 +830,10 @@
             return None
         return int(st.value), int(mv.value), float(r0.value), float(r1.value)
 
+    def literal_dma_set_next_tag(self, tag: int):
+        if self.eng.lib.krep_gpu_debug_literal_dma_set_next_tag(self.h, tag):
+            raise ValueError(f"bad tag {tag:#x}")
+
     def literal_dma_state(self):
         a, b, r = C.c_int(0), C.c_int(0), C.c_double(0)
         if self.eng.lib.krep_gpu_debug_literal_dma_state(self.h, C.byref(a), C.byref(b), C.byref(r)):
```
